# facebookresearch/SlowFast

Measured on AMD Instinct MI355X. Metric: clips/sec (fwd+bwd), SlowFast-8x8-R50 32x224^2 synthetic clips, per-GPU batch 32, higher is better.
Workload: dtype fp16; 1 GPU; SLOWFAST_8x8_R50: forward + cross_entropy loss + backward + sgd step, inputs resident in HBM, per-GPU batch 32; global_batch=32, parallelism=dp1, launch=hip-graph(fwd+bwd) + eager all-reduce/optimizer, optimizer=FlatOptimizer (fused unscale+norm+clip+update, dynamic loss scale on device)

## Files before the change

include/sfamd.h:

```cpp
#ifndef SFAMD_H
#define SFAMD_H
#include <stddef.h>
#include <stdint.h>
#ifdef __cplusplus
extern "C" {
#endif

#define SF_ABI_VERSION 26
typedef void* sf_stream_t;

typedef struct sf_conv_desc {
    int32_t N, Ci, Ti, Hi, Wi;
    int32_t Co, To, Ho, Wo;
    int32_t kT, kH, kW;
    int32_t sT, sH, sW;
    int32_t pT, pH, pW;
    int32_t dT, dH, dW;
    int32_t Cw;
    int32_t ldx, ldy;
    int32_t Cow;
} sf_conv_desc;

int sf_abi_version(void);
const char* sf_backend(void);
#define SF_ACT_FP16 0
#define SF_ACT_BF16_ID 1
int sf_act_dtype(void);
const char* sf_last_error(void);
const char* sf_build_id(void);

int sf_conv_weight_ld(const sf_conv_desc* d, int32_t* ldf, int32_t* ldd);
int sf_prep_weights(const sf_conv_desc* d, const float* w, void* wf, void* wd, sf_stream_t stream);
typedef struct sf_prep_item {
    const float* w;
    void* wf;
    void* wd;
    int32_t Co, Cow, Cw, Cp, taps, ldf, ldd;
    int32_t pad;
} sf_prep_item;
int sf_prep_item_fill(const sf_conv_desc* d, const float* w, void* wf, void* wd, sf_prep_item* item);
int64_t sf_prep_item_blocks(const sf_prep_item* item);
int sf_prep_weights_batch(const sf_prep_item* items, const int32_t* blk_item, const int32_t* blk_off, int32_t nblocks,
                          sf_stream_t stream);
int sf_conv_fwd_mtiles(const sf_conv_desc* d);
int sf_conv_fwd(const sf_conv_desc* d, const void* x, const void* wf, const float* in_scale, const float* in_shift,
                int in_relu, const float* bias, void* y, float* stat_part, sf_stream_t stream);
int sf_conv_fwd_fused(const sf_conv_desc* d, const void* x, const void* wf, const float* bias, const void* resid,
                      int32_t ldr, int out_relu, void* y, sf_stream_t stream);
int sf_conv_dgrad(const sf_conv_desc* d, const void* dy, const void* wd, const void* resid, int32_t ldr,
                  const void* resid_bits, void* dx, sf_stream_t stream);
int sf_conv_dgrad_bn(const sf_conv_desc* d, const void* dy, const void* wd, const void* resid, int32_t ldr,
                     const void* resid_bits, void* dx, const float* mask_scale, const float* mask_shift,
                     const void* mask_bits, const void* bn_y, int32_t bn_ldy, float* bn_part, int32_t bn_part_rows,
                     int32_t* bn_rows, sf_stream_t stream);
int64_t sf_conv_wgrad_workspace(const sf_conv_desc* d);
int64_t sf_conv_wgrad_rowtab_bytes(const sf_conv_desc* d);
int sf_conv_wgrad_rowtab(const sf_conv_desc* d, void* tab, sf_stream_t stream);
int sf_conv_wgrad(const sf_conv_desc* d, const void* x, const float* in_scale, const float* in_shift, int in_relu,
                  const void* dy, float* dw, float out_scale, int zero_first, void* workspace, int64_t workspace_bytes,
                  const void* rowtab, sf_stream_t stream);

int sf_bn_finalize(float* part, int32_t nblk, int32_t C, int32_t Creal, float count, const float* gamma, const float* beta,
                   float* running_mean, float* running_var, float momentum, float eps, float* scale, float* shift,
                   float* save_mean, float* save_rstd, sf_stream_t stream);
int sf_bn_act(int64_t M, int32_t C, const void* y, int32_t ldy, const float* scale, const float* shift, const void* r,
              int32_t ldr, const float* rscale, const float* rshift, int relu, void* out, int32_t ldo, void* mask_out,
              sf_stream_t stream);
int sf_bn_bwd_blocks(int64_t M, int32_t C);
int sf_bn_bwd_reduce(int64_t M, int32_t C, const void* dz, int32_t lddz, const void* zmask, int32_t ldm, const void* y,
                     int32_t ldy, const float* scale, const float* shift, int relu_self, float* part,
                     sf_stream_t stream);
int sf_bn_bwd_finalize(float* part, int32_t nblk, int32_t C, int32_t Creal, float count, const float* gamma, const float* mean,
                       const float* rstd, float inv_loss_scale, float* dgamma, float* dbeta, int accumulate,
                       float* coef, sf_stream_t stream);
int sf_bn_bwd_apply(int64_t M, int32_t C, const void* dz, int32_t lddz, const void* zmask, int32_t ldm, const void* y,
                    int32_t ldy, const float* scale, const float* shift, int relu_self, const float* coef, void* dy,
                    int32_t lddy, void* gout, int32_t ldg, sf_stream_t stream);

int sf_pool_fwd(int32_t N, int32_t T, int32_t H, int32_t W, int32_t C, int32_t kH, int32_t kW, int32_t sH, int32_t sW,
                int32_t pH, int32_t pW, const void* y, int32_t ldy, const float* scale, const float* shift, int relu,
                void* out, int32_t ldo, void* argmax, int32_t cls, sf_stream_t stream);
int sf_pool_bwd(int32_t N, int32_t T, int32_t H, int32_t W, int32_t C, int32_t kH, int32_t kW, int32_t sH, int32_t sW,
                int32_t pH, int32_t pW, const void* pooled, int32_t ldp, const void* argmax, int relu,
                const void* dout, int32_t lddo, void* g, int32_t ldg, int32_t cls, sf_stream_t stream);

int sf_pool3d_fwd(int32_t N, int32_t T, int32_t H, int32_t W, int32_t C, int32_t kT, int32_t kH, int32_t kW, const void* x,
                  int32_t ldx, void* out, int32_t ldo, void* argmax, sf_stream_t stream);
int sf_pool3d_bwd(int32_t N, int32_t T, int32_t H, int32_t W, int32_t C, int32_t kT, int32_t kH, int32_t kW,
                  const void* argmax, const void* dout, int32_t lddo, void* dx, int32_t lddx, sf_stream_t stream);

int sf_ncthw_to_cl(const float* x, int32_t N, int32_t C, int64_t S, int32_t Cp, void* out, sf_stream_t stream);
int sf_cl_to_ncthw(const void* x, int32_t ld, int32_t N, int32_t C, int64_t S, float* out, sf_stream_t stream);


int sf_bgemm(int64_t M, int32_t N, int32_t K, const void* A, int32_t lda, const void* W, int32_t ldw, const float* bias,
             const void* resid, int32_t ldr, void* Y, int32_t ldy, int32_t nbatch, int32_t bh, int64_t sa_b, int64_t sa_h,
             int64_t sw_b, int64_t sw_h, int64_t sy_b, int64_t sy_h, int64_t sr_b, int64_t sr_h, int32_t resid_row0,
             float alpha, sf_stream_t stream);
typedef struct sf_rows32 {
    const float* in;
    float* out;
    int32_t ld, period;
} sf_rows32;
int sf_gemm_rows32(int64_t M, int32_t N, int32_t K, const void* A, int32_t lda, const void* W, int32_t ldw, const float* bias,
                   const void* resid, int32_t ldr, void* Y, int32_t ldy, const sf_rows32* side, sf_stream_t stream);
int sf_bgemm_tn(int64_t M, int32_t R, int32_t Kc, const void* P, int32_t ldp, const void* X, int32_t ldx, void* Out,
                int32_t ldo, float scale, int32_t nbatch, int32_t bh, int64_t sp_b, int64_t sp_h, int64_t sx_b,
                int64_t sx_h, int64_t so_b, int64_t so_h, sf_stream_t stream);

int sf_layernorm_fwd(int64_t M, int32_t C, const void* x, int32_t ldx, const float* gamma, const float* beta, float eps,
                     void* y, int32_t ldy, float* mean, float* rstd, sf_stream_t stream);
int sf_layernorm_fwd_rows32(int64_t M, int32_t C, const void* x, int32_t ldx, const float* gamma, const float* beta, float eps,
                            void* y, int32_t ldy, float* mean, float* rstd, const sf_rows32* side, sf_stream_t stream);
int sf_layernorm_bwd_blocks(int64_t M, int32_t C);
int sf_layernorm_bwd(int64_t M, int32_t C, const void* dy, int32_t lddy, const void* x, int32_t ldx, const float* gamma,
                     const float* mean, const float* rstd, const void* resid, int32_t ldr, void* dx, int32_t lddx,
                     float* part, sf_stream_t stream);
int sf_layernorm_bwd_sums(int64_t M, int32_t C, const void* dy, int32_t lddy, const void* x, int32_t ldx, const float* gamma,
                          const float* mean, const float* rstd, const void* resid, int32_t ldr, void* dx, int32_t lddx,
                          float* part, sf_stream_t stream);
int sf_colsum_blocks(int64_t M, int32_t C);
int sf_colsum(int64_t M, int32_t C, const void* x, int32_t ldx, float* part, sf_stream_t stream);
int sf_colsum_finalize(float* part, int32_t nblk, int32_t C, int32_t fold, float* out0, float* out1, float scale,
                       int accumulate, sf_stream_t stream);
typedef struct sf_colfin_item {
    float* part;
    int32_t nblk, C, fold;
    float* out0;
    float* out1;
    float scale;
    int32_t accumulate;
    int32_t row_stride;
} sf_colfin_item;
int sf_colsum_finalize_batch(const sf_colfin_item* items, int32_t n, sf_stream_t stream);
int sf_rows_sum(const float* part, int32_t nblk, int64_t row_len, int64_t offset, int32_t n, float* out, float scale,
                int accumulate, sf_stream_t stream);
int sf_gelu_fwd(int64_t n, const void* h, void* a, sf_stream_t stream);
int sf_gelu_bwd(int64_t n, const void* h, const void* da, void* dh, sf_stream_t stream);

typedef struct sf_dw_desc {
    int32_t N, C, Cw, cls;
    int32_t Ti, Hi, Wi, To, Ho, Wo;
    int32_t kT, kH, kW, sT, sH, sW, pT, pH, pW;
    int32_t ldx, ldy;
    int32_t Cwreal;
} sf_dw_desc;
int sf_dwconv_fwd_blocks(const sf_dw_desc* d);
int sf_dwconv_fwd_sample_rows(const sf_dw_desc* d);
int sf_dwconv_fwd(const sf_dw_desc* d, const void* x, const float* w, void* y, float* stat_part, sf_stream_t stream);
int sf_dwconv_dgrad(const sf_dw_desc* d, const void* dy, const float* w, void* dx, sf_stream_t stream);
int sf_dwconv_dgrad_sum_rows(const sf_dw_desc* d);
int sf_dwconv_dgrad_sums(const sf_dw_desc* d, const void* dy, const float* w, void* dx, float* sum_part, sf_stream_t stream);
int64_t sf_dwconv_wgrad_workspace(const sf_dw_desc* d);
int sf_dwconv_wgrad(const sf_dw_desc* d, const void* x, const void* dy, float* dw, float out_scale, int zero_first,
                    void* workspace, int64_t workspace_bytes, sf_stream_t stream);
int sf_dwconv_pair_ok(const sf_dw_desc* d);
int sf_dwconv_fwd_pair(const sf_dw_desc* d, const void* x, const void* x2, const float* w, const float* w2, void* y, void* y2,
                       sf_stream_t stream);
int sf_dwconv_dgrad_pair(const sf_dw_desc* d, const void* dy, const void* dy2, const float* w, const float* w2, void* dx, void* dx2,
                         sf_stream_t stream);
int sf_dwconv_wgrad_pair(const sf_dw_desc* d, const void* x, const void* x2, const void* dy, const void* dy2, float* dw, float* dw2,
                         float out_scale, int zero_first, int zero_first2, void* workspace, int64_t workspace_bytes,
                         sf_stream_t stream);

typedef struct sf_attn_desc {
    int32_t B, heads, D, cls;
    int32_t Nq, qT, qH, qW;
    int32_t Nk, kT, kH, kW;
    int32_t rows_h, rows_w, rows_t;
} sf_attn_desc;
int sf_relpos_gather(const sf_attn_desc* d, const void* G, int32_t ldg, const int32_t* idx_h, const int32_t* idx_w,
                     const int32_t* idx_t, float* rq, sf_stream_t stream);
int sf_relpos_scatter(const sf_attn_desc* d, const float* drq, const int32_t* idx_h, const int32_t* idx_w,
                      const int32_t* idx_t, void* E, int32_t lde, sf_stream_t stream);
int sf_relpos_pack(const float* rel_h, const float* rel_w, const float* rel_t, int32_t rows_h, int32_t rows_w, int32_t rows_t,
                   int32_t D, int32_t TRp, void* t16, void* t16t, sf_stream_t stream);
int sf_relpos_unpack(const float* dtab, int32_t rows_h, int32_t rows_w, int32_t rows_t, int32_t D, float* grad_h, float* grad_w,
                     float* grad_t, int32_t acc_h, int32_t acc_w, int32_t acc_t, sf_stream_t stream);
int sf_softmax_fwd(const sf_attn_desc* d, void* s, int32_t lds, float scale, const float* rq, sf_stream_t stream);
int sf_softmax_bwd(const sf_attn_desc* d, void* dp, const void* prob, int32_t lds, float scale, float* drq,
                   sf_stream_t stream);
int sf_attn_fwd(const sf_attn_desc* d, const void* q, int32_t ldq, const void* k, const void* v, int32_t ldk, float scale,
                const float* rq, const void* onehot, int32_t residual, void* o, int32_t ldo, float* lse,
                sf_stream_t stream);
int64_t sf_attn_bwd_workspace(const sf_attn_desc* d);
int sf_attn_bwd(const sf_attn_desc* d, const void* q, int32_t ldq, const void* k, const void* v, int32_t ldk, float scale,
                const float* rq, const void* onehot, int32_t residual, const void* o, const void* dout, int32_t ldo,
                const float* lse, float* delta, void* dq, int32_t lddq, void* dk, void* dv, int32_t lddk, float* drq,
                void* workspace, int64_t workspace_bytes, sf_stream_t stream);
int sf_tmean_fwd(int32_t B, int32_t T, int64_t HW, int32_t C, const void* x, int32_t ldx, float* m, sf_stream_t stream);
int sf_tmean_bwd(int32_t B, int32_t T, int64_t HW, int32_t C, const float* dm, void* dx, int32_t lddx, sf_stream_t stream);
int sf_roi_align_max_fwd(int32_t R, int32_t B, int32_t H, int32_t W, int32_t C, int32_t res, float scale, int32_t aligned,
                         const float* m, const float* rois, float* out, int32_t ldo, int32_t col0, void* argmax,
                         sf_stream_t stream);
int sf_roi_align_max_bwd(int32_t R, int32_t B, int32_t H, int32_t W, int32_t C, int32_t res, float scale, int32_t aligned,
                         const float* rois, const float* dout, int32_t lddo, int32_t col0, const void* argmax, float* dm,
                         sf_stream_t stream);
int sf_gemm_act(int64_t M, int32_t N, int32_t K, const void* A, int32_t lda, const void* W, int32_t ldw, const float* bias,
                void* Y, int32_t ldy, int32_t mode, void* aux, int32_t ldaux, sf_stream_t stream);
int sf_gemm_act_colsum(int64_t M, int32_t N, int32_t K, const void* A, int32_t lda, const void* W, int32_t ldw,
                       const float* bias, void* Y, int32_t ldy, int32_t mode, void* aux, int32_t ldaux,
                       float* colsum_part, int32_t colsum_part_rows, int32_t* colsum_rows, sf_stream_t stream);
int sf_pack_clip_u8(const void* frames, int32_t N, int32_t Tin, int32_t H, int32_t W, const int32_t* t_index, int32_t Tout,
                    float mean0, float mean1, float mean2, float std0, float std1, float std2, int32_t reverse, void* out,
                    sf_stream_t stream);
int sf_mix_clip_f32(const float* src, float* dst, int32_t B, int32_t C, int32_t T, int32_t H, int32_t W, int32_t mode,
                    float lam, float one_minus_lam, int32_t yl, int32_t yh, int32_t xl, int32_t xh, sf_stream_t stream);
// ... 72 lines not shown
```

slowfast_amd/csrc/sf_api.hip:

```cpp
#include "../../include/sfamd.h"
#include "sf_bn.h"
#include "sf_common.h"
#include "sf_igemm.h"
#include "sf_igemm2.h"
#include "sf_wgrad2.h"
#include "sf_pool.h"
#include "sf_dwconv.h"
#include "sf_dwsweep.h"
#include "sf_dwtemporal.h"
#include "sf_tokens.h"
#include "sf_x3d.h"
#include "sf_stem.h"
#include "sf_attn.h"
#include "sf_roi.h"
#include "sf_optim.h"
#include "sf_mixup.h"
#include "sf_erase.h"

#include <stdarg.h>
#include <stdio.h>
#include <stdlib.h>
#include <string.h>

static thread_local char g_err[512] = "";

static int fail(const char* fmt, ...) {
    va_list ap;
    va_start(ap, fmt);
    vsnprintf(g_err, sizeof(g_err), fmt, ap);
    va_end(ap);
    return -1;
}
static int check_launch(const char* what) {
    hipError_t e = hipGetLastError();
    if (e != hipSuccess) return fail("%s: launch failed: %s", what, hipGetErrorString(e));
    return 0;
}
#define REQUIRE(cond, ...) \
    do { if (!(cond)) return fail(__VA_ARGS__); } while (0)

static inline int cdiv(int64_t a, int64_t b) { return (int)((a + b - 1) / b); }
static inline int roundup(int a, int b) { return (a + b - 1) / b * b; }

static inline int test_hook(const char* name, int def) { const char* e = getenv(name); return e ? atoi(e) : def; }
#ifdef SF_DIAG
static inline int tune_knob(const char* name, int def) { const char* e = getenv(name); return e ? atoi(e) : def; }
#else
#define tune_knob(name, def) (def)
#endif

extern "C" int sf_abi_version(void) { return SF_ABI_VERSION; }
extern "C" const char* sf_backend(void) {
#ifdef SF_HOSTSIM
    return "hostsim";
#else
    return "gfx950";
#endif
}
extern "C" int sf_act_dtype(void) { return SF_ACT_DTYPE_ID; }
extern "C" const char* sf_last_error(void) { return g_err; }
#ifndef SF_BUILD_ID
#define SF_BUILD_ID "unversioned"
#endif
extern "C" const char* sf_build_id(void) {
    static const char tagged[] = "sfamd-build-id:" SF_BUILD_ID;
    return tagged + 15;
}

static int check_desc(const sf_conv_desc* d) {
    REQUIRE(d != nullptr, "conv: null descriptor");
    REQUIRE(d->N > 0 && d->Ci > 0 && d->Co > 0, "conv: empty tensor");
    REQUIRE(d->Ci % 8 == 0 && d->Co % 8 == 0, "conv: channel counts must be multiples of 8 (Ci=%d Co=%d)", d->Ci, d->Co);
    REQUIRE(d->ldx >= d->Ci && d->ldx % 8 == 0 && d->ldy >= d->Co && d->ldy % 8 == 0, "conv: bad row pitch");
    REQUIRE(d->Cw > 0 && d->Cw <= d->Ci, "conv: Cw must be in (0, Ci]");
    REQUIRE(d->Cow >= 0 && d->Cow <= d->Co, "conv: Cow must be in [0, Co]");
    REQUIRE(d->sT > 0 && d->sH > 0 && d->sW > 0 && d->dT > 0 && d->dH > 0 && d->dW > 0, "conv: stride/dilation");
    int To = (d->Ti + 2 * d->pT - d->dT * (d->kT - 1) - 1) / d->sT + 1;
    int Ho = (d->Hi + 2 * d->pH - d->dH * (d->kH - 1) - 1) / d->sH + 1;
    int Wo = (d->Wi + 2 * d->pW - d->dW * (d->kW - 1) - 1) / d->sW + 1;
    REQUIRE(d->To >= 1 && d->Ho >= 1 && d->Wo >= 1 && d->To <= To && d->Ho <= Ho && d->Wo <= Wo,
            "conv: output dims (%d,%d,%d) exceed the geometry's (%d,%d,%d)", d->To, d->Ho, d->Wo, To, Ho, Wo);
    int64_t Mo = (int64_t)d->N * d->To * d->Ho * d->Wo, Mi = (int64_t)d->N * d->Ti * d->Hi * d->Wi;
    REQUIRE(Mo < (1ll << 31) && Mi < (1ll << 31), "conv: more than 2^31 positions");
    return 0;
}

static void fill_gather_common(GatherSide& g, const sf_conv_desc* d) {
    g.kT = d->kT; g.kH = d->kH; g.kW = d->kW;
    g.strT = d->sT; g.strH = d->sH; g.strW = d->sW;
    g.padT = d->pT; g.padH = d->pH; g.padW = d->pW;
    g.dilT = d->dT; g.dilH = d->dH; g.dilW = d->dW;
    g.fdkW = make_fastdiv(d->kW);
    g.fdkH = make_fastdiv(d->kH);
    g.fdsT = make_fastdiv(d->sT);
    g.fdsH = make_fastdiv(d->sH);
    g.fdsW = make_fastdiv(d->sW);
    g.scale = nullptr; g.shift = nullptr; g.relu = 0;
    g.fdHW = make_fastdiv((uint32_t)d->Hi * (uint32_t)d->Wi);
}
static bool is_pointwise(const sf_conv_desc* d) {
    return d->kH == 1 && d->kW == 1 && d->sT == 1 && d->sH == 1 && d->sW == 1 && d->pH == 0 && d->pW == 0 &&
           d->Ho == d->Hi && d->Wo == d->Wi;
}

static GatherSide gather_fwd(const sf_conv_desc* d, const void* x, const float* sc, const float* sh, int relu) {
    GatherSide g;
    memset(&g, 0, sizeof(g));
    fill_gather_common(g, d);
    g.src = (const f16*)x; g.ld = d->ldx; g.C = d->Ci;
    g.sT = d->Ti; g.sH = d->Hi; g.sW = d->Wi;
    g.mode = 0;
    g.Ktot = d->kT * d->kH * d->kW * d->Ci;
    g.fdC = make_fastdiv(d->Ci);
    g.fdrW = make_fastdiv(d->Wo); g.fdrH = make_fastdiv(d->Ho); g.fdrT = make_fastdiv(d->To);
    g.rowT = d->To;
    g.scale = sc; g.shift = sh; g.relu = relu;
    return g;
}
static GatherSide gather_dgrad(const sf_conv_desc* d, const void* dy) {
    GatherSide g;
    memset(&g, 0, sizeof(g));
    fill_gather_common(g, d);
    g.src = (const f16*)dy; g.ld = d->ldy; g.C = d->Co;
    g.sT = d->To; g.sH = d->Ho; g.sW = d->Wo;
    g.mode = 1;
    g.Ktot = d->kT * d->kH * d->kW * d->Co;
    g.fdC = make_fastdiv(d->Co);
    g.fdrW = make_fastdiv(d->Wi); g.fdrH = make_fastdiv(d->Hi); g.fdrT = make_fastdiv(d->Ti);
    g.rowT = d->Ti;
    return g;
}

static bool igemm_glds_ok(const IgemmParams& p, bool pw) {
    static const bool off = tune_knob("SF_IGEMM_GLDS", 1) == 0;
    if (off || !pw || p.g.scale) return false;
    if (p.g.Ktot != p.g.C || p.g.Ktot % 32 != 0 || p.g.ld % 8 != 0 || p.ldw % 8 != 0) return false;
    if (p.g.padT != 0) return false;
    if (((uintptr_t)p.g.src | (uintptr_t)p.wmat) & 15) return false;
    if (p.bh > 0 && ((p.sa_b | p.sa_h | p.sw_b | p.sw_h) & 7)) return false;
    return true;
}

template <int BN, int WM, int WN>
static void launch_igemm(const IgemmParams& p, bool pw, hipStream_t s, int nbatch = 1) {
    int mt = cdiv(p.M, 128);
    dim3 grid((unsigned)(mt * p.ntiles_n), (unsigned)nbatch);
    static const bool occ4 = tune_knob("SF_IGEMM_OCC4", 1) != 0;
    if (p.f32.out) {
        if (igemm_glds_ok(p, pw)) hipLaunchKernelGGL((sf_igemm_kernel<BN, WM, WN, true, true, BN == 128, true>), grid, dim3(SF_THREADS), 0, s, p);
        else hipLaunchKernelGGL((sf_igemm_kernel<BN, WM, WN, true, false, BN == 128, true>), grid, dim3(SF_THREADS), 0, s, p);
        return;
    }
    if (igemm_glds_ok(p, pw)) {
        hipLaunchKernelGGL((sf_igemm_kernel<BN, WM, WN, true, true, BN == 128>), grid, dim3(SF_THREADS), 0, s, p);
        return;
    }
    constexpr bool kCap = BN == 128;
    const bool cap = kCap && occ4;
    if (pw) {
        if (cap) hipLaunchKernelGGL((sf_igemm_kernel<BN, WM, WN, true, false, kCap>), grid, dim3(SF_THREADS), 0, s, p);
        else hipLaunchKernelGGL((sf_igemm_kernel<BN, WM, WN, true, false, false>), grid, dim3(SF_THREADS), 0, s, p);
    } else {
        if (cap) hipLaunchKernelGGL((sf_igemm_kernel<BN, WM, WN, false, false, kCap>), grid, dim3(SF_THREADS), 0, s, p);
        else hipLaunchKernelGGL((sf_igemm_kernel<BN, WM, WN, false, false, false>), grid, dim3(SF_THREADS), 0, s, p);
    }
}

template <int BN, int BK>
static void launch_igemm2(Igemm2Params& q, hipStream_t s) {
    q.ntiles_n = cdiv(q.Nout, BN);
    const dim3 grid((unsigned)(cdiv(q.M, 256) * q.ntiles_n));
    if constexpr (BN >= 64) {
        if (q.f32.out) { hipLaunchKernelGGL((sf_igemm2_kernel<256, BN, 4, 2, BK, 3, true>), grid, dim3(512), 0, s, q); return; }
    }
    hipLaunchKernelGGL((sf_igemm2_kernel<256, BN, 4, 2, BK, 3>), grid, dim3(512), 0, s, q);
}
static void launch_igemm2_auto(Igemm2Params& q, hipStream_t s) {
    const char* e;
    const int tiles = cdiv(q.M, 256) * cdiv(q.Nout, q.Nout > 64 ? 128 : 64);
    const int force_bk = tune_knob("SF_IGEMM2_BK", 0);
    const bool bk64 = q.C % 64 == 0 && force_bk != 32 && (force_bk == 64 || tiles <= 320);
    static const bool trace = test_hook("SF_TRACE", 0) != 0;
    q.ablate = tune_knob("SF_IGEMM2_ABLATE", 0);
    if (trace) fprintf(stderr, "[sfamd] igemm2: M=%d N=%d C=%d taps=%d BK=%d omap=%d\n", q.M, q.Nout, q.C, q.ntaps, bk64 ? 64 : 32, q.omap);
    const int t128 = test_hook("SF_IGEMM2_T128", 1);
    if (t128 && q.linear && q.Nout > 64 && !q.stat_part && !q.bnb_part && (!bk64 || t128 == 2)) {
        q.ntiles_n = cdiv(q.Nout, 128);
        const dim3 grid((unsigned)(cdiv(q.M, 128) * q.ntiles_n));
        if (q.f32.out) hipLaunchKernelGGL((sf_igemm2_kernel<128, 128, 2, 2, 32, 3, true>), grid, dim3(256), 0, s, q);
        else hipLaunchKernelGGL((sf_igemm2_kernel<128, 128, 2, 2, 32, 3>), grid, dim3(256), 0, s, q);
        return;
    }
    if (q.Nout > 64) { if (bk64) launch_igemm2<128, 64>(q, s); else launch_igemm2<128, 32>(q, s); }
    else if (q.Nout > 32) { if (bk64) launch_igemm2<64, 64>(q, s); else launch_igemm2<64, 32>(q, s); }
    else launch_igemm2<32, 32>(q, s);
}
static bool igemm2_operands_ok(const IgemmParams& p, int nbatch) {
    const GatherSide& g = p.g;
    if (nbatch != 1 || g.scale) return false;
    if (p.bh > 1 || (p.bh == 1 && (p.sa_b | p.sa_h | p.sw_b | p.sw_h | p.sy_b | p.sy_h | p.sr_b | p.sr_h))) return false;
    const int taps = g.kT * g.kH * g.kW;
    if (taps > SF_I2_MAXTAPS || g.C % 32 != 0 || g.Ktot != taps * g.C) return false;
    if (g.ld % 8 != 0 || p.ldw % 8 != 0 || p.ldw < g.Ktot) return false;
    if (((uintptr_t)g.src | (uintptr_t)p.wmat) & 15) return false;
    if ((g.kT - 1) * g.dilT > 127 || (g.kH - 1) * g.dilH > 127 || (g.kW - 1) * g.dilW > 127) return false;
    return true;
}
static void igemm2_common(Igemm2Params& q, const IgemmParams& p) {
    const GatherSide& g = p.g;
    memset(&q, 0, sizeof(q));
    q.src = g.src; q.ld = g.ld; q.C = g.C;
    q.sT = g.sT; q.sH = g.sH; q.sW = g.sW;
    q.wmat = p.wmat; q.ldw = p.ldw; q.Nout = p.Nout;
    q.y = p.y; q.ldy = p.ldy; q.bias = p.bias; q.resid = p.resid; q.ldr = p.ldr; q.stat_part = p.stat_part;
    q.act_mode = p.act_mode; q.act_aux = p.act_aux; q.ld_aux = p.ld_aux; q.resid_row0 = p.resid_row0; q.alpha = p.alpha;
    q.resid_bits = p.resid_bits;
    q.bnb_y = p.bnb_y; q.bnb_ld = p.bnb_ld; q.bnb_scale = p.bnb_scale; q.bnb_shift = p.bnb_shift; q.bnb_part = p.bnb_part;
    q.bnb_bits = p.bnb_bits;
    q.f32 = p.f32;
    q.linear = p.linear;
}
static bool try_igemm2(const IgemmParams& p, hipStream_t s, int nbatch = 1) {
    const char* e;
    const bool off = test_hook("SF_IGEMM2", 1) == 0;
    const int mink = test_hook("SF_IGEMM2_MINK", 512);
    const int minrows = test_hook("SF_IGEMM2_MINROWS", 4096);
    const GatherSide& g = p.g;
    if (off || !igemm2_operands_ok(p, nbatch)) return false;
    if (g.Ktot < mink || p.Nout <= 32 || p.M < minrows) return false;
    if (g.mode == 1 && !(g.strT == 1 && g.strH == 1 && g.strW == 1)) return false;
    const int taps = g.kT * g.kH * g.kW;
    Igemm2Params q;
    igemm2_common(q, p);
    q.fdrW = g.fdrW; q.fdrH = g.fdrH; q.fdrT = g.fdrT;
    const int sgn = g.mode == 0 ? 1 : -1;
    if (g.mode == 0) {
        q.mulT = g.strT; q.mulH = g.strH; q.mulW = g.strW;
        q.offT = -g.padT; q.offH = -g.padH; q.offW = -g.padW;
    } else {
        q.mulT = q.mulH = q.mulW = 1;
        q.offT = g.padT; q.offH = g.padH; q.offW = g.padW;
    }
    q.ntaps = taps;
    int t = 0;
    for (int kt = 0; kt < g.kT; ++kt)
        for (int kh = 0; kh < g.kH; ++kh)
            for (int kw = 0; kw < g.kW; ++kw, ++t) {
                const int dt = sgn * kt * g.dilT, dh = sgn * kh * g.dilH, dw = sgn * kw * g.dilW;
                q.dt[t] = (int8_t)dt; q.dh[t] = (int8_t)dh; q.dw[t] = (int8_t)dw;
                q.taps[t].dlin = (dt * g.sH + dh) * g.sW + dw;
                q.taps[t].wcol = t * g.C;
            }
    q.M = p.M;
    launch_igemm2_auto(q, s);
    return true;
}

static bool try_igemm2_strided_dgrad(const IgemmParams& p, hipStream_t s) {
    const char* e;
    const bool off = test_hook("SF_IGEMM2", 1) == 0 || tune_knob("SF_IGEMM2_STRIDED", 1) == 0;
    const int minrows = test_hook("SF_IGEMM2_MINROWS", 4096);
    const GatherSide& g = p.g;
    if (off || g.mode != 1 || (g.strT == 1 && g.strH == 1 && g.strW == 1)) return false;
    if (!igemm2_operands_ok(p, 1) || p.Nout <= 16 || p.M < minrows || p.stat_part || p.act_mode) return false;
    const int Ti = (int)g.fdrT.d, Hi = (int)g.fdrH.d, Wi = (int)g.fdrW.d;
    const int N = p.M / (Ti * Hi * Wi);
    const int str[3] = {g.strT, g.strH, g.strW}, pad[3] = {g.padT, g.padH, g.padW}, dil[3] = {g.dilT, g.dilH, g.dilW};
    const int ker[3] = {g.kT, g.kH, g.kW}, ext[3] = {Ti, Hi, Wi};
    for (int rt = 0; rt < str[0]; ++rt)
        for (int rh = 0; rh < str[1]; ++rh)
            for (int rw = 0; rw < str[2]; ++rw) {
                const int r[3] = {rt, rh, rw};
                int q0[3], cnt[3];
                bool empty = false;
                for (int a = 0; a < 3; ++a) {
                    const int num = pad[a] - r[a];
                    q0[a] = num > 0 ? (num + str[a] - 1) / str[a] : 0;
                    const int top = ext[a] - 1 + pad[a] - r[a];
                    const int q1 = top >= 0 ? top / str[a] : -1;
                    cnt[a] = q1 - q0[a] + 1;
                    if (cnt[a] <= 0) empty = true;
                }
                if (empty) continue;
                Igemm2Params q;
                igemm2_common(q, p);
                q.fdrT = make_fastdiv(cnt[0]); q.fdrH = make_fastdiv(cnt[1]); q.fdrW = make_fastdiv(cnt[2]);
                q.mulT = q.mulH = q.mulW = 1;
                q.offT = q0[0]; q.offH = q0[1]; q.offW = q0[2];
                int nt = 0, tap = 0;
                for (int kt = 0; kt < ker[0]; ++kt)
                    for (int kh = 0; kh < ker[1]; ++kh)
                        for (int kw = 0; kw < ker[2]; ++kw, ++tap) {
                            const int k[3] = {kt, kh, kw};
                            int d[3];
                            bool ok = true;
                            for (int a = 0; a < 3; ++a) {
                                const int v = r[a] - k[a] * dil[a];
                                if (v % str[a] != 0) { ok = false; break; }
                                d[a] = v / str[a];
                            }
                            if (!ok) continue;
                            q.dt[nt] = (int8_t)d[0]; q.dh[nt] = (int8_t)d[1]; q.dw[nt] = (int8_t)d[2];
                            q.taps[nt].dlin = (d[0] * g.sH + d[1]) * g.sW + d[2];
                            q.taps[nt].wcol = tap * g.C;
                            ++nt;
                        }
                q.ntaps = nt;
                q.M = N * cnt[0] * cnt[1] * cnt[2];
                q.omap = 1;
                q.oT = Ti; q.oH = Hi; q.oW = Wi;
                q.omT = str[0]; q.omH = str[1]; q.omW = str[2];
                q.ooT = str[0] * q0[0] + r[0] - pad[0]; q.ooH = str[1] * q0[1] + r[1] - pad[1]; q.ooW = str[2] * q0[2] + r[2] - pad[2];
                launch_igemm2_auto(q, s);
            }
    return true;
}

static int run_igemm(IgemmParams& p, bool pw, hipStream_t s, int* bm_used = nullptr) {
    if (bm_used) *bm_used = 256;
    if (try_igemm2(p, s)) return check_launch("igemm2");
    if (bm_used) *bm_used = 0;
    if (try_igemm2_strided_dgrad(p, s)) return check_launch("igemm2 strided dgrad");
    if (bm_used) *bm_used = 128;
    if (p.Nout > 64) { p.ntiles_n = cdiv(p.Nout, 128); launch_igemm<128, 64, 64>(p, pw, s); }
    else if (p.Nout > 32) { p.ntiles_n = 1; launch_igemm<64, 32, 64>(p, pw, s); }
    else if (p.Nout > 16) { p.ntiles_n = 1; launch_igemm<32, 32, 32>(p, pw, s); }
    else { p.ntiles_n = 1; launch_igemm<16, 32, 16>(p, pw, s); }
    return check_launch("igemm");
}

struct StemPlan {
    bool ok, thin3, small;
    int tiles_w, tiles_h, tiles_t, ntiles, F, PR;
    int wg_blocks, tiles_per_block, Kpad, wgroups;
    size_t ws_bytes;
};
static StemPlan plan_stem(const sf_conv_desc* d) {
    StemPlan s;
    memset(&s, 0, sizeof(s));
    static const bool off = tune_knob("SF_STEM_GENERIC", 0) != 0;
    if (off) return s;
    static const bool thin3_on = tune_knob("SF_STEM_THIN3", 1) != 0;
    const bool stemlike = d->kW == 4 && d->pW == 2;
    const bool thin3 = thin3_on && d->kW == 3 && d->pW == 1 && d->sH == 1 && d->sT == 1;
    if (d->Ci != 8 || d->Cw != 8 || !(stemlike || thin3) || d->sW != 1 || d->dT != 1 || d->dH != 1 || d->dW != 1)
        return s;
    s.thin3 = thin3;
    if (d->Co > 16 || d->Co % 8 != 0 || (d->Cow && d->Cow != d->Co)) return s;
    if (d->kT * d->kH > SF_STEM_MAX_SLICES) return s;
    s.F = (SF_STEM_TT - 1) * d->sT + d->kT;
    s.PR = (SF_STEM_TH - 1) * d->sH + d->kH;
    if ((int64_t)s.F * s.PR * SF_STEM_PC > SF_STEM_CHUNKS) return s;
    s.small = (int64_t)s.F * s.PR * SF_STEM_PC <= SF_STEM_CHUNKS_SMALL;
    s.tiles_w = cdiv(d->Wo, SF_STEM_TW);
    s.tiles_h = cdiv(d->Ho, SF_STEM_TH);
    s.tiles_t = cdiv(d->To, SF_STEM_TT);
    const int64_t nt = (int64_t)d->N * s.tiles_t * s.tiles_h * s.tiles_w;
    if (nt >= (1ll << 30)) return s;
    s.ntiles = (int)nt;
    const int gmax = s.small ? 1024 : 512;
    int g = s.ntiles < gmax ? s.ntiles : gmax;
    s.tiles_per_block = cdiv(s.ntiles, g);
    s.wg_blocks = cdiv(s.ntiles, s.tiles_per_block);
    s.Kpad = roundup(d->kT * d->kH * 32, 128);
    { const int nsl = d->kT * d->kH; s.wgroups = nsl <= 4 ? 8 / nsl : 1; }
    s.ws_bytes = (size_t)s.wg_blocks * s.wgroups * 16 * s.Kpad * 4;
    s.ok = true;
    return s;
}
#define SF_STEM_SLIDE_GROUPS 4
#define SF_STEM_FWD_LAUNCH(sp, q, stream)                                                                                          \
    do {                                                                                                                          \
        static const bool rm_ = tune_knob("SF_STEM_ROWMAJOR", 1) != 0;                           \
        const dim3 g_((sp).ntiles), b_(SF_THREADS);                                                                               \
        const int sg_ = test_hook("SF_STEM_SLIDE", SF_STEM_SLIDE_GROUPS);                                                         \
        if (rm_ && sg_ > 0 && (q).sH == 2 && (q).kH == 7 && !(sp).small && (q).sT == 1 && (q).kT > 1 && (q).kT <= 5 &&            \
            (q).Co <= 8 && !(q).bnb_y) {                                                                                                         \
            StemParams qs_ = (q);                    \
            qs_.seg_groups = sg_ < (sp).tiles_t ? sg_ : (sp).tiles_t;                                                             \
            qs_.tiles_t = cdiv((sp).tiles_t, qs_.seg_groups);                                                                     \
            qs_.fd_tt = make_fastdiv(qs_.tiles_t);                                                                                \
            const dim3 gs_((unsigned)((int64_t)(q).N * qs_.tiles_t * (sp).tiles_h * (sp).tiles_w));                                \
            if (test_hook("SF_TRACE", 0)) fprintf(stderr, "[sfamd] stem_fwd_slide: %u runs of %d groups\n", gs_.x, qs_.seg_groups); \
            hipLaunchKernelGGL((sf_stem_fwd_slide_kernel<2, 7>), gs_, b_, 0, (hipStream_t)(stream), qs_);                         \
        } else if (rm_ && (q).sH == 2 && (q).kH == 7 && !(sp).small)                                                              \
            hipLaunchKernelGGL((sf_stem_fwd_kernel<SF_STEM_CHUNKS, 2, 7>), g_, b_, 0, (hipStream_t)(stream), q);                  \
        else if (rm_ && (q).sH == 1 && (q).kH == 3 && (sp).small)                                                                 \
            hipLaunchKernelGGL((sf_stem_fwd_kernel<SF_STEM_CHUNKS_SMALL, 1, 3>), g_, b_, 0, (hipStream_t)(stream), q);            \
        else if ((sp).small) hipLaunchKernelGGL((sf_stem_fwd_kernel<SF_STEM_CHUNKS_SMALL>), g_, b_, 0, (hipStream_t)(stream), q); \
        else hipLaunchKernelGGL((sf_stem_fwd_kernel<SF_STEM_CHUNKS>), g_, b_, 0, (hipStream_t)(stream), q);                       \
    } while (0)
static StemParams stem_params(const sf_conv_desc* d, const StemPlan& s, const void* x) {
    StemParams p;
    memset(&p, 0, sizeof(p));
    p.x = (const f16*)x; p.ldx = d->ldx;
    p.N = d->N; p.Ti = d->Ti; p.Hi = d->Hi; p.Wi = d->Wi;
    p.To = d->To; p.Ho = d->Ho; p.Wo = d->Wo; p.Co = d->Co;
    p.kT = d->kT; p.kH = d->kH; p.sT = d->sT; p.sH = d->sH; p.pT = d->pT; p.pH = d->pH;
    p.pW = d->pW;
    if (s.thin3) { p.wo0 = 0; p.wos = 24; p.wog = 8; p.kwc = 3; }
    else { p.wo0 = 0; p.wos = 32; p.wog = 8; p.kwc = 4; }
    p.ldy = d->ldy;
    p.tiles_w = s.tiles_w; p.tiles_h = s.tiles_h; p.tiles_t = s.tiles_t; p.ntiles = s.ntiles;
    p.fd_tw = make_fastdiv(s.tiles_w); p.fd_th = make_fastdiv(s.tiles_h); p.fd_tt = make_fastdiv(s.tiles_t);
    p.F = s.F; p.PR = s.PR;
    p.fd_pc = make_fastdiv(SF_STEM_PC); p.fd_prpc = make_fastdiv(s.PR * SF_STEM_PC);
    p.Kpad = s.Kpad; p.tiles_per_block = s.tiles_per_block; p.wgroups = s.wgroups;
    return p;
}

extern "C" int sf_conv_weight_ld(const sf_conv_desc* d, int32_t* ldf, int32_t* ldd) {
    REQUIRE(d && ldf && ldd, "sf_conv_weight_ld: null argument");
    int taps = d->kT * d->kH * d->kW;
    *ldf = roundup(taps * d->Ci, 32);
    *ldd = roundup(taps * d->Co, 32);
    return 0;
}

static PrepParams prep_params(const sf_conv_desc* d, const float* w, void* wf, void* wd) {
    PrepParams p;
    memset(&p, 0, sizeof(p));
    p.w = w; p.Co = d->Co; p.Cow = d->Cow ? d->Cow : d->Co; p.Cw = d->Cw; p.Cp = d->Ci; p.taps = d->kT * d->kH * d->kW;
    int32_t ldf, ldd;
    sf_conv_weight_ld(d, &ldf, &ldd);
    p.wf = (f16*)wf; p.ldf = ldf; p.wd = (f16*)wd; p.ldd = ldd;
    return p;
}

extern "C" int sf_prep_weights(const sf_conv_desc* d, const float* w, void* wf, void* wd, sf_stream_t stream) {
    if (check_desc(d)) return -1;
    REQUIRE(w && wf, "sf_prep_weights: null pointer");
    const PrepParams p = prep_params(d, w, wf, wd);
    int64_t total = (int64_t)p.Co * p.ldf + (wd ? (int64_t)p.Cp * p.ldd : 0);
    int blocks = (int)((total + SF_THREADS - 1) / SF_THREADS);
    if (blocks > 4096) blocks = 4096;
    hipLaunchKernelGGL(sf_prep_weights_kernel, dim3(blocks), dim3(SF_THREADS), 0, (hipStream_t)stream, p);
    return check_launch("prep_weights");
}

static_assert(sizeof(sf_prep_item) == sizeof(PrepParams), "sf_prep_item must mirror PrepParams");
extern "C" int sf_prep_item_fill(const sf_conv_desc* d, const float* w, void* wf, void* wd, sf_prep_item* item) {
    if (check_desc(d)) return -1;
    REQUIRE(w && wf && item, "sf_prep_item_fill: null pointer");
    PrepParams p = prep_params(d, w, wf, wd);
    p.pad = sf_prep_tile_co(p.taps);
    memcpy(item, &p, sizeof(p));
    return 0;
}

extern "C" int64_t sf_prep_item_blocks(const sf_prep_item* item) {
    REQUIRE(item && item->Co > 0 && item->ldf > 0 && item->taps > 0, "sf_prep_item_blocks: bad item");
    REQUIRE(item->pad == sf_prep_tile_co(item->taps), "sf_prep_item_blocks: item was not written by sf_prep_item_fill");
    if (item->pad > 0) return (int64_t)cdiv(item->Co, item->pad) * cdiv(item->Cp, SF_PREP_TILE_CI);
    const int64_t n = (int64_t)item->Co * item->ldf + (item->wd ? (int64_t)item->Cp * item->ldd : 0);
    return cdiv(n, SF_PREP_BLOCK_ELEMS);
}

extern "C" int sf_prep_weights_batch(const sf_prep_item* items, const int32_t* blk_item, const int32_t* blk_off,
                                     int32_t nblocks, sf_stream_t stream) {
    REQUIRE(items && blk_item && blk_off && nblocks > 0, "sf_prep_weights_batch: bad arguments");
    hipLaunchKernelGGL(sf_prep_weights_batch_kernel, dim3(nblocks), dim3(SF_THREADS), 0, (hipStream_t)stream,
                       (const PrepParams*)items, blk_item, blk_off);
    return check_launch("prep_weights_batch");
}

extern "C" int sf_conv_fwd_mtiles(const sf_conv_desc* d) {
    if (!d) return fail("sf_conv_fwd_mtiles: null descriptor");
    return cdiv((int64_t)d->N * d->To * d->Ho * d->Wo, 128);
}

extern "C" int sf_conv_fwd(const sf_conv_desc* d, const void* x, const void* wf, const float* in_scale,
                           const float* in_shift, int in_relu, const float* bias, void* y, float* stat_part,
                           sf_stream_t stream) {
    if (check_desc(d)) return -1;
    REQUIRE(x && wf && y, "sf_conv_fwd: null pointer");
    REQUIRE((in_scale == nullptr) == (in_shift == nullptr), "sf_conv_fwd: in_scale/in_shift must come together");
    REQUIRE(!in_scale || d->Ci <= 512, "sf_conv_fwd: fused input BatchNorm supports Ci <= 512 (got %d)", d->Ci);
    if (!in_scale && !bias) {
        const StemPlan sp = plan_stem(d);
        if (sp.ok && (!stat_part || sp.ntiles <= sf_conv_fwd_mtiles(d))) {
            StemParams q = stem_params(d, sp, x);
            int32_t ldf0, ldd0;
            sf_conv_weight_ld(d, &ldf0, &ldd0);
            q.wmat = (const f16*)wf; q.ldw = ldf0; q.y = (f16*)y;
            q.stat_part = stat_part; q.stat_rows = sf_conv_fwd_mtiles(d);
            const bool trace = test_hook("SF_TRACE", 0) != 0;
            if (trace) fprintf(stderr, "[sfamd] stem_fwd: %d tiles, patch %dx%dx%d chunks\n", sp.ntiles, sp.F, sp.PR, SF_STEM_PC);
            SF_STEM_FWD_LAUNCH(sp, q, stream);
            return check_launch("stem_fwd");
        }
    }
    IgemmParams p;
    memset(&p, 0, sizeof(p));
    p.g = gather_fwd(d, x, in_scale, in_shift, in_relu);
    p.M = d->N * d->To * d->Ho * d->Wo;
    int32_t ldf, ldd;
    sf_conv_weight_ld(d, &ldf, &ldd);
    p.wmat = (const f16*)wf; p.ldw = ldf; p.Nout = d->Co;
    p.ksteps = cdiv(p.g.Ktot, 32);
    p.y = (f16*)y; p.ldy = d->ldy;
    p.bias = bias; p.resid = nullptr; p.ldr = 0;
    p.stat_part = stat_part;
    return run_igemm(p, is_pointwise(d), (hipStream_t)stream);
}

extern "C" int sf_conv_fwd_fused(const sf_conv_desc* d, const void* x, const void* wf, const float* bias,
                                 const void* resid, int32_t ldr, int out_relu, void* y, sf_stream_t stream) {
    if (check_desc(d)) return -1;
    REQUIRE(x && wf && y, "sf_conv_fwd_fused: null pointer");
    REQUIRE(!resid || (ldr >= d->Co && ldr % 8 == 0), "sf_conv_fwd_fused: bad residual pitch");
    if (!resid) {
        const StemPlan sp = plan_stem(d);
        if (sp.ok) {
            StemParams q = stem_params(d, sp, x);
            int32_t ldf0, ldd0;
            sf_conv_weight_ld(d, &ldf0, &ldd0);
            q.wmat = (const f16*)wf; q.ldw = ldf0; q.y = (f16*)y;
            q.bias = bias; q.out_relu = out_relu;
            SF_STEM_FWD_LAUNCH(sp, q, stream);
            return check_launch("stem_fwd_fused");
        }
    }
    IgemmParams p;
    memset(&p, 0, sizeof(p));
    p.g = gather_fwd(d, x, nullptr, nullptr, 0);
    p.M = d->N * d->To * d->Ho * d->Wo;
    int32_t ldf, ldd;
    sf_conv_weight_ld(d, &ldf, &ldd);
    p.wmat = (const f16*)wf; p.ldw = ldf; p.Nout = d->Co;
    p.ksteps = cdiv(p.g.Ktot, 32);
    p.y = (f16*)y; p.ldy = d->ldy;
    p.bias = bias; p.resid = (const f16*)resid; p.ldr = ldr;
    p.act_mode = out_relu ? 3 : 0;
    return run_igemm(p, is_pointwise(d), (hipStream_t)stream);
}

struct BnFuse {
    const float* scale; const float* shift; const void* bits;
    const void* y0; int32_t ld0; float* part0;
};
static int conv_dgrad_impl(const sf_conv_desc* d, const void* dy, const void* wd, const void* resid, int32_t ldr,
                           const void* resid_bits, void* dx, const BnFuse* bn, int32_t* bn_rows, sf_stream_t stream) {
    if (check_desc(d)) return -1;
    REQUIRE(dy && wd && dx, "sf_conv_dgrad: null pointer");
    REQUIRE(!resid || (ldr >= d->Ci && ldr % 8 == 0), "sf_conv_dgrad: bad residual pitch");
    IgemmParams p;
    memset(&p, 0, sizeof(p));
    p.g = gather_dgrad(d, dy);
    p.M = d->N * d->Ti * d->Hi * d->Wi;
    int32_t ldf, ldd;
    sf_conv_weight_ld(d, &ldf, &ldd);
    p.wmat = (const f16*)wd; p.ldw = ldd; p.Nout = d->Ci;
    p.ksteps = cdiv(p.g.Ktot, 32);
    p.y = (f16*)dx; p.ldy = d->ldx;
    p.resid = (const f16*)resid; p.ldr = ldr;
    REQUIRE(!resid_bits || resid, "sf_conv_dgrad: resid_bits without a residual");
    p.resid_bits = (const uint8_t*)resid_bits;
    const bool fuse = bn && d->sT == 1 && d->sH == 1 && d->sW == 1;
    if (!resid && d->Co == 8 && d->To == d->Ti && d->Ho == d->Hi && d->Wo == d->Wi) {
        sf_conv_desc dd = *d;
        dd.Ci = d->Co; dd.Cw = d->Co; dd.Co = d->Ci; dd.Cow = 0;
        dd.pT = d->kT - 1 - d->pT; dd.pH = d->kH - 1 - d->pH; dd.pW = d->kW - 1 - d->pW;
        dd.ldx = d->ldy; dd.ldy = d->ldx;
        const StemPlan sp = plan_stem(&dd);
        if (sp.ok && sp.thin3 && (!fuse || sp.ntiles <= cdiv(p.M, 128))) {
            StemParams q = stem_params(&dd, sp, dy);
            const int S = d->kT * d->kH;
            q.wmat = (const f16*)wd; q.ldw = ldd; q.y = (f16*)dx;
            q.wo0 = ((S - 1) * 3 + 2) * 8; q.wos = -24; q.wog = -8; q.kwc = 3;
            if (fuse) {
                q.bnb_y = (const f16*)bn->y0; q.bnb_ld = bn->ld0; q.bnb_scale = bn->scale; q.bnb_shift = bn->shift;
                q.bnb_bits = (const uint8_t*)bn->bits;
                q.stat_part = bn->part0; q.stat_rows = 0;
            }
            SF_STEM_FWD_LAUNCH(sp, q, stream);
            if (bn_rows) *bn_rows = fuse ? sp.ntiles : 0;
            return check_launch("stem_dgrad");
        }
    }
    if (fuse) {
        p.bnb_y = (const f16*)bn->y0; p.bnb_ld = bn->ld0; p.bnb_part = bn->part0;
        p.bnb_scale = bn->scale; p.bnb_shift = bn->shift; p.bnb_bits = (const uint8_t*)bn->bits;
    }
    int bm = 0;
    const int rc = run_igemm(p, is_pointwise(d), (hipStream_t)stream, &bm);
    if (bn_rows) *bn_rows = (fuse && bm > 0) ? cdiv(p.M, bm) : 0;
    return rc;
}

extern "C" int sf_conv_dgrad(const sf_conv_desc* d, const void* dy, const void* wd, const void* resid, int32_t ldr,
                             const void* resid_bits, void* dx, sf_stream_t stream) {
    return conv_dgrad_impl(d, dy, wd, resid, ldr, resid_bits, dx, nullptr, nullptr, stream);
}

extern "C" int sf_conv_dgrad_bn(const sf_conv_desc* d, const void* dy, const void* wd, const void* resid, int32_t ldr,
                                const void* resid_bits, void* dx, const float* mask_scale, const float* mask_shift,
                                const void* mask_bits, const void* bn_y, int32_t bn_ldy, float* bn_part, int32_t bn_part_rows,
                                int32_t* bn_rows, sf_stream_t stream) {
    REQUIRE(d && bn_y && bn_part && bn_rows, "sf_conv_dgrad_bn: null pointer");
    REQUIRE(mask_bits || (mask_scale && mask_shift), "sf_conv_dgrad_bn: a mask source is needed (mask_bits, or mask_scale + mask_shift)");
    REQUIRE(bn_ldy >= d->Ci && bn_ldy % 8 == 0 && ((uintptr_t)bn_y & 15) == 0, "sf_conv_dgrad_bn: bad bn_y pitch / alignment");
    REQUIRE((int64_t)bn_part_rows * 128 >= (int64_t)d->N * d->Ti * d->Hi * d->Wi,
            "sf_conv_dgrad_bn: the partial table needs ceil(positions / 128) rows of [2][Ci] floats");
    const BnFuse bn = {mask_scale, mask_shift, mask_bits, bn_y, bn_ldy, bn_part};
    return conv_dgrad_impl(d, dy, wd, resid, ldr, resid_bits, dx, &bn, bn_rows, stream);
}

template <int BMW, int WM, int WN, int KS>
static void launch_wgrad(WgradParams& p, dim3 grid3, hipStream_t s) {
    p.tiles_k = grid3.x; p.tiles_c = grid3.y;
    const dim3 grid(grid3.x * grid3.y * grid3.z);
    hipLaunchKernelGGL((sf_wgrad_kernel<BMW, WM, WN, KS>), grid, dim3(SF_THREADS), 0, s, p);
}

struct WgradPlan {
    int BMW, KS, tiles_k, tiles_c, Co_pad, Kpad, nchunks, chunks_per_split, splits;
    size_t ws_bytes;
};
static WgradPlan plan_wgrad(const sf_conv_desc* d) {
    WgradPlan w;
    const int taps = d->kT * d->kH * d->kW;
    const int Ktot = taps * d->Ci;
    const int64_t M = (int64_t)d->N * d->To * d->Ho * d->Wo;
    w.BMW = d->Co >= 128 ? 128 : d->Co >= 64 ? 64 : d->Co >= 32 ? 32 : 16;
    w.KS = w.BMW <= 32 ? 4 : 1;
    w.tiles_k = cdiv(Ktot, 128);
    w.tiles_c = cdiv(d->Co, w.BMW);
    w.Kpad = w.tiles_k * 128;
    w.Co_pad = w.tiles_c * w.BMW;
    w.nchunks = cdiv(M, 32);
    const int64_t slab = (int64_t)w.Co_pad * w.Kpad * 4;
    static const int target = tune_knob("SF_WGRAD_BLOCKS", 1024);
    int splits = cdiv(target, (int64_t)w.tiles_k * w.tiles_c);
    const int64_t cap = (256ll << 20) / slab;
    if (splits > cap) splits = (int)(cap < 1 ? 1 : cap);
    const int nstages = cdiv(w.nchunks, w.KS);
    if (splits > nstages) splits = nstages;
    if (splits < 1) splits = 1;
    w.chunks_per_split = cdiv(nstages, splits) * w.KS;
    w.splits = cdiv(w.nchunks, w.chunks_per_split);
    w.ws_bytes = (size_t)slab * w.splits;
    return w;
}

struct Wgrad2Plan {
    bool ok, thin, dual;
    int BMW, BKW, tiles_k, tiles_c, Co_pad, Kpad, rows_per_split, splits;
    int slabs;
    size_t tab_bytes, ws_bytes;
};
static Wgrad2Plan plan_wgrad2(const sf_conv_desc* d) {
    Wgrad2Plan w;
    memset(&w, 0, sizeof(w));
    const char* e;
    if (test_hook("SF_WGRAD2", 1) == 0) return w;
    const int mink = test_hook("SF_WGRAD2_MINK", 192);
    const int minrows = test_hook("SF_WGRAD2_MINROWS", 4096);
    const int taps = d->kT * d->kH * d->kW;
    const int target = test_hook("SF_WGRAD2_BLOCKS", 512);
    (void)taps;
    const int Ktot = taps * d->Ci;
    const int64_t M = (int64_t)d->N * d->To * d->Ho * d->Wo;
    if (taps > SF_I2_MAXTAPS || M < minrows) return w;
    if ((d->kT - 1) * d->dT > 127 || (d->kH - 1) * d->dH > 127 || (d->kW - 1) * d->dW > 127) return w;
    if (plan_stem(d).ok) return w;
    if (d->Co <= 32) {
        if (test_hook("SF_WGRAD2T", 1) == 0) return w;
        const int minrows_t = test_hook("SF_WGRAD2T_MINROWS", 16384);
        if (M < minrows_t) return w;
        w.thin = true;
        w.BMW = d->Co <= 16 ? 16 : 32;
        w.BKW = Ktot <= 32 ? 32 : 128;
        w.tiles_k = cdiv(Ktot, w.BKW);
        w.tiles_c = 1;
        w.Kpad = w.tiles_k * w.BKW;
        w.Co_pad = w.BMW;
        const int target_t = test_hook("SF_WGRAD2T_BLOCKS", w.BKW == 128 ? 512 : w.BMW == 32 ? 768 : 1024);
        int splits = target_t / w.tiles_k;
        if (splits < 1) splits = 1;
        w.rows_per_split = roundup(cdiv(M, splits), 128);
        w.splits = cdiv(M, w.rows_per_split);
        w.tab_bytes = ((size_t)M * 8 + 255) / 256 * 256 + 1280;
        w.ws_bytes = w.tab_bytes + (size_t)w.Co_pad * w.Kpad * 4 * w.splits;
        w.slabs = w.splits;
        w.ok = true;
        return w;
    }
    if (Ktot < mink) return w;
    w.BMW = d->Co > 64 ? 128 : 64;
    w.tiles_k = cdiv(Ktot, 256);
    w.tiles_c = cdiv(d->Co, w.BMW);
    w.Kpad = w.tiles_k * 256;
    w.Co_pad = w.tiles_c * w.BMW;
    int splits = target / (w.tiles_k * w.tiles_c);
    const int64_t slab = (int64_t)w.Co_pad * w.Kpad * 4;
    const int64_t cap = (256ll << 20) / slab;
    if (splits > cap) splits = (int)(cap < 1 ? 1 : cap);
    if (splits < 1) splits = 1;
    w.dual = false;
    if (splits >= 2 && test_hook("SF_WGRAD2_DUAL", 1) != 0) {
        const int tiles = w.tiles_k * w.tiles_c;
        const int pairs = (target / 2) / tiles;
        const int64_t steps = cdiv(cdiv(M, splits), 32);
        if (pairs >= 1 && 2 * pairs * 10 >= (2 * pairs < splits ? splits : 2 * pairs) * 9 && steps <= test_hook("SF_WGRAD2_DUAL_STEPS", 80)) {
            w.dual = true;
            if (2 * pairs < splits) splits = 2 * pairs;
        }
    }
    w.rows_per_split = roundup(cdiv(M, splits), 32);
    w.splits = cdiv(M, w.rows_per_split);
    if (w.splits < 2) w.dual = false;
    w.slabs = w.dual ? cdiv(w.splits, 2) : w.splits;
    w.tab_bytes = ((size_t)M * 8 + 255) / 256 * 256 + 1280;
    w.ws_bytes = w.tab_bytes + (size_t)slab * w.splits;
    w.ok = true;
    return w;
}

static void launch_rowtab(const sf_conv_desc* d, void* tab, hipStream_t s) {
    RowtabParams t;
    memset(&t, 0, sizeof(t));
    t.tab = (i32x2*)tab;
    t.M = d->N * d->To * d->Ho * d->Wo;
    t.fdW = make_fastdiv(d->Wo); t.fdH = make_fastdiv(d->Ho); t.fdT = make_fastdiv(d->To);
    t.sT = d->Ti; t.sH = d->Hi; t.sW = d->Wi;
    t.strT = d->sT; t.strH = d->sH; t.strW = d->sW; t.padT = d->pT; t.padH = d->pH; t.padW = d->pW;
    t.ntaps = d->kT * d->kH * d->kW;
    int ti = 0;
    for (int kt = 0; kt < d->kT; ++kt)
        for (int kh = 0; kh < d->kH; ++kh)
            for (int kw = 0; kw < d->kW; ++kw, ++ti) {
                t.dt[ti] = (int8_t)(kt * d->dT); t.dh[ti] = (int8_t)(kh * d->dH); t.dw[ti] = (int8_t)(kw * d->dW);
            }
    hipLaunchKernelGGL(sf_wgrad2_rowtab_kernel, dim3(cdiv(t.M, SF_THREADS)), dim3(SF_THREADS), 0, s, t);
}

extern "C" int64_t sf_conv_wgrad_rowtab_bytes(const sf_conv_desc* d) {
    if (check_desc(d)) return -1;
    const Wgrad2Plan w2 = plan_wgrad2(d);
    return w2.ok ? (int64_t)w2.tab_bytes : 0;
}

extern "C" int sf_conv_wgrad_rowtab(const sf_conv_desc* d, void* tab, sf_stream_t stream) {
    if (check_desc(d)) return -1;
    REQUIRE(tab && (uintptr_t)tab % 16 == 0, "sf_conv_wgrad_rowtab: tab must be a 16-byte aligned device pointer");
    REQUIRE(plan_wgrad2(d).ok, "sf_conv_wgrad_rowtab: this geometry does not take the row-table kernel (sf_conv_wgrad_rowtab_bytes == 0)");
    launch_rowtab(d, tab, (hipStream_t)stream);
    return check_launch("wgrad_rowtab");
}

extern "C" int64_t sf_conv_wgrad_workspace(const sf_conv_desc* d) {
    if (check_desc(d)) return -1;
    int64_t generic = (int64_t)plan_wgrad(d).ws_bytes;
    const Wgrad2Plan w2 = plan_wgrad2(d);
    if (w2.ok && (int64_t)w2.ws_bytes > generic) generic = (int64_t)w2.ws_bytes;
    const StemPlan sp = plan_stem(d);
    return sp.ok && (int64_t)sp.ws_bytes > generic ? (int64_t)sp.ws_bytes : generic;
}
// ... 2009 lines not shown
```

slowfast_amd/csrc/sf_igemm.h:

```cpp
#pragma once
#include "sf_common.h"

struct IgemmParams {
    GatherSide g;
    int M;
    const f16* wmat;
    int ldw;
    int Nout;
    int ksteps;
    f16* y;
    int ldy;
    const float* bias;
    const f16* resid;
    int ldr;
    float* stat_part;
    int ntiles_n;
    int bh;
    int64_t sa_b, sa_h, sw_b, sw_h, sy_b, sy_h, sr_b, sr_h;
    int act_mode;
    f16* act_aux;
    int ld_aux;
    int resid_row0;
    const uint8_t* resid_bits;
    float alpha;
    const f16* bnb_y; int bnb_ld;
    const float* bnb_scale; const float* bnb_shift;
    float* bnb_part;
    const uint8_t* bnb_bits;
    F32Rows f32;
    int linear;
};

__device__ __forceinline__ void bnb_accumulate(const f16x8& dz, const f16x8& yv, const float (&sc)[8], const float (&sh)[8],
                                               float (&sg)[8], float (&sgy)[8], bool use_bits, uint32_t bits) {
#pragma unroll
    for (int e = 0; e < 8; ++e) {
        const bool open = use_bits ? ((bits >> e) & 1u) != 0u : ((float)yv[e] * sc[e] + sh[e] > 0.f);
        const float g = open ? (float)dz[e] : 0.f;
        sg[e] += g;
        sgy[e] += g * (float)yv[e];
    }
}

struct EpiLoads {
    f16x8 r, y;
    uint32_t rbits, bbits;
};

template <int NW, int CG>
__device__ __forceinline__ void bnb_reduce_store(float (&sg)[8], float (&sgy)[8], float* red, float* prow, int n0, int Nout,
                                                 float* sgy2 = nullptr, float* prow2 = nullptr) {
    const int tid = threadIdx.x, lane = tid & 63, wave = tid >> 6;
#pragma unroll
    for (int e = 0; e < 8; ++e)
        for (int mask = CG; mask < 64; mask <<= 1) {
            sg[e] += __shfl_xor(sg[e], mask);
            sgy[e] += __shfl_xor(sgy[e], mask);
            if (prow2) sgy2[e] += __shfl_xor(sgy2[e], mask);
        }
    __syncthreads();
    if (lane < CG) {
#pragma unroll
        for (int e = 0; e < 8; ++e) {
            red[(wave * CG + lane) * 24 + e] = sg[e];
            red[(wave * CG + lane) * 24 + 8 + e] = sgy[e];
            if (prow2) red[(wave * CG + lane) * 24 + 16 + e] = sgy2[e];
        }
    }
    __syncthreads();
    if (tid < CG * 8) {
        const int cgi = tid >> 3, e = tid & 7;
        const int col = n0 + cgi * 8 + e;
        if (col < Nout) {
            float s = 0.f, q = 0.f, q2 = 0.f;
#pragma unroll
            for (int w = 0; w < NW; ++w) {
                s += red[(w * CG + cgi) * 24 + e];
                q += red[(w * CG + cgi) * 24 + 8 + e];
                if (prow2) q2 += red[(w * CG + cgi) * 24 + 16 + e];
            }
            prow[col] = s;
            prow[Nout + col] = q;
            if (prow2) { prow2[col] = s; prow2[Nout + col] = q2; }
        }
    }
}

template <int BN, int WM, int WN, bool PW, bool GL = false, bool OCC4 = false, bool F32R = false>
__global__ __launch_bounds__(SF_THREADS, OCC4 ? 4 : 1) void sf_igemm_kernel(IgemmParams p) {
    constexpr int BM = 128, BK = 32;
    constexpr int NST = 2;
    constexpr int WAVES_N = BN / WN, WAVES_M = BM / WM;
    static_assert(WAVES_M * WAVES_N == 4, "4 waves per workgroup");
    constexpr int TM = WM / 16, TN = WN / 16;
    constexpr int A_ELEMS = BM * BK, B_ELEMS = BN * BK;
    constexpr int STG_LD = BN + 8;
    constexpr int SMEM_MAIN = NST * (A_ELEMS + B_ELEMS), SMEM_STG = BM * STG_LD;
    constexpr int SMEM = SMEM_MAIN > SMEM_STG ? SMEM_MAIN : SMEM_STG;
    constexpr int NB = (BN * 4 + SF_THREADS - 1) / SF_THREADS;

    constexpr int TF_BYTES = GL ? 0 : 2 * 512 * 4;
    __shared__ __attribute__((aligned(16))) unsigned char lds_raw[SMEM * 2 + TF_BYTES + WAVES_M * 2 * BN * 4];
    f16* const smem = reinterpret_cast<f16*>(lds_raw);
    float* const s_scale = reinterpret_cast<float*>(lds_raw + SMEM * 2);
    float* const s_shift = s_scale + 512;
    float (*const s_red)[2][BN] = reinterpret_cast<float (*)[2][BN]>(lds_raw + SMEM * 2 + TF_BYTES);

    const int tid = threadIdx.x;
    const int lane = tid & 63, wave = __builtin_amdgcn_readfirstlane(tid >> 6);
    const int wm = wave / WAVES_N, wn = wave % WAVES_N;
    const int tile = (int)xcd_remap(blockIdx.x, gridDim.x);
    const int nt = tile % p.ntiles_n, mt = tile / p.ntiles_n;
    const int m0 = mt * BM, n0 = nt * BN;
    const GatherSide& g = p.g;
    const bool has_tf = g.scale != nullptr;
    const f16* a_src = g.src;
    const f16* wmat = p.wmat;
    f16* yout = p.y;
    const f16* resid = p.resid;
    if (p.bh > 0) {
        const int zb = blockIdx.y / p.bh, zj = blockIdx.y % p.bh;
        a_src += zb * p.sa_b + zj * p.sa_h;
        wmat += zb * p.sw_b + zj * p.sw_h;
        yout += zb * p.sy_b + zj * p.sy_h;
        if (resid) resid += zb * p.sr_b + zj * p.sr_h;
    }

    if constexpr (!GL) {
        if (has_tf) {
            for (int c = tid; c < g.C; c += SF_THREADS) {
                s_scale[c] = g.scale[c];
                s_shift[c] = g.shift[c];
            }
        }
    }

    const int kq = tid & 3;
    RowPos rp[2];
    if constexpr (!GL) {
#pragma unroll
        for (int j = 0; j < 2; ++j) {
            int row = m0 + (tid >> 2) + 64 * j;
            rp[j] = PW ? decode_row_pw(g, (uint32_t)row, row < p.M) : decode_row(g, (uint32_t)row, row < p.M);
        }
    }
    const float act_lo = g.relu ? 0.f : -INFINITY;
    constexpr int NBC = (BN / 16 + 3) / 4;
    const f16* ga[2];
    const f16* gb[NBC];
    if constexpr (GL) {
#pragma unroll
        for (int j = 0; j < 2; ++j) {
            const int row = (wave + 4 * j) * 16 + (lane >> 2);
            const int slot = ((lane & 3) - 2 * ((row >> 2) & 3)) & 3;
            int m = m0 + row;
            if (m >= p.M) m = p.M - 1;
            ga[j] = a_src + (int64_t)m * g.ld + slot * 8;
        }
#pragma unroll
        for (int j = 0; j < NBC; ++j) {
            const int row = (wave + 4 * j) * 16 + (lane >> 2);
            const int slot = ((lane & 3) - 2 * ((row >> 2) & 3)) & 3;
            int co = n0 + row;
            if (co >= p.Nout) co = p.Nout - 1;
            gb[j] = wmat + (int64_t)co * p.ldw + slot * 8;
        }
    }
    auto issue_tile = [&](int ks, int buf) {
        f16* As = smem + buf * (A_ELEMS + B_ELEMS);
        f16* Bs = As + A_ELEMS;
#pragma unroll
        for (int j = 0; j < 2; ++j) SF_GLOBAL_LOAD_LDS16(ga[j] + ks * BK, As + (wave + 4 * j) * 16 * BK);
#pragma unroll
        for (int j = 0; j < NBC; ++j)
            if ((wave + 4 * j) * 16 < BN) SF_GLOBAL_LOAD_LDS16(gb[j] + ks * BK, Bs + (wave + 4 * j) * 16 * BK);
    };

    struct Stage {
        f16x8 ra[2], rb[NB];
        bool ok[2];
        uint32_t c0;
    };
    Stage st0;

    auto load_tile = [&](int ks, Stage& st) {
        const uint32_t k0 = (uint32_t)(ks * BK + kq * 8);
#pragma unroll
        for (int j = 0; j < 2; ++j) {
            int64_t off;
            uint32_t c0 = 0;
            bool ok = PW ? gather_offset_pw(g, rp[j], k0, off, c0) : gather_offset(g, rp[j], k0, off, c0);
            st.ra[j] = ok ? ld16(a_src + off) : zero8();
            st.ok[j] = ok;
            if (ok) st.c0 = c0;
        }
#pragma unroll
        for (int j = 0; j < NB; ++j) {
            int idx = tid + SF_THREADS * j;
            int brow = idx >> 2;
            int co = n0 + brow;
            bool ok = (idx < BN * 4) && (co < p.Nout) && (k0 < (uint32_t)g.Ktot);
            st.rb[j] = ok ? ld16(wmat + (int64_t)co * p.ldw + k0) : zero8();
        }
    };
    auto store_tile = [&](int buf, const Stage& st) {
        f16* As = smem + buf * (A_ELEMS + B_ELEMS);
        f16* Bs = As + A_ELEMS;
#pragma unroll
        for (int j = 0; j < 2; ++j) {
            f16x8 v = st.ra[j];
            if (has_tf && st.ok[j]) v = bn_act8(v, s_scale + st.c0, s_shift + st.c0, act_lo);
            st16(As + lds_tile_off((tid >> 2) + 64 * j, kq), v);
        }
#pragma unroll
        for (int j = 0; j < NB; ++j) {
            int idx = tid + SF_THREADS * j;
            if (idx < BN * 4) st16(Bs + lds_tile_off(idx >> 2, kq), st.rb[j]);
        }
    };

    f32x4 acc[TM][TN];
#pragma unroll
    for (int i = 0; i < TM; ++i)
#pragma unroll
        for (int j = 0; j < TN; ++j) acc[i][j] = (f32x4){0.f, 0.f, 0.f, 0.f};

    auto compute = [&](int buf) {
        const f16* As = smem + buf * (A_ELEMS + B_ELEMS);
        const f16* Bs = As + A_ELEMS;
        f16x8 af[TM], bf[TN];
#pragma unroll
        for (int i = 0; i < TM; ++i) af[i] = ld16(As + lds_tile_off(wm * WM + i * 16 + (lane & 15), lane >> 4));
#pragma unroll
        for (int j = 0; j < TN; ++j) bf[j] = ld16(Bs + lds_tile_off(wn * WN + j * 16 + (lane & 15), lane >> 4));
#pragma unroll
        for (int i = 0; i < TM; ++i)
#pragma unroll
            for (int j = 0; j < TN; ++j)
                acc[i][j] = SF_MFMA16(af[i], bf[j], acc[i][j]);
    };

    if constexpr (GL) {
        issue_tile(0, 0);
        SF_WAIT_VMEM();
        __syncthreads();
        for (int ks = 0; ks < p.ksteps; ++ks) {
            if (ks + 1 < p.ksteps) issue_tile(ks + 1, (ks + 1) & 1);
            compute(ks & 1);
            SF_WAIT_VMEM();
            __syncthreads();
        }
    } else {
        if (has_tf) __syncthreads();
        load_tile(0, st0);
        store_tile(0, st0);
        __syncthreads();
        for (int ks = 0; ks < p.ksteps; ++ks) {
            const bool more = ks + 1 < p.ksteps;
            if (more) load_tile(ks + 1, st0);
            compute(ks & 1);
            if (more) store_tile((ks + 1) & 1, st0);
            __syncthreads();
        }
    }

    {
        const float alpha = p.alpha != 0.f ? p.alpha : 1.f;
#pragma unroll
        for (int j = 0; j < TN; ++j) {
            const int colj = n0 + wn * WN + j * 16 + (lane & 15);
            const float b = (p.bias && colj < p.Nout) ? p.bias[colj] : 0.f;
#pragma unroll
            for (int i = 0; i < TM; ++i)
#pragma unroll
                for (int r = 0; r < 4; ++r) acc[i][j][r] = acc[i][j][r] * alpha + b;
        }
    }
    if constexpr (F32R) f32_rows_epilogue<TM, TN>(acc, p.f32, m0 + wm * WM, n0 + wn * WN, p.M, p.Nout, resid, p.ldr, p.resid_row0);
    if (p.stat_part) {
#pragma unroll
        for (int j = 0; j < TN; ++j) {
            float s = 0.f, q = 0.f;
#pragma unroll
            for (int i = 0; i < TM; ++i)
#pragma unroll
                for (int r = 0; r < 4; ++r) {
                    const bool rowok = m0 + wm * WM + i * 16 + 4 * (lane >> 4) + r < p.M;
                    const float v = rowok ? acc[i][j][r] : 0.f;
                    s += v;
                    q += v * v;
                }
            s = wave_sum_over_row_groups(s);
            q = wave_sum_over_row_groups(q);
            if (lane < 16) {
                s_red[wm][0][wn * WN + j * 16 + lane] = s;
                s_red[wm][1][wn * WN + j * 16 + lane] = q;
            }
        }
    }
    f16* stg = smem;
#pragma unroll
    for (int i = 0; i < TM; ++i)
#pragma unroll
        for (int j = 0; j < TN; ++j) {
            const int col = wn * WN + j * 16 + (lane & 15);
#pragma unroll
            for (int r = 0; r < 4; ++r) {
                const int row = wm * WM + i * 16 + 4 * (lane >> 4) + r;
                stg[row * STG_LD + col] = (f16)acc[i][j][r];
            }
        }
    __syncthreads();
    if (p.stat_part && tid < BN) {
        const int col = n0 + tid;
        if (col < p.Nout) {
            float s = 0.f, q = 0.f;
#pragma unroll
            for (int w = 0; w < WAVES_M; ++w) {
                s += s_red[w][0][tid];
                q += s_red[w][1][tid];
            }
            p.stat_part[((int64_t)mt * 2 + 0) * p.Nout + col] = s;
            p.stat_part[((int64_t)mt * 2 + 1) * p.Nout + col] = q;
        }
    }
    constexpr int CG = BN / 8;
    static_assert(SF_THREADS % CG == 0 && 64 % CG == 0, "a thread keeps one column group over the whole store loop");
    const bool bnb = p.bnb_part != nullptr;
    float bsg[8], bsgy[8], bsc[8], bsh[8];
#pragma unroll
    for (int e = 0; e < 8; ++e) { bsg[e] = 0.f; bsgy[e] = 0.f; bsc[e] = 1.f; bsh[e] = 0.f; }
    if (bnb && p.bnb_y && !p.bnb_bits && n0 + (tid % CG) * 8 < p.Nout) { load8f(p.bnb_scale + n0 + (tid % CG) * 8, bsc); load8f(p.bnb_shift + n0 + (tid % CG) * 8, bsh); }
    constexpr int ITER = BM * CG / SF_THREADS > 0 ? BM * CG / SF_THREADS : 1;
    static_assert(BM * CG % SF_THREADS == 0 || BM * CG < SF_THREADS, "whole store iterations");
    constexpr int CH = (BN >= 128 && OCC4) ? 2 : 1;
    static_assert(ITER % CH == 0, "whole chunks");
    const int ecg = tid % CG, ecol = n0 + ecg * 8;
    for (int it0 = 0; it0 < ITER; it0 += CH) {
        EpiLoads L[CH];
        bool ok[CH], rok[CH];
#pragma unroll
        for (int u = 0; u < CH; ++u) {
            const int idx = tid + (it0 + u) * SF_THREADS;
            const int row = idx / CG, m = m0 + row;
            ok[u] = idx < BM * CG && m < p.M && ecol < p.Nout;
            rok[u] = ok[u] && resid && m >= p.resid_row0;
            if constexpr (F32R) {
                uint32_t srow;
                if (f32_row(p.f32, m, srow)) rok[u] = false;
            }
            L[u].rbits = 0xffu; L[u].bbits = 0u;
            if (rok[u]) {
                L[u].r = ld16(resid + (int64_t)m * p.ldr + ecol);
                if (p.resid_bits) L[u].rbits = p.resid_bits[(int64_t)m * (p.Nout >> 3) + (ecol >> 3)];
            }
            if (ok[u] && bnb && p.bnb_y) {
                L[u].y = ld16(p.bnb_y + (int64_t)m * p.bnb_ld + ecol);
                if (p.bnb_bits) L[u].bbits = p.bnb_bits[(int64_t)m * (p.Nout >> 3) + (ecol >> 3)];
            }
        }
#pragma unroll
        for (int u = 0; u < CH; ++u) {
            if (!ok[u]) continue;
            const int idx = tid + (it0 + u) * SF_THREADS;
            const int row = idx / CG, m = m0 + row;
            f16x8 v = ld16(stg + row * STG_LD + ecg * 8);
            if (rok[u]) {
#pragma unroll
                for (int e = 0; e < 8; ++e) {
                    const f16 r = ((L[u].rbits >> e) & 1u) ? L[u].r[e] : (f16)0.f;
                    v[e] = (f16)((float)v[e] + (float)r);
                }
            }
            if (p.act_mode == 2) {
                const f16x8 h = ld16(p.act_aux + (int64_t)m * p.ld_aux + ecol);
#pragma unroll
                for (int e = 0; e < 8; ++e) v[e] = (f16)((float)v[e] * gelu_df((float)h[e]));
            }
            if (p.act_mode == 3) {
#pragma unroll
                for (int e = 0; e < 8; ++e) v[e] = v[e] > (f16)0.f ? v[e] : (f16)0.f;
            }
            st16(yout + (int64_t)m * p.ldy + ecol, v);
            if (p.act_mode == 1) {
                f16x8 a;
#pragma unroll
                for (int e = 0; e < 8; ++e) a[e] = (f16)gelu_f((float)v[e]);
                st16(p.act_aux + (int64_t)m * p.ld_aux + ecol, a);
            }
            if (bnb && p.bnb_y) bnb_accumulate(v, L[u].y, bsc, bsh, bsg, bsgy, p.bnb_bits != nullptr, L[u].bbits);
            else if (bnb) {
#pragma unroll
                for (int e = 0; e < 8; ++e) bsg[e] += (float)v[e];
            }
        }
    }
    if (bnb) bnb_reduce_store<4, CG>(bsg, bsgy, reinterpret_cast<float*>(smem), p.bnb_part + (int64_t)mt * 2 * p.Nout, n0, p.Nout);
}

struct WgradParams {
    GatherSide g;
    const f16* dy;
    int ldy;
    int Co;
    int M;
    float* ws;
    int Co_pad, Kpad;
    int nchunks;
    int chunks_per_split;
    int tiles_k, tiles_c;
    int bh;
    int64_t sp_b, sp_h, sx_b, sx_h, so_b, so_h;
    f16* out16; int ldo; float out_scale;
};

struct WgradReduceParams {
    const float* ws;
    int splits, Co, Co_pad, Kpad, Ktot;
    FastDiv fdC;
    float* dw;
    int Cw, taps;
    float out_scale;
    int accumulate;
    int lanes;
    int slice4;
};

__global__ __launch_bounds__(SF_THREADS) void sf_wgrad_reduce_kernel(WgradReduceParams p) {
    __shared__ f32x4 s_acc[SF_THREADS];
    const int L = p.lanes, E = SF_THREADS / L;
    const int e = threadIdx.x % E, z0 = threadIdx.x / E;
    const int64_t total = (int64_t)p.Co * p.Kpad;
    const int64_t slab = (int64_t)p.Co_pad * p.Kpad;
    const int64_t idx = ((int64_t)blockIdx.x * E + e) * 4;
    f32x4 a0 = {0.f, 0.f, 0.f, 0.f}, a1 = a0, a2 = a0, a3 = a0;
    if (idx < total) {
        const float* src = p.ws + idx;
        int z = z0;
        for (; z + 3 * L < p.splits; z += 4 * L) {
            const f32x4 v0 = *reinterpret_cast<const f32x4*>(src + (int64_t)z * slab);
            const f32x4 v1 = *reinterpret_cast<const f32x4*>(src + (int64_t)(z + L) * slab);
            const f32x4 v2 = *reinterpret_cast<const f32x4*>(src + (int64_t)(z + 2 * L) * slab);
            const f32x4 v3 = *reinterpret_cast<const f32x4*>(src + (int64_t)(z + 3 * L) * slab);
            a0 += v0; a1 += v1; a2 += v2; a3 += v3;
        }
        for (; z < p.splits; z += L) a0 += *reinterpret_cast<const f32x4*>(src + (int64_t)z * slab);
    }
    s_acc[threadIdx.x] = (a0 + a1) + (a2 + a3);
    __syncthreads();
    for (int half = L >> 1; half >= 1; half >>= 1) {
        if (z0 < half) s_acc[threadIdx.x] += s_acc[threadIdx.x + half * E];
        __syncthreads();
    }
    if (z0 == 0 && idx < total) {
        const int co = (int)(idx / p.Kpad), kcol0 = (int)(idx % p.Kpad);
        const f32x4 r = s_acc[threadIdx.x];
#pragma unroll
        for (int j = 0; j < 4; ++j) {
            const int kcol = kcol0 + j;
            if (kcol < p.Ktot) {
                uint32_t tap, ci;
                fd_divmod((uint32_t)kcol, p.fdC, tap, ci);
                if (p.slice4) {
                    if ((tap & 3u) == 3u) continue;
                    tap = (tap >> 2) * 3u + (tap & 3u);
                }
                if (ci < (uint32_t)p.Cw) {
                    float* dst = p.dw + ((int64_t)co * p.Cw + ci) * p.taps + tap;
                    const float v = r[j] * p.out_scale;
                    *dst = p.accumulate ? *dst + v : v;
                }
            }
        }
    }
}

template <class V>
// ... 206 lines not shown
```

slowfast_amd/csrc/sf_igemm2.h:

```cpp
#pragma once
#include "sf_common.h"

#define SF_I2_MAXTAPS 32



struct Igemm2Tap {
    int32_t dlin;
    int32_t wcol;
};

struct Igemm2Params {
    const f16* src;
    int ld, C;
    int sT, sH, sW;
    FastDiv fdrW, fdrH, fdrT;
    int mulT, mulH, mulW, offT, offH, offW;
    int ntaps;
    int8_t dt[SF_I2_MAXTAPS], dh[SF_I2_MAXTAPS], dw[SF_I2_MAXTAPS];
    Igemm2Tap taps[SF_I2_MAXTAPS];
    int M;
    const f16* wmat;
    int ldw, Nout;
    f16* y;
    int ldy;
    const float* bias;
    const f16* resid;
    int ldr;
    float* stat_part;
    int ntiles_n;
    int act_mode;
    f16* act_aux;
    int ld_aux;
    int resid_row0;
    float alpha;
    const uint8_t* resid_bits;
    int omap;
    int oT, oH, oW, omT, omH, omW, ooT, ooH, ooW;
    const f16* bnb_y; int bnb_ld;
    const float* bnb_scale; const float* bnb_shift;
    float* bnb_part;
    const uint8_t* bnb_bits;
    int ablate;
    F32Rows f32;
    int linear;
};

template <int BK>
__device__ __forceinline__ int i2_lds_off(int row, int kslot) {
    if constexpr (BK == 64) return row * 64 + ((kslot ^ (row & 7)) << 3);
    else return lds_tile_off(row, kslot);
}

template <int BM, int BN, int WAVES_M, int WAVES_N, bool F32R>
__device__ __forceinline__ void i2_epilogue(const Igemm2Params& p, f32x4 (&acc)[BM / WAVES_M / 16][BN / WAVES_N / 16], f16* smem,
                                            float (*s_red)[2][BN], int* s_orow, int mt, int nt) {
    constexpr int NW = WAVES_M * WAVES_N, NT = 64 * NW;
    constexpr int WM = BM / WAVES_M, WN = BN / WAVES_N;
    constexpr int TM = WM / 16, TN = WN / 16;
    constexpr int STG_LD = BN + 8;
    constexpr int HALVES = BM / 128, WPH = WAVES_M / HALVES;
    static_assert(WAVES_M % HALVES == 0, "a wave row belongs to one 128-row group");
    const int tid = threadIdx.x;
    const int lane = tid & 63, wave = __builtin_amdgcn_readfirstlane(tid >> 6);
    const int wm = wave / WAVES_N, wn = wave % WAVES_N;
    const int m0 = mt * BM, n0 = nt * BN;
    {
        const float alpha = p.alpha != 0.f ? p.alpha : 1.f;
#pragma unroll
        for (int j = 0; j < TN; ++j) {
            const int colj = n0 + wn * WN + j * 16 + (lane & 15);
            const float b = (p.bias && colj < p.Nout) ? p.bias[colj] : 0.f;
#pragma unroll
            for (int i = 0; i < TM; ++i)
#pragma unroll
                for (int r = 0; r < 4; ++r) acc[i][j][r] = acc[i][j][r] * alpha + b;
        }
    }
    if constexpr (F32R) f32_rows_epilogue<TM, TN>(acc, p.f32, m0 + wm * WM, n0 + wn * WN, p.M, p.Nout, p.resid, p.ldr, p.resid_row0);
    if (p.stat_part) {
#pragma unroll
        for (int j = 0; j < TN; ++j) {
            float s = 0.f, q = 0.f;
#pragma unroll
            for (int i = 0; i < TM; ++i)
#pragma unroll
                for (int r = 0; r < 4; ++r) {
                    const bool rowok = m0 + wm * WM + i * 16 + 4 * (lane >> 4) + r < p.M;
                    const float v = rowok ? acc[i][j][r] : 0.f;
                    s += v;
                    q += v * v;
                }
            s = wave_sum_over_row_groups(s);
            q = wave_sum_over_row_groups(q);
            if (lane < 16) {
                s_red[wm][0][wn * WN + j * 16 + lane] = s;
                s_red[wm][1][wn * WN + j * 16 + lane] = q;
            }
        }
    }
    f16* stg = smem;
#pragma unroll
    for (int i = 0; i < TM; ++i)
#pragma unroll
        for (int j = 0; j < TN; ++j) {
            const int col = wn * WN + j * 16 + (lane & 15);
#pragma unroll
            for (int r = 0; r < 4; ++r) {
                const int row = wm * WM + i * 16 + 4 * (lane >> 4) + r;
                stg[row * STG_LD + col] = (f16)acc[i][j][r];
            }
        }
    __syncthreads();
    if (p.stat_part && tid < HALVES * BN) {
        const int half = tid / BN, c = tid % BN;
        const int col = n0 + c;
        const int prow = mt * HALVES + half;
        if (col < p.Nout && (int64_t)prow * 128 < p.M) {
            float s = 0.f, q = 0.f;
#pragma unroll
            for (int w = 0; w < WPH; ++w) {
                s += s_red[half * WPH + w][0][c];
                q += s_red[half * WPH + w][1][c];
            }
            p.stat_part[((int64_t)prow * 2 + 0) * p.Nout + col] = s;
            p.stat_part[((int64_t)prow * 2 + 1) * p.Nout + col] = q;
        }
    }
    constexpr int CG = BN / 8;
    static_assert(NT % CG == 0 && 64 % CG == 0, "a thread keeps one column group over the whole store loop");
    const bool bnb = p.bnb_part != nullptr;
    float bsg[8], bsgy[8], bsc[8], bsh[8];
#pragma unroll
    for (int e = 0; e < 8; ++e) { bsg[e] = 0.f; bsgy[e] = 0.f; bsc[e] = 1.f; bsh[e] = 0.f; }
    if (bnb && p.bnb_y && !p.bnb_bits && n0 + (tid % CG) * 8 < p.Nout) { load8f(p.bnb_scale + n0 + (tid % CG) * 8, bsc); load8f(p.bnb_shift + n0 + (tid % CG) * 8, bsh); }
    constexpr int ITER = BM * CG / NT;
    static_assert(BM * CG % NT == 0 && ITER >= 1, "whole store iterations");
    constexpr int CH = ITER < 2 ? ITER : 2;
    static_assert(ITER % CH == 0, "whole chunks");
    const int ecg = tid % CG, ecol = n0 + ecg * 8;
    for (int it0 = 0; it0 < ITER; it0 += CH) {
        EpiLoads L[CH];
        bool ok[CH], rok[CH];
        int mo[CH];
#pragma unroll
        for (int u = 0; u < CH; ++u) {
            const int idx = tid + (it0 + u) * NT;
            const int row = idx / CG, mr = m0 + row;
            ok[u] = mr < p.M && ecol < p.Nout;
            const int m = ok[u] ? (p.omap ? s_orow[row] : mr) : 0;
            mo[u] = m;
            rok[u] = ok[u] && p.resid && m >= p.resid_row0;
            if constexpr (F32R) {
                uint32_t srow;
                if (f32_row(p.f32, m, srow)) rok[u] = false;
            }
            L[u].rbits = 0xffu; L[u].bbits = 0u;
            if (rok[u]) {
                L[u].r = ld16(p.resid + (int64_t)m * p.ldr + ecol);
                if (p.resid_bits) L[u].rbits = p.resid_bits[(int64_t)m * (p.Nout >> 3) + (ecol >> 3)];
            }
            if (ok[u] && bnb && p.bnb_y) {
                L[u].y = ld16(p.bnb_y + (int64_t)m * p.bnb_ld + ecol);
                if (p.bnb_bits) L[u].bbits = p.bnb_bits[(int64_t)m * (p.Nout >> 3) + (ecol >> 3)];
            }
        }
#pragma unroll
        for (int u = 0; u < CH; ++u) {
            if (!ok[u]) continue;
            const int idx = tid + (it0 + u) * NT;
            const int row = idx / CG, m = mo[u];
            f16x8 v = ld16(stg + row * STG_LD + ecg * 8);
            if (rok[u]) {
#pragma unroll
                for (int e = 0; e < 8; ++e) {
                    const f16 r = ((L[u].rbits >> e) & 1u) ? L[u].r[e] : (f16)0.f;
                    v[e] = (f16)((float)v[e] + (float)r);
                }
            }
            if (p.act_mode == 2) {
                const f16x8 h = ld16(p.act_aux + (int64_t)m * p.ld_aux + ecol);
#pragma unroll
                for (int e = 0; e < 8; ++e) v[e] = (f16)((float)v[e] * gelu_df((float)h[e]));
            }
            if (p.act_mode == 3) {
#pragma unroll
                for (int e = 0; e < 8; ++e) v[e] = v[e] > (f16)0.f ? v[e] : (f16)0.f;
            }
            st16(p.y + (int64_t)m * p.ldy + ecol, v);
            if (p.act_mode == 1) {
                f16x8 a;
#pragma unroll
                for (int e = 0; e < 8; ++e) a[e] = (f16)gelu_f((float)v[e]);
                st16(p.act_aux + (int64_t)m * p.ld_aux + ecol, a);
            }
            if (bnb && p.bnb_y) bnb_accumulate(v, L[u].y, bsc, bsh, bsg, bsgy, p.bnb_bits != nullptr, L[u].bbits);
            else if (bnb) {
#pragma unroll
                for (int e = 0; e < 8; ++e) bsg[e] += (float)v[e];
            }
        }
    }
    if (bnb) bnb_reduce_store<NW, CG>(bsg, bsgy, reinterpret_cast<float*>(smem), p.bnb_part + (int64_t)mt * 2 * p.Nout, n0, p.Nout);
}

template <int BM, int BN, int WAVES_M, int WAVES_N, int BK, int NST, bool F32R = false>
__global__ __launch_bounds__(64 * WAVES_M * WAVES_N, (BK == 32 ? 2 : 1) * (WAVES_M * WAVES_N) / 4) void sf_igemm2_kernel(Igemm2Params p) {
    constexpr int NW = WAVES_M * WAVES_N, NT = 64 * NW;
    constexpr int WM = BM / WAVES_M, WN = BN / WAVES_N;
    constexpr int TM = WM / 16, TN = WN / 16;
    constexpr int KSL = BK / 8;
    constexpr int RPI = 64 / KSL;
    constexpr int NA = BM / RPI / NW;
    constexpr int NBI = BN / RPI;
    constexpr int NB = (NBI + NW - 1) / NW;
    static_assert(BM % (RPI * NW) == 0, "A tile: whole copy instructions per wave");
    static_assert(NBI % NW == 0 || NBI < NW, "B tile: uniform copy count per wave or one partial round");
    static_assert(BM % 128 == 0, "statistics are kept per 128 rows");
    constexpr int A_ELEMS = BM * BK, B_ELEMS = BN * BK, STAGE = A_ELEMS + B_ELEMS;
    constexpr int STG_LD = BN + 8;
    constexpr int SMEM_MAIN = NST * STAGE, SMEM_STG = BM * STG_LD;
    constexpr int SMEM = SMEM_MAIN > SMEM_STG ? SMEM_MAIN : SMEM_STG;
    constexpr int HALVES = BM / 128, WPH = WAVES_M / HALVES;
    static_assert(WAVES_M % HALVES == 0, "a wave row belongs to one 128-row group");

    __shared__ __attribute__((aligned(16))) unsigned char lds_raw[SMEM * 2 + WAVES_M * 2 * BN * 4 + BM * 4];
    f16* const smem = reinterpret_cast<f16*>(lds_raw);
    float (*const s_red)[2][BN] = reinterpret_cast<float (*)[2][BN]>(lds_raw + SMEM * 2);
    int* const s_orow = reinterpret_cast<int*>(lds_raw + SMEM * 2 + WAVES_M * 2 * BN * 4);

    const int tid = threadIdx.x;
    const int lane = tid & 63, wave = __builtin_amdgcn_readfirstlane(tid >> 6);
    const int wm = wave / WAVES_N, wn = wave % WAVES_N;
    const int tile = (int)xcd_remap(blockIdx.x, gridDim.x);
    const int nt = tile % p.ntiles_n, mt = tile / p.ntiles_n;
    const int m0 = mt * BM, n0 = nt * BN;

    const int lrow = lane / KSL;
    int kslot;
    if constexpr (BK == 64) kslot = (lane & 7) ^ (lrow & 7);
    else kslot = ((lane & 3) - 2 * ((lrow >> 2) & 3)) & 3;
    int64_t aoff[NA];
    uint32_t amask[NA];
#pragma unroll
    for (int j = 0; j < NA; ++j) {
        int m = m0 + (wave + NW * j) * RPI + lrow;
        if (m >= p.M) m = p.M - 1;
        uint32_t q, a, b, c, n;
        fd_divmod((uint32_t)m, p.fdrW, q, c);
        fd_divmod(q, p.fdrH, q, b);
        fd_divmod(q, p.fdrT, n, a);
        const int bt = (int)a * p.mulT + p.offT, bh = (int)b * p.mulH + p.offH, bw = (int)c * p.mulW + p.offW;
        aoff[j] = ((((int64_t)n * p.sT + bt) * p.sH + bh) * p.sW + bw) * (int64_t)p.ld + kslot * 8;
        uint32_t mk = 0;
        for (int t = 0; t < p.ntaps; ++t) {
            const int st = bt + p.dt[t], sh = bh + p.dh[t], sw = bw + p.dw[t];
            const bool ok = (unsigned)st < (unsigned)p.sT && (unsigned)sh < (unsigned)p.sH && (unsigned)sw < (unsigned)p.sW;
            mk |= (ok ? 1u : 0u) << t;
        }
        amask[j] = mk;
    }
    if (p.omap) {
        for (int r = tid; r < BM; r += NT) {
            int m = m0 + r;
            if (m >= p.M) m = p.M - 1;
            uint32_t q, a, b, c, n;
            fd_divmod((uint32_t)m, p.fdrW, q, c);
            fd_divmod(q, p.fdrH, q, b);
            fd_divmod(q, p.fdrT, n, a);
            s_orow[r] = (((int)n * p.oT + (int)a * p.omT + p.ooT) * p.oH + (int)b * p.omH + p.ooH) * p.oW + (int)c * p.omW + p.ooW;
        }
    }
    const f16* bptr[NB];
#pragma unroll
    for (int j = 0; j < NB; ++j) {
        int co = n0 + (wave + NW * j) * RPI + lrow;
        if (co >= p.Nout) co = p.Nout - 1;
        bptr[j] = p.wmat + (int64_t)co * p.ldw + kslot * 8;
    }
    const f16* const zline = reinterpret_cast<const f16*>(sf_zero_line);
    const int csteps = p.C / BK;
    const int ksteps = p.ntaps * csteps;

    auto issue = [&](int tap, int c0, int buf) {
        f16* As = smem + buf * STAGE;
        f16* Bs = As + A_ELEMS;
        const int64_t dsrc = (int64_t)p.taps[tap].dlin * p.ld + c0;
        const int wk = p.taps[tap].wcol + c0;
#pragma unroll
        for (int j = 0; j < NA; ++j) {
            const f16* g = ((amask[j] >> tap) & 1u) ? p.src + (aoff[j] + dsrc) : zline;
            SF_GLOBAL_LOAD_LDS16(g, As + (wave + NW * j) * 512);
        }
#pragma unroll
        for (int j = 0; j < NB; ++j)
            if (NBI % NW == 0 || wave + NW * j < NBI) SF_GLOBAL_LOAD_LDS16(bptr[j] + wk, Bs + (wave + NW * j) * 512);
    };

    f32x4 acc[TM][TN];
#pragma unroll
    for (int i = 0; i < TM; ++i)
#pragma unroll
        for (int j = 0; j < TN; ++j) acc[i][j] = (f32x4){0.f, 0.f, 0.f, 0.f};

    auto compute = [&](int buf) {
        const f16* As = smem + buf * STAGE;
        const f16* Bs = As + A_ELEMS;
#pragma unroll
        for (int kk = 0; kk < BK / 32; ++kk) {
            f16x8 af[TM], bf[TN];
#pragma unroll
            for (int i = 0; i < TM; ++i) af[i] = ld16(As + i2_lds_off<BK>(wm * WM + i * 16 + (lane & 15), kk * 4 + (lane >> 4)));
#pragma unroll
            for (int j = 0; j < TN; ++j) bf[j] = ld16(Bs + i2_lds_off<BK>(wn * WN + j * 16 + (lane & 15), kk * 4 + (lane >> 4)));
            if (SF_ABLATE(p) & 4) {
#pragma unroll
                for (int i = 0; i < TM; ++i) SF_KEEP_ALIVE(af[i]);
#pragma unroll
                for (int j = 0; j < TN; ++j) SF_KEEP_ALIVE(bf[j]);
                continue;
            }
#pragma unroll
            for (int i = 0; i < TM; ++i)
#pragma unroll
                for (int j = 0; j < TN; ++j)
                    acc[i][j] = SF_MFMA16(af[i], bf[j], acc[i][j]);
        }
    };

    {
        constexpr int COPIES = NA + (NBI % NW == 0 ? NB : NB - 1);
        int tap_i = 0, c_i = 0;
        auto advance = [&]() { if (++tap_i == p.ntaps) { tap_i = 0; c_i += BK; } };
        int issued = 0;
        for (; issued < NST - 1 && issued < ksteps; ++issued) { issue(tap_i, c_i, issued); advance(); }
        int cur = 0, nxt = NST - 1;
        for (int ks = 0; ks < ksteps; ++ks) {
            if constexpr (NST == 3) {
                if (ks + 1 < ksteps) SF_WAIT_VMEM_N(COPIES);
                else SF_WAIT_VMEM();
            } else {
                SF_WAIT_VMEM();
            }
            if (!(SF_ABLATE(p) & 16)) SF_BARRIER_KEEP_VMEM();
            if (issued < ksteps) { if (!(SF_ABLATE(p) & 1)) issue(tap_i, c_i, nxt); advance(); ++issued; }
            if (!(SF_ABLATE(p) & 2)) compute(cur);
            cur = cur == NST - 1 ? 0 : cur + 1;
            nxt = nxt == NST - 1 ? 0 : nxt + 1;
        }
        __syncthreads();
        if (SF_ABLATE(p) & 8) return;
    }

    i2_epilogue<BM, BN, WAVES_M, WAVES_N, F32R>(p, acc, smem, s_red, s_orow, mt, nt);
}
```

slowfast_amd/engine.py:

```python
import functools
import os

import torch

from . import lib as _sflib

from . import ops

_f16 = _sflib.act_dtype()
_listeners = []
FORCE_WEIGHT_PREP = False
PARAM_EPOCH = 0
PACK_RECORD = None
PACK_PLAN = os.environ.get("SF_PACK_PLAN", "1") != "0"
MATERIALIZE = os.environ.get("SF_MATERIALIZE", "1") != "0"
BN_FUSE_REDUCE = os.environ.get("SF_BN_FUSE_REDUCE", "1") != "0"
SEGMENTS = None


class _Segments:
    def __init__(self):
        self.cuts = []

    def cut(self, tensors):
        leaves = [t.detach().requires_grad_(True) if t.requires_grad else t for t in tensors]
        for l, t in zip(leaves, tensors):
            tag = getattr(t, "_sf_block_bn", None)
            if l is not t and tag is not None:
                l._sf_block_bn = tag
        if any(l is not t for l, t in zip(leaves, tensors)):
            self.cuts.append((list(tensors), leaves))
        return leaves


class WeightPackPlan:

    def __init__(self, record):
        from ctypes import byref, sizeof
        import numpy as np
        from .lib import PrepItem, get_lib
        lib = get_lib()
        seen, self.entries = set(), []
        for unit, geom, need_dgrad in record:
            k = (id(unit), None if geom is None else geom.Ci)
            if k in seen:
                continue
            seen.add(k)
            self.entries.append((unit, geom, need_dgrad))
        self.device = None
        items = (PrepItem * max(1, len(self.entries)))()
        blk_item, blk_off = [], []
        self._bufs, self._src = [], []
        for i, (unit, geom, need_dgrad) in enumerate(self.entries):
            w, desc, wf, wd = unit.pack_item(geom, need_dgrad)
            assert w.dtype == torch.float32 and w.is_contiguous()
            self.device = w.device
            lib.call("sf_prep_item_fill", byref(desc), w.data_ptr(), wf.data_ptr(), None if wd is None else wd.data_ptr(),
                     byref(items[i]))
            nb = lib.call("sf_prep_item_blocks", byref(items[i]))
            blk_item += [i] * nb
            blk_off += list(range(nb))
            self._bufs.append((wf, wd))
            self._src.append((w, w.data_ptr()))
        self.nblocks = len(blk_item)
        if self.entries:
            raw = np.frombuffer(bytes(items), dtype=np.uint8).copy()
            self.items = torch.from_numpy(raw).to(self.device)
            self.blk_item = torch.tensor(blk_item, dtype=torch.int32, device=self.device)
            self.blk_off = torch.tensor(blk_off, dtype=torch.int32, device=self.device)

    def __len__(self):
        return len(self.entries)

    def valid(self):
        return all(w.data_ptr() == ptr for w, ptr in self._src)

    def run(self):
        if not self.entries:
            return
        from .lib import get_lib
        stream = torch.cuda.current_stream(self.device).cuda_stream if self.device.type == "cuda" else None
        get_lib().call("sf_prep_weights_batch", self.items.data_ptr(), self.blk_item.data_ptr(), self.blk_off.data_ptr(),
                       self.nblocks, stream)
        for (unit, geom, _), (wf, wd) in zip(self.entries, self._bufs):
            unit.pack_assign(geom, wf, wd)

    def release(self):
        for unit, _, _ in self.entries:
            unit._planned = False


def cut(x):
    if SEGMENTS is None:
        return x
    if isinstance(x, (list, tuple)):
        return type(x)(SEGMENTS.cut(list(x)))
    return SEGMENTS.cut([x])[0]


WGRAD_STREAM = os.environ.get("SF_WGRAD_STREAM", "0") != "0"
_side_streams = {}
_side_keep = []
_side_pending = set()
_join_queued = False


def _fork_wgrad(device):
    global _join_queued
    side = _side_streams.get(device)
    if side is None:
        side = _side_streams[device] = torch.cuda.Stream(device=device)
    side.wait_stream(torch.cuda.current_stream(device))
    _side_pending.add(device)
    if not _join_queued:
        try:
            torch.autograd.Variable._execution_engine.queue_callback(join_side_streams)
            _join_queued = True
        except RuntimeError:
            pass
    return side


def join_side_streams():
    global _join_queued
    _join_queued = False
    for device in list(_side_pending):
        torch.cuda.current_stream(device).wait_stream(_side_streams[device])
    _side_pending.clear()
    _side_keep.clear()
    for device in {d for d, _ in _pathway_streams}:
        _join_pathways(device)


PATHWAY_STREAMS = os.environ.get("SF_PATHWAY_STREAMS", "1") != "0"
CAT_IN_PLACE = os.environ.get("SF_CAT_IN_PLACE", "1") != "0"
_pathway_streams = {}
_pathway_main = {}


def _pathway_stream(device, p):
    s = _pathway_streams.get((device, p))
    if s is None:
        s = _pathway_streams[(device, p)] = torch.cuda.Stream(device=device)
    return s


def run_pathways(n, fn, like):
    if not (PATHWAY_STREAMS and n > 1 and like.is_cuda):
        return [fn(p) for p in range(n)]
    dev = like.device
    main = torch.cuda.current_stream(dev)
    _pathway_main[dev] = main
    outs = [None] * n
    sides = []
    for p in range(1, n):
        side = _pathway_stream(dev, p)
        side.wait_stream(main)
        with torch.cuda.stream(side):
            outs[p] = fn(p)
        sides.append(side)
    outs[0] = fn(0)
    for side in sides:
        main.wait_stream(side)
    return outs


BRANCH_STREAMS = os.environ.get("SF_BRANCH_STREAMS", "1") != "0"


# ... 288 lines not shown
    def _fold_source(self, w):
        return w

    def fold(self):
        w = self.conv.weight.detach().float()
        b = self.conv.bias.detach().float() if self.conv.bias is not None else None
        bn = self.bn
        if bn is not None:
            assert bn.running_mean is not None, "BatchNorm without running statistics cannot be folded"
            scale = torch.rsqrt(bn.running_var.detach().float() + bn.eps)
            if bn.weight is not None:
                scale = scale * bn.weight.detach().float()
            shift = -bn.running_mean.detach().float() * scale
            if bn.bias is not None:
                shift = shift + bn.bias.detach().float()
            w = w * scale.view(-1, 1, 1, 1, 1)
            b = shift if b is None else b * scale + shift
        self._fold_w, self._fold_b, self._fold_packed = self._fold_source(w).contiguous(), b, {}

    def infer(self, x, relu=False, resid=None, out=None):
        geom = self.geom(x.shape)
        packed = self._fold_packed.get(geom.in_shape)
        if packed is None:
            wf, _ = ops.prep_weights(self._fold_w, geom, need_dgrad=False)
            b = self._fold_b
            if b is not None and b.numel() < geom.Co:
                b = torch.nn.functional.pad(b, (0, geom.Co - b.numel()))
            packed = self._fold_packed[geom.in_shape] = (wf, None if b is None else b.contiguous())
        return ops.conv_fwd_fused(x, packed[0], geom, bias=packed[1], resid=resid, relu=relu, out=out)


class StemConvUnit(ConvUnit):

    def __init__(self, conv, bn=None):
        super().__init__(conv, bn)
        kT, kH, kW = conv.kernel_size
        sT, sH, sW = conv.stride
        pT, pH, pW = conv.padding
        assert conv.in_channels <= 4 and sW % 2 == 0 and conv.dilation == (1, 1, 1)
        self.lead = pW % 2
        self.kext = kW + self.lead + ((kW + self.lead) % 2)
        self.k2 = (kT, kH, self.kext // 2)
        self.s2 = (sT, sH, sW // 2)
        self.p2 = (pT, pH, (pW + self.lead) // 2)

    def prepare_input(self, x):
        if getattr(x, "_sf_wpairs", False):
            return x
        return ops.ncthw_to_cl_wpairs(x.float())

    @staticmethod
    def prepare_shape(shape):
        N, C, T, H, W = shape
        return (N, 8, T, H, W // 2)

    def geom(self, in_shape):
        key = tuple(in_shape)
        g = self._geoms.get(key)
        if g is None:
            c = self.conv
            N, C2, T, H, W2 = key
            assert C2 == 8
            Wo = (2 * W2 + 2 * c.padding[2] - c.kernel_size[2]) // c.stride[2] + 1
            g = ops.ConvGeom(key, c.out_channels, self.k2, self.s2, self.p2, (1, 1, 1), Cw=8)
            g = ops.ConvGeom(key, c.out_channels, self.k2, self.s2, self.p2, (1, 1, 1), Cw=8,
                             out_dims=(g.To, g.Ho, Wo))
            self._geoms[key] = g
        return g

    def _virtual_weight(self, w):
        Co, Cin, kT, kH, kW = w.shape
        wv = torch.nn.functional.pad(w, (self.lead, self.kext - kW - self.lead, 0, 0, 0, 0, 0, 4 - Cin))
        wv = wv.view(Co, 4, kT, kH, self.kext // 2, 2).permute(0, 5, 1, 2, 3, 4)
        return wv.reshape(Co, 8, kT, kH, self.kext // 2).contiguous()

    def _fold_source(self, w):
        return self._virtual_weight(w)

    def weights(self, geom, fresh=False):
        w = self.conv.weight
        key = (w.data_ptr(), w._version, geom.Ci, w.device, PARAM_EPOCH)
        if (fresh and FORCE_WEIGHT_PREP) or self._wkey != key:
            self._w = ops.prep_weights(self._virtual_weight(w.detach()), geom, need_dgrad=False)
            self._wkey = key
        return self._w

    def backward(self, x, in_affine, dy, need_dx, resid=None):
        assert not need_dx, "the stems take the input clip: no data gradient"
        geom = self.geom(x.shape)
        w = self.conv.weight
        if w.requires_grad:
            Co, Cin, kT, kH, kW = w.shape
            dwv = torch.empty((Co, 8, kT, kH, self.kext // 2), dtype=torch.float32, device=w.device)
            ops.conv_wgrad(x, dy, geom, dwv, in_affine=in_affine, out_scale=1.0, zero_first=True)
            dw = dwv.view(Co, 2, 4, kT, kH, self.kext // 2).permute(0, 2, 3, 4, 5, 1).reshape(Co, 4, kT, kH, self.kext)
            dw = dw[:, :Cin, :, :, self.lead:self.lead + kW]
            dst, zero_first = _grad_dest(w)
            if zero_first:
                dst.copy_(dw)
            else:
                dst.add_(dw)
        return None


class StemFn(torch.autograd.Function):

    @staticmethod
    def forward(ctx, x, mod, *params):
        record_params(ctx, params)
        unit = mod._unit
        xcl = unit.prepare_input(x) if isinstance(unit, StemConvUnit) else ops.to_cl(x)
        y, st = unit.forward(xcl, None, mod.training)
        k, s, p = mod.pool_layer.kernel_size, mod.pool_layer.stride, mod.pool_layer.padding
        assert k[0] == 1 and s[0] == 1 and p[0] == 0, "stem pooling is spatial-only in every reference config"
        out, arg = ops.pool_fwd(y, k[1:], s[1:], p[1:], affine=(st.scale, st.shift, True))
        if CAPTURE is not None:
            CAPTURE.append({"kind": "stem", "mod": mod, "raw": [y], "bn": [(st.scale, st.shift)], "out": out,
                            "argmax": torch.where(arg == 255, torch.zeros_like(arg), arg)})
        ctx.mod, ctx.xcl, ctx.y, ctx.st = mod, xcl, y, st
        ctx.pool = (tuple(k[1:]), tuple(s[1:]), tuple(p[1:]))
        ctx.pooled, ctx.arg = out, arg
        return out

    @staticmethod
    @delivers_grads
    def backward(ctx, dout):
        unit = ctx.mod._unit
        st = ctx.st
        g = ops.pool_bwd(ctx.y.shape, ctx.pooled, ctx.arg, as_cl(dout), *ctx.pool, relu=True)
        dy = unit.bn_backward(g, ctx.y, st)
        unit.backward(ctx.xcl, None, dy, need_dx=False)
        _notify(unit.params())
        ctx.xcl = ctx.y = ctx.pooled = ctx.arg = None
        return (None, None) + param_grads(ctx, 2)


class FuseFn(torch.autograd.Function):

    @staticmethod
    def forward(ctx, x_s, x_f, mod, *params):
        record_params(ctx, params)
        unit = mod._unit
        x_s, x_f = as_cl(x_s), as_cl(x_f)
        yf, st = unit.forward(x_f, None, mod.training)
        N, Cs, T, H, W = x_s.shape
        Cf = yf.shape[1]
        assert tuple(yf.shape) == (N, Cf, T, H, W), "lateral connection does not match the Slow pathway shape"
        cat = getattr(x_s, "_sf_cat", None)
        if cat is not None and tuple(cat.shape) == (N, Cs + Cf, T, H, W) and cat.data_ptr() == x_s.data_ptr():
            pass
        else:
            cat = ops.cl_empty((N, Cs + Cf, T, H, W), x_s.device)
            ops.bn_act(x_s, out=cat[:, :Cs])
        ops.bn_act(yf, st.scale, st.shift, relu=True, out=cat[:, Cs:])
        if CAPTURE is not None:
            CAPTURE.append({"kind": "fuse", "mod": mod, "raw": [yf], "bn": [(st.scale, st.shift)]})
        ctx.mod, ctx.yf, ctx.st, ctx.Cs = mod, yf, st, Cs
        ctx.save_for_backward(x_f)
        return cat, x_f.view_as(x_f)

    @staticmethod
    @delivers_grads
    def backward(ctx, dcat, dxf):
        unit = ctx.mod._unit
        (x_f,) = ctx.saved_tensors
        dcat = as_cl(dcat)
        dyf = unit.bn_backward(dcat[:, ctx.Cs:], ctx.yf, ctx.st, relu_self=True)
        need_dx = ctx.needs_input_grad[1]
        dx_f = unit.backward(x_f, None, dyf, need_dx=need_dx, resid=as_cl(dxf) if dxf is not None else None)
        _notify(unit.params())
        ctx.yf = None
        dx_s = dcat[:, :ctx.Cs] if ctx.needs_input_grad[0] else None
        return (dx_s, dx_f, None) + param_grads(ctx, 3)


class ResBlockFn(torch.autograd.Function):

    @staticmethod
    def forward(ctx, x, mod, *params):
        record_params(ctx, params)
        ctx.prev_bn = getattr(x, "_sf_block_bn", None) if BN_FUSE_REDUCE else None
        x = as_cl(x)
        units, P = mod.branch2._chain, mod._proj
        tr = mod.training
        raw, bn, act = [], [], []
        h, prologue = x, None
        for i, u in enumerate(units):
            h, st = u.forward(h, prologue, tr)
            raw.append(h)
            bn.append(st)
            if MATERIALIZE and i + 1 < len(units):
                h = ops.bn_act(h, st.scale, st.shift, relu=True)
                act.append(h)
                prologue = None
            else:
                act.append(None)
                prologue = (st.scale, st.shift, True)
        yc, sc = raw[-1], bn[-1]
        out_view, cat = None, None
        extra = getattr(mod, "_cat_extra", 0)
        if extra and CAT_IN_PLACE:
            N_, C_, T_, H_, W_ = yc.shape
            cat = ops.cl_empty((N_, C_ + extra, T_, H_, W_), x.device)
            out_view = cat[:, :C_]
        if P is not None:
            y1, s1 = P.forward(x, None, tr)
            out, bits = ops.bn_act(yc, sc.scale, sc.shift, relu=True, resid=y1, rscale=s1.scale, rshift=s1.shift,
                                   want_mask=True, out=out_view)
        else:
            y1, s1 = None, None
            out, bits = ops.bn_act(yc, sc.scale, sc.shift, relu=True, resid=x, want_mask=True, out=out_view)
        if cat is not None:
            out._sf_cat = cat
        if CAPTURE is not None:
            CAPTURE.append({"kind": "resblock", "mod": mod, "raw": list(raw), "bn": [(b.scale, b.shift) for b in bn], "out": out})
        ctx.mod = mod
        ctx.raw = (raw, y1, act, bits)
        ctx.bn = (bn, s1)
        ctx.save_for_backward(x)
        if BN_FUSE_REDUCE and tr:
            out._sf_block_bn = {"bits": bits, "y0": yc, "sync": _sync_of(units[-1].bn) is not None}
        return out

    @staticmethod
    @delivers_grads
    def backward(ctx, dout):
        mod = ctx.mod
        units, P = mod.branch2._chain, mod._proj
        (x,) = ctx.saved_tensors
        raw, y1, act, bits = ctx.raw
        bn, s1 = ctx.bn
        last = len(units) - 1
        part_c = tagged_bn_part(dout, raw[last])
        dout = as_cl(dout)
        need_dx = ctx.needs_input_grad[0]
        dy = units[last].bn_backward(dout, raw[last], bn[last], zmask=bits, part=part_c)
        if P is not None:
            dy1 = P.bn_backward(dout, y1, s1, zmask=bits)
        for i in range(last, 0, -1):
            part = None
            if act[i - 1] is not None and BN_FUSE_REDUCE and _sync_of(units[i - 1].bn) is None:
                d_in, part = units[i].backward(act[i - 1], None, dy, need_dx=True, bn_fuse=(raw[i - 1], bn[i - 1]))
            elif act[i - 1] is not None:
                d_in = units[i].backward(act[i - 1], None, dy, need_dx=True)
            else:
                d_in = units[i].backward(raw[i - 1], (bn[i - 1].scale, bn[i - 1].shift, True), dy, need_dx=True)
            dy = units[i - 1].bn_backward(d_in, raw[i - 1], bn[i - 1], relu_self=True, part=part)
        prev = ctx.prev_bn if need_dx else None
        if prev is not None and prev["sync"]:
            prev = None
        if P is not None:
            dx1 = P.backward(x, None, dy1, need_dx=need_dx)
            dx = units[0].backward(x, None, dy, need_dx=need_dx, resid=dx1, bn_fuse=prev)
        else:
            dx = units[0].backward(x, None, dy, need_dx=need_dx, resid=dout, resid_bits=bits, bn_fuse=prev)
        if prev is not None:
            dx, pc = dx
            if pc is not None:
                tag_bn_part(dx, prev["y0"], pc)
        _notify(mod._param_list)
        ctx.raw = ctx.bn = ctx.prev_bn = None
        return (dx, None) + param_grads(ctx, 2)


CUT_BACKWARD = False
_cut_bn_tags = {}


def retag_cut_grad(g):
    tag = _cut_bn_tags.pop(g.data_ptr(), None)
    if tag is not None and getattr(g, "_sf_bn_part", None) is None and tag[2] == g.data_ptr() and tag[3] == g._version:
        g._sf_bn_part = tag


def tag_bn_part(dx, y0, part):
    dx._sf_bn_part = (y0.data_ptr(), part, dx.data_ptr(), dx._version)
    if CUT_BACKWARD:
        _cut_bn_tags[dx.data_ptr()] = dx._sf_bn_part


def tagged_bn_part(dout, y0):
    tag = getattr(dout, "_sf_bn_part", None)
    if tag is None or tag[0] != y0.data_ptr() or tag[2] != dout.data_ptr() or tag[3] != dout._version:
        return None
    return tag[1]


class ConvBNActFn(torch.autograd.Function):

    @staticmethod
    def forward(ctx, x, unit, relu, training, *params):
        record_params(ctx, params)
        x = as_cl(x)
        y, st = unit.forward(x, None, training)
        out = ops.bn_act(y, st.scale, st.shift, relu=relu)
        if CAPTURE is not None:
            CAPTURE.append({"kind": "convbnact", "mod": None, "raw": [y], "bn": [(st.scale, st.shift)], "out": out})
        ctx.unit, ctx.relu, ctx.y, ctx.st = unit, relu, y, st
        ctx.save_for_backward(x)
        return out

    @staticmethod
    @delivers_grads
    def backward(ctx, dout):
        unit = ctx.unit
        (x,) = ctx.saved_tensors
        dy = unit.bn_backward(as_cl(dout), ctx.y, ctx.st, relu_self=ctx.relu)
        dx = unit.backward(x, None, dy, need_dx=ctx.needs_input_grad[0])
        _notify(unit.params())
        ctx.y = None
        return (dx, None, None, None) + param_grads(ctx, 4)
```

slowfast_amd/lib.py:

```python
import ctypes
import os
from ctypes import POINTER, Structure, c_char_p, c_float, c_int, c_int32, c_int64, c_void_p

_HERE = os.path.dirname(os.path.abspath(__file__))
ABI_VERSION = 26
ACT_MODE = os.environ.get("SF_ACT_DTYPE", "fp16").lower()
if ACT_MODE not in ("fp16", "bf16"):
    raise ValueError(f"SF_ACT_DTYPE={ACT_MODE!r}: expected fp16 or bf16")
DEFAULT_LIBRARY = os.path.join(_HERE, "libsfamd.so" if ACT_MODE == "fp16" else "libsfamd_bf16.so")


def act_dtype():
    import torch
    return torch.float16 if ACT_MODE == "fp16" else torch.bfloat16


def act_eps():
    return 2.0 ** -11 if ACT_MODE == "fp16" else 2.0 ** -8


class ConvDesc(Structure):

    _fields_ = [(n, c_int32) for n in (
        "N", "Ci", "Ti", "Hi", "Wi", "Co", "To", "Ho", "Wo", "kT", "kH", "kW", "sT", "sH", "sW",
        "pT", "pH", "pW", "dT", "dH", "dW", "Cw", "ldx", "ldy", "Cow")]


class PrepItem(Structure):

    _fields_ = [("w", c_void_p), ("wf", c_void_p), ("wd", c_void_p)] + [(n, c_int32) for n in (
        "Co", "Cow", "Cw", "Cp", "taps", "ldf", "ldd", "pad")]


class DwDesc(Structure):

    _fields_ = [(n, c_int32) for n in (
        "N", "C", "Cw", "cls", "Ti", "Hi", "Wi", "To", "Ho", "Wo", "kT", "kH", "kW", "sT", "sH", "sW",
        "pT", "pH", "pW", "ldx", "ldy", "Cwreal")]


class Rows32(Structure):

    _fields_ = [("in_", c_void_p), ("out", c_void_p), ("ld", c_int32), ("period", c_int32)]


class ColFinItem(Structure):

    _fields_ = [("part", c_void_p), ("nblk", c_int32), ("C", c_int32), ("fold", c_int32), ("out0", c_void_p),
                ("out1", c_void_p), ("scale", c_float), ("accumulate", c_int32), ("row_stride", c_int32)]


class AttnDesc(Structure):

    _fields_ = [(n, c_int32) for n in (
        "B", "heads", "D", "cls", "Nq", "qT", "qH", "qW", "Nk", "kT", "kH", "kW", "rows_h", "rows_w", "rows_t")]


_P = c_void_p
_F = c_void_p
_SIGNATURES = {
    "sf_abi_version": (c_int, []),
    "sf_backend": (c_char_p, []),
    "sf_act_dtype": (c_int, []),
    "sf_last_error": (c_char_p, []),
    "sf_build_id": (c_char_p, []),
    "sf_conv_weight_ld": (c_int, [POINTER(ConvDesc), POINTER(c_int32), POINTER(c_int32)]),
    "sf_prep_weights": (c_int, [POINTER(ConvDesc), _F, _P, _P, _P]),
    "sf_prep_item_fill": (c_int, [POINTER(ConvDesc), _F, _P, _P, POINTER(PrepItem)]),
    "sf_prep_item_blocks": (c_int64, [POINTER(PrepItem)]),
    "sf_prep_weights_batch": (c_int, [_P, _P, _P, c_int32, _P]),
    "sf_conv_fwd_mtiles": (c_int, [POINTER(ConvDesc)]),
    "sf_conv_fwd": (c_int, [POINTER(ConvDesc), _P, _P, _F, _F, c_int, _F, _P, _F, _P]),
    "sf_conv_fwd_fused": (c_int, [POINTER(ConvDesc), _P, _P, _F, _P, c_int32, c_int, _P, _P]),
    "sf_conv_dgrad": (c_int, [POINTER(ConvDesc), _P, _P, _P, c_int32, _P, _P, _P]),
    "sf_conv_dgrad_bn": (c_int, [POINTER(ConvDesc), _P, _P, _P, c_int32, _P, _P, _P, _P, _P, _P, c_int32, _P, c_int32,
                                 POINTER(c_int32), _P]),
    "sf_conv_wgrad_workspace": (c_int64, [POINTER(ConvDesc)]),
    "sf_conv_wgrad_rowtab_bytes": (c_int64, [POINTER(ConvDesc)]),
    "sf_conv_wgrad_rowtab": (c_int, [POINTER(ConvDesc), _P, _P]),
    "sf_conv_wgrad": (c_int, [POINTER(ConvDesc), _P, _F, _F, c_int, _P, _F, c_float, c_int, _P, c_int64, _P, _P]),
    "sf_bn_finalize": (c_int, [_F, c_int32, c_int32, c_int32, c_float, _F, _F, _F, _F, c_float, c_float, _F, _F, _F, _F, _P]),
    "sf_bn_act": (c_int, [c_int64, c_int32, _P, c_int32, _F, _F, _P, c_int32, _F, _F, c_int, _P, c_int32, _P, _P]),
    "sf_bn_bwd_blocks": (c_int, [c_int64, c_int32]),
    "sf_flat_blocks": (c_int, [c_int64]),
    "sf_flat_sumsq": (c_int, [_F, c_int64, _F, _P]),
    "sf_step_control": (c_int, [_F, c_int32, _F, c_float, c_float, c_int, c_float, c_float, c_int32, _P]),
    "sf_flat_sgd": (c_int, [_F, _F, _F, _P, _P, _P, c_int32, _F, _P, _P, c_int32, c_float, c_float, c_float, c_int, _P]),
    "sf_flat_adamw": (c_int, [_F, _F, _F, _F, _P, _P, _P, c_int32, _F, _P, _P, c_int32, c_float, c_float, c_float, c_float, _P]),
    "sf_flat_sgd_tab": (c_int, [_F, _F, _F, _P, _P, _P, c_int32, _F, _F, _F, c_float, c_float, c_float, c_int, _P]),
    "sf_flat_adamw_tab": (c_int, [_F, _F, _F, _F, _P, _P, _P, c_int32, _F, _F, _F, c_float, c_float, c_float, c_float, _P]),
    "sf_flat_lars_trust": (c_int, [_F, _F, _P, _P, _P, c_int32, _P, c_int32, _F, _F, _P, _F, c_float, c_float, c_float, _P]),
    "sf_bn_bwd_reduce": (c_int, [c_int64, c_int32, _P, c_int32, _P, c_int32, _P, c_int32, _F, _F, c_int, _F, _P]),
    "sf_bn_bwd_finalize": (c_int, [_F, c_int32, c_int32, c_int32, c_float, _F, _F, _F, c_float, _F, _F, c_int, _F, _P]),
    "sf_bn_bwd_apply": (c_int, [c_int64, c_int32, _P, c_int32, _P, c_int32, _P, c_int32, _F, _F, c_int, _F, _P,
                                c_int32, _P, c_int32, _P]),
    "sf_pool_fwd": (c_int, [c_int32] * 11 + [_P, c_int32, _F, _F, c_int, _P, c_int32, _P, c_int32, _P]),
    "sf_pool_bwd": (c_int, [c_int32] * 11 + [_P, c_int32, _P, c_int, _P, c_int32, _P, c_int32, c_int32, _P]),
    "sf_pool3d_fwd": (c_int, [c_int32] * 8 + [_P, c_int32, _P, c_int32, _P, _P]),
    "sf_pool3d_bwd": (c_int, [c_int32] * 8 + [_P, _P, c_int32, _P, c_int32, _P]),
    "sf_ncthw_to_cl": (c_int, [_F, c_int32, c_int32, c_int64, c_int32, _P, _P]),
    "sf_cl_to_ncthw": (c_int, [_P, c_int32, c_int32, c_int32, c_int64, _F, _P]),
    "sf_bgemm": (c_int, [c_int64, c_int32, c_int32, _P, c_int32, _P, c_int32, _F, _P, c_int32, _P, c_int32, c_int32,
                         c_int32] + [c_int64] * 8 + [c_int32, c_float, _P]),
    "sf_bgemm_tn": (c_int, [c_int64, c_int32, c_int32, _P, c_int32, _P, c_int32, _P, c_int32, c_float, c_int32, c_int32]
                    + [c_int64] * 6 + [_P]),
    "sf_layernorm_fwd": (c_int, [c_int64, c_int32, _P, c_int32, _F, _F, c_float, _P, c_int32, _F, _F, _P]),
    "sf_gemm_rows32": (c_int, [c_int64, c_int32, c_int32, _P, c_int32, _P, c_int32, _F, _P, c_int32, _P, c_int32,
                               POINTER(Rows32), _P]),
    "sf_layernorm_fwd_rows32": (c_int, [c_int64, c_int32, _P, c_int32, _F, _F, c_float, _P, c_int32, _F, _F,
                                        POINTER(Rows32), _P]),
    "sf_layernorm_bwd_blocks": (c_int, [c_int64, c_int32]),
    "sf_layernorm_bwd": (c_int, [c_int64, c_int32, _P, c_int32, _P, c_int32, _F, _F, _F, _P, c_int32, _P, c_int32, _F, _P]),
    "sf_layernorm_bwd_sums": (c_int, [c_int64, c_int32, _P, c_int32, _P, c_int32, _F, _F, _F, _P, c_int32, _P, c_int32, _F, _P]),
    "sf_colsum_blocks": (c_int, [c_int64, c_int32]),
    "sf_colsum": (c_int, [c_int64, c_int32, _P, c_int32, _F, _P]),
    "sf_colsum_finalize": (c_int, [_F, c_int32, c_int32, c_int32, _F, _F, c_float, c_int, _P]),
    "sf_colsum_finalize_batch": (c_int, [POINTER(ColFinItem), c_int32, _P]),
    "sf_rows_sum": (c_int, [_F, c_int32, c_int64, c_int64, c_int32, _F, c_float, c_int, _P]),
    "sf_gelu_fwd": (c_int, [c_int64, _P, _P, _P]),
    "sf_gelu_bwd": (c_int, [c_int64, _P, _P, _P, _P]),
    "sf_dwconv_fwd_blocks": (c_int, [POINTER(DwDesc)]),
    "sf_dwconv_fwd_sample_rows": (c_int, [POINTER(DwDesc)]),
    "sf_dwconv_pair_ok": (c_int, [POINTER(DwDesc)]),
    "sf_dwconv_fwd_pair": (c_int, [POINTER(DwDesc), _P, _P, _F, _F, _P, _P, _P]),
    "sf_dwconv_dgrad_pair": (c_int, [POINTER(DwDesc), _P, _P, _F, _F, _P, _P, _P]),
    "sf_dwconv_wgrad_pair": (c_int, [POINTER(DwDesc), _P, _P, _P, _P, _F, _F, c_float, c_int, c_int, _P, c_int64, _P]),
    "sf_dwconv_fwd": (c_int, [POINTER(DwDesc), _P, _F, _P, _F, _P]),
    "sf_dwconv_dgrad": (c_int, [POINTER(DwDesc), _P, _F, _P, _P]),
    "sf_dwconv_dgrad_sum_rows": (c_int, [POINTER(DwDesc)]),
    "sf_dwconv_dgrad_sums": (c_int, [POINTER(DwDesc), _P, _F, _P, _F, _P]),
    "sf_dwconv_wgrad_workspace": (c_int64, [POINTER(DwDesc)]),
    "sf_dwconv_wgrad": (c_int, [POINTER(DwDesc), _P, _P, _F, c_float, c_int, _P, c_int64, _P]),
    "sf_relpos_gather": (c_int, [POINTER(AttnDesc), _P, c_int32, _P, _P, _P, _F, _P]),
    "sf_relpos_scatter": (c_int, [POINTER(AttnDesc), _F, _P, _P, _P, _P, c_int32, _P]),
    "sf_relpos_pack": (c_int, [_F, _F, _F, c_int32, c_int32, c_int32, c_int32, c_int32, _P, _P, _P]),
    "sf_relpos_unpack": (c_int, [_F, c_int32, c_int32, c_int32, c_int32, _F, _F, _F, c_int32, c_int32, c_int32, _P]),
    "sf_softmax_fwd": (c_int, [POINTER(AttnDesc), _P, c_int32, c_float, _F, _P]),
    "sf_softmax_bwd": (c_int, [POINTER(AttnDesc), _P, _P, c_int32, c_float, _F, _P]),
    "sf_attn_fwd": (c_int, [POINTER(AttnDesc), _P, c_int32, _P, _P, c_int32, c_float, _F, _P, c_int32, _P, c_int32, _F, _P]),
    "sf_attn_bwd_workspace": (c_int64, [POINTER(AttnDesc)]),
    "sf_attn_bwd": (c_int, [POINTER(AttnDesc), _P, c_int32, _P, _P, c_int32, c_float, _F, _P, c_int32, _P, _P, c_int32, _F,
                            _F, _P, c_int32, _P, _P, c_int32, _F, _P, c_int64, _P]),
    "sf_tmean_fwd": (c_int, [c_int32, c_int32, c_int64, c_int32, _P, c_int32, _F, _P]),
    "sf_tmean_bwd": (c_int, [c_int32, c_int32, c_int64, c_int32, _F, _P, c_int32, _P]),
    "sf_roi_align_max_fwd": (c_int, [c_int32, c_int32, c_int32, c_int32, c_int32, c_int32, c_float, c_int32, _F, _F, _F,
                                     c_int32, c_int32, _P, _P]),
    "sf_roi_align_max_bwd": (c_int, [c_int32, c_int32, c_int32, c_int32, c_int32, c_int32, c_float, c_int32, _F, _F,
                                     c_int32, c_int32, _P, _F, _P]),
    "sf_gemm_act": (c_int, [c_int64, c_int32, c_int32, _P, c_int32, _P, c_int32, _F, _P, c_int32, c_int32, _P, c_int32, _P]),
    "sf_gemm_act_colsum": (c_int, [c_int64, c_int32, c_int32, _P, c_int32, _P, c_int32, _F, _P, c_int32, c_int32, _P, c_int32, _P, c_int32, POINTER(c_int32), _P]),
    "sf_pack_clip_u8": (c_int, [_P, c_int32, c_int32, c_int32, c_int32, _P, c_int32, c_float, c_float, c_float, c_float,
                                c_float, c_float, c_int32, _P, _P]),
    "sf_mix_clip_f32": (c_int, [_F, _F, c_int32, c_int32, c_int32, c_int32, c_int32, c_int32, c_float, c_float, c_int32, c_int32,
                                c_int32, c_int32, _P]),
    "sf_pack_clip_u8_mix": (c_int, [_P, c_int32, c_int32, c_int32, c_int32, _P, c_int32, c_float, c_float, c_float, c_float,
                                    c_float, c_float, c_int32, _P, c_int32, c_float, c_float, c_int32, c_int32, c_int32, c_int32,
                                    _P]),
    "sf_mix_targets": (c_int, [_P, c_int32, c_int32, c_float, c_float, c_float, c_float, _F, _P]),
    "sf_erase_clip_f32": (c_int, [_F, _F, c_int32, c_int32, c_int32, c_int32, c_int32, c_int32, _P, _P, c_int32, c_int32, _P]),
    "sf_pack_clip_u8_aug": (c_int, [_P, c_int32, c_int32, c_int32, c_int32, _P, c_int32, c_float, c_float, c_float, c_float,
                                    c_float, c_float, c_int32, _P, c_int32, _P, _P, c_int32, c_int32, c_int32, c_float, c_float,
                                    c_int32, c_int32, c_int32, c_int32, _P]),
    "sf_row_scale_add": (c_int, [_P, c_int32, _P, c_int64, _P, c_int32, _P, c_int32, c_int64, c_int32, _P]),
    "sf_row_scale_add_rows32": (c_int, [_P, c_int32, _P, c_int64, _P, c_int32, _P, c_int32, c_int64, c_int32,
                                        POINTER(Rows32), _P]),
    "sf_transpose_heads": (c_int, [_P, c_int32, _P, c_int32, c_int32, c_int32, c_int32, c_int32, _P]),
    "sf_sample_chunks": (c_int, [c_int64, c_int32]),
    "sf_sample_mean": (c_int, [c_int32, c_int64, c_int32, _P, c_int32, _F, _F, c_int, _F, _F, _P]),
    "sf_se_gate_fwd": (c_int, [c_int32, c_int32, c_int32, c_int32, _F, _F, _F, _F, _F, _F, _F, _P]),
    "sf_gate_act_fwd": (c_int, [c_int32, c_int64, c_int32, _P, c_int32, _F, _F, _F, c_int, _P, c_int32, _P]),
    "sf_gate_grad": (c_int, [c_int32, c_int64, c_int32, _P, c_int32, _F, _F, _P, c_int32, _F, c_int, _F, _F, _P]),
    "sf_se_gate_bwd": (c_int, [c_int32, c_int32, c_int32, c_int32, _F, _F, _F, _F, _F, _F, _F, _F, _P]),
    "sf_outer_sum": (c_int, [_F, c_int32, _F, c_int32, c_int32, c_int32, c_int32, _F, c_float, c_int, _P]),
    "sf_gate_act_bwd": (c_int, [c_int32, c_int64, c_int32, _P, c_int32, _F, _F, _F, c_int, _P, c_int32, _F, _P, c_int32, _P]),
    "sf_gate_bwd_sums": (c_int, [c_int32, c_int64, c_int32, _P, c_int32, _F, _F, _P, c_int32, _F, c_int, _P, c_int32, _F, _F, _P]),
    "sf_bn_bwd_apply_sample": (c_int, [c_int64, c_int32, _P, c_int32, _P, c_int32, _F, _F, c_int64, _P, c_int32, _P]),
    "sf_gate_act_bwd_bn_rows": (c_int, [c_int32, c_int64, c_int32]),
    "sf_gate_act_bwd_bn": (c_int, [c_int32, c_int64, c_int32, _P, c_int32, _F, _F, _F, c_int, _P, c_int32, _F, _P, c_int32, _F, _P]),
}
EXPORTED_SYMBOLS = tuple(_SIGNATURES)


class SfError(RuntimeError):
    pass


class SfLibrary:
    def __init__(self, path):
        if not os.path.exists(path):
            raise SfError(
                f"native library not found: {path}. Build it with `python -m slowfast_amd.build_ext` "
                "(hipcc --offload-arch=gfx950); slowfast_amd has no CPU/PyTorch fallback.")
        self.path = path
        self.cdll = ctypes.CDLL(path)
        for name, (res, args) in _SIGNATURES.items():
            fn = getattr(self.cdll, name)
            fn.restype = res
            fn.argtypes = args
        ver = self.cdll.sf_abi_version()
        if ver != ABI_VERSION:
            raise SfError(f"{path}: ABI version {ver}, expected {ABI_VERSION}")
        self.backend = self.cdll.sf_backend().decode()
        self.build_id = self.cdll.sf_build_id().decode()
        from . import build_ext
        if build_ext.sources_present():
            want = build_ext.source_id(sim=self.backend == "hostsim")
            if self.build_id != want and os.environ.get("SF_ALLOW_STALE_LIBRARY", "0") == "0":
                raise SfError(f"{path} was built from other sources (build id {self.build_id}, sources {want}): rebuild with "
                              "`python -m slowfast_amd.build_ext` (SF_ALLOW_STALE_LIBRARY=1 overrides)")
        else:
            import warnings
            warnings.warn(f"{path}: kernel sources not found beside the package, build id {self.build_id} not verified")
        self.act_mode = ("fp16", "bf16")[self.cdll.sf_act_dtype()]
        if self.act_mode != ACT_MODE:
            raise SfError(f"{path} is the {self.act_mode} build of the library, this process runs with SF_ACT_DTYPE={ACT_MODE}")

    def call(self, name, *args, work=None):
        fn = getattr(self.cdll, name)
        if _observer is not None:
            rc = _observer(name, lambda: fn(*args), work)
        else:
            rc = fn(*args)
        if rc < 0:
            raise SfError(f"{name}: {self.cdll.sf_last_error().decode()}")
        return rc


_lib = None
_observer = None
# ... 18 lines not shown
```

slowfast_amd/ops.py:

```python
from ctypes import byref, c_int32

import torch

from . import lib as _sflib

from .lib import ConvDesc, SfError, get_lib

_f16 = _sflib.act_dtype()


def _triple(v):
    return tuple(v) if isinstance(v, (tuple, list)) else (v, v, v)


def _stream(t):
    if t.is_cuda:
        return torch.cuda.current_stream(t.device).cuda_stream
    if get_lib().backend != "hostsim":
        raise SfError("slowfast_amd kernels need CUDA/HIP tensors (got a CPU tensor and the gfx950 library)")
    return None


def _ptr(t):
    return None if t is None else t.data_ptr()


def cl_empty(shape, device, ld=None, zero=False):
    N, C, T, H, W = shape
    ld = C if ld is None else ld
    base = (torch.zeros if zero else torch.empty)((N, T, H, W, ld), dtype=_f16, device=device)
    return base[..., :C].permute(0, 4, 1, 2, 3)


def cl_ld(x):
    if x.dim() != 5 or x.dtype != _f16:
        raise SfError(f"expected a 5-D fp16 channels-last activation, got {tuple(x.shape)} {x.dtype}")
    N, C, T, H, W = x.shape
    if C > 1 and x.stride(1) != 1:
        raise SfError("activation is not channels-last (channel stride != 1); use ops.to_cl()")
    if W > 1:
        ld = x.stride(4)
    elif H > 1:
        ld = x.stride(3)
    elif T > 1:
        ld = x.stride(2)
    elif N > 1:
        ld = x.stride(0)
    else:
        ld = C
    exp = (T * H * W * ld, 1, H * W * ld, W * ld, ld)
    for dim, size in enumerate(x.shape):
        if size > 1 and x.stride(dim) != exp[dim]:
            raise SfError(f"activation strides {x.stride()} are not channels-last with pitch {ld}")
    if ld < C or ld % 8 or C % 8 or x.data_ptr() % 16:
        raise SfError(f"activation needs C % 8 == 0, pitch % 8 == 0, 16-byte base (C={C}, ld={ld})")
    return ld


def is_cl(x):
    try:
        cl_ld(x)
        return True
    except SfError:
        return False


def rows(x):
    N, C, T, H, W = x.shape
    return N * T * H * W


def ncthw_to_cl(x, Cp=None):
    assert x.dim() == 5 and x.dtype == torch.float32
    x = x.contiguous()
    N, C, T, H, W = x.shape
    Cp = Cp or (C + 7) // 8 * 8
    out = cl_empty((N, Cp, T, H, W), x.device)
    get_lib().call("sf_ncthw_to_cl", x.data_ptr(), N, C, T * H * W, Cp, out.data_ptr(), _stream(x),
                   work=dict(bytes=4.0 * x.numel() + 2.0 * out.numel()))
    return out


def ncthw_to_cl_wpairs(x):
    assert x.dim() == 5 and x.dtype == torch.float32 and x.shape[1] <= 4 and x.shape[4] % 2 == 0
    x = x.contiguous()
    N, C, T, H, W = x.shape
    base = torch.empty((N, T, H, W // 2, 8), dtype=_f16, device=x.device)
    get_lib().call("sf_ncthw_to_cl", x.data_ptr(), N, C, T * H * W, 4, base.data_ptr(), _stream(x),
                   work=dict(bytes=4.0 * x.numel() + 2.0 * base.numel()))
    return base.permute(0, 4, 1, 2, 3)


def cl_to_ncthw(x):
    ld = cl_ld(x)
    N, C, T, H, W = x.shape
    out = torch.empty((N, C, T, H, W), dtype=torch.float32, device=x.device)
    get_lib().call("sf_cl_to_ncthw", x.data_ptr(), ld, N, C, T * H * W, out.data_ptr(), _stream(x))
    return out


def to_cl(x):
    if x.dtype == _f16 and is_cl(x):
        return x
    return ncthw_to_cl(x.float())


class ConvGeom:

    def __init__(self, in_shape, Co, kernel, stride=1, padding=0, dilation=1, Cw=None, out_dims=None):
        self.N, self.Ci, self.Ti, self.Hi, self.Wi = in_shape
        self.Cow = Co
        self.Co = (Co + 7) // 8 * 8
        self.k, self.s, self.p, self.d = _triple(kernel), _triple(stride), _triple(padding), _triple(dilation)
        self.Cw = self.Ci if Cw is None else Cw
        self.To, self.Ho, self.Wo = [
            (i + 2 * p - d * (k - 1) - 1) // s + 1
            for i, k, s, p, d in zip((self.Ti, self.Hi, self.Wi), self.k, self.s, self.p, self.d)]
        if out_dims is not None:
            assert all(1 <= o <= f for o, f in zip(out_dims, (self.To, self.Ho, self.Wo)))
            self.To, self.Ho, self.Wo = out_dims
        self.taps = self.k[0] * self.k[1] * self.k[2]
        ldf, ldd = c_int32(), c_int32()
        get_lib().call("sf_conv_weight_ld", byref(self.desc(self.Ci, self.Co)), byref(ldf), byref(ldd))
        self.ldf, self.ldd = ldf.value, ldd.value
        self.ws_bytes = None

    @property
    def in_shape(self):
        return (self.N, self.Ci, self.Ti, self.Hi, self.Wi)

    @property
    def out_shape(self):
        return (self.N, self.Co, self.To, self.Ho, self.Wo)

    @property
    def out_rows(self):
        return self.N * self.To * self.Ho * self.Wo

    def work(self, reads_x=0, reads_y=0, writes_x=0, writes_y=0):
        xe = self.N * self.Cw * self.Ti * self.Hi * self.Wi
        ye = self.out_rows * self.Co
        return dict(flops=2.0 * self.out_rows * self.Co * self.Cw * self.taps,
                    bytes=2.0 * ((reads_x + writes_x) * xe + (reads_y + writes_y) * ye))

    def desc(self, ldx, ldy):
        return ConvDesc(self.N, self.Ci, self.Ti, self.Hi, self.Wi, self.Co, self.To, self.Ho, self.Wo,
                        *self.k, *self.s, *self.p, *self.d, self.Cw, ldx, ldy, self.Cow)


def prep_weights(w, geom, need_dgrad=True):
    assert w.dtype == torch.float32 and tuple(w.shape) == (geom.Cow, geom.Cw) + geom.k, (w.shape, geom.Cow, geom.Cw)
    w = w.contiguous()
    wf = torch.empty((geom.Co, geom.ldf), dtype=_f16, device=w.device)
    wd = torch.empty((geom.Ci, geom.ldd), dtype=_f16, device=w.device) if need_dgrad else None
    get_lib().call("sf_prep_weights", byref(geom.desc(geom.Ci, geom.Co)), w.data_ptr(), wf.data_ptr(), _ptr(wd),
                   _stream(w))
    return wf, wd


def _affine(in_affine):
    if in_affine is None:
        return None, None, 0
    scale, shift, relu = in_affine
    assert scale.dtype == torch.float32 and shift.dtype == torch.float32
    return scale, shift, int(bool(relu))


def conv_fwd(x, wf, geom, in_affine=None, bias=None, stats=True, out=None):
    assert tuple(x.shape) == geom.in_shape, (x.shape, geom.in_shape)
    ldx = cl_ld(x)
    y = cl_empty(geom.out_shape, x.device) if out is None else out
    ldy = cl_ld(y)
    lib = get_lib()
    d = geom.desc(ldx, ldy)
    part = None
    if stats:
        mt = lib.call("sf_conv_fwd_mtiles", byref(d))
        part = torch.empty((mt, 2, geom.Co), dtype=torch.float32, device=x.device)
    sc, sh, relu = _affine(in_affine)
    lib.call("sf_conv_fwd", byref(d), x.data_ptr(), wf.data_ptr(), _ptr(sc), _ptr(sh), relu, _ptr(bias),
             y.data_ptr(), _ptr(part), _stream(x), work=geom.work(reads_x=1, reads_y=0, writes_y=1))
    return y, part


def conv_fwd_fused(x, wf, geom, bias=None, resid=None, relu=False, out=None):
    assert tuple(x.shape) == geom.in_shape, (x.shape, geom.in_shape)
    y = cl_empty(geom.out_shape, x.device) if out is None else out
    assert tuple(y.shape) == geom.out_shape
    if bias is not None:
        assert bias.dtype == torch.float32 and bias.numel() == geom.Co, "bias must cover the padded channel count"
    ldr = 0
    if resid is not None:
        assert tuple(resid.shape) == geom.out_shape
        ldr = cl_ld(resid)
    get_lib().call("sf_conv_fwd_fused", byref(geom.desc(cl_ld(x), cl_ld(y))), x.data_ptr(), wf.data_ptr(), _ptr(bias),
                   _ptr(resid), ldr, int(bool(relu)), y.data_ptr(), _stream(x),
                   work=geom.work(reads_x=1, reads_y=int(resid is not None), writes_y=1))
    return y


def conv_dgrad(dy, wd, geom, resid=None, out=None, resid_bits=None, bn=None):
    assert tuple(dy.shape) == geom.out_shape
    if resid is not None:
        assert tuple(resid.shape) == geom.in_shape
    if out is not None:
        assert tuple(out.shape) == geom.in_shape
    if bn is not None:
        if not isinstance(bn, dict):
            y0, sc, sh = bn
            bits = None
        else:
            bits, y0 = bn["bits"], bn["y0"]
            sc = sh = None
            assert bits.dtype == torch.uint8 and bits.numel() == rows(y0) * (geom.Ci // 8) and bits.is_contiguous()
        assert tuple(y0.shape) == geom.in_shape
        dx = cl_empty(geom.in_shape, dy.device) if out is None else out
        M = rows(y0)
        cap = (M + 127) // 128
        part = torch.empty((cap, 2, geom.Ci), dtype=torch.float32, device=dy.device)
        nrows = c_int32(0)
        if resid_bits is not None:
            assert resid is not None and resid_bits.dtype == torch.uint8 and resid_bits.numel() == rows(resid) * (geom.Ci // 8)
        get_lib().call("sf_conv_dgrad_bn", byref(geom.desc(cl_ld(dx), cl_ld(dy))), dy.data_ptr(), wd.data_ptr(), _ptr(resid),
                       cl_ld(resid) if resid is not None else 0, _ptr(resid_bits), dx.data_ptr(), _ptr(sc), _ptr(sh), _ptr(bits),
                       y0.data_ptr(), cl_ld(y0), part.data_ptr(), cap, byref(nrows), _stream(dy),
                       work=geom.work(reads_x=1 + int(resid is not None), reads_y=1, writes_x=1))
        return dx, (part[:nrows.value] if nrows.value > 0 else None)
    ldy = cl_ld(dy)
    dx = cl_empty(geom.in_shape, dy.device) if out is None else out
    ldx = cl_ld(dx)
    ldr = cl_ld(resid) if resid is not None else 0
    if resid_bits is not None:
        assert resid is not None and resid_bits.dtype == torch.uint8 and resid_bits.numel() == rows(resid) * (geom.Ci // 8)
    get_lib().call("sf_conv_dgrad", byref(geom.desc(ldx, ldy)), dy.data_ptr(), wd.data_ptr(), _ptr(resid), ldr,
                   _ptr(resid_bits), dx.data_ptr(), _stream(dy),
                   work=geom.work(reads_x=int(resid is not None), reads_y=1, writes_x=1))
    return dx


_workspaces = {}
_retired_workspaces = []


def _workspace(device, nbytes, key=None):
    sid = torch.cuda.current_stream(device).cuda_stream if device.type == "cuda" else 0
    k = (device, key, sid)
    ws = _workspaces.get(k)
    if ws is None or ws.numel() < nbytes:
        if ws is not None:
            _retired_workspaces.append(ws)
        ws = torch.empty(max(int(nbytes * 1.25), 1 << 20), dtype=torch.uint8, device=device)
        _workspaces[k] = ws
    return ws


def conv_wgrad(x, dy, geom, dw, in_affine=None, out_scale=1.0, zero_first=True, side=False):
    assert tuple(x.shape) == geom.in_shape and tuple(dy.shape) == geom.out_shape
    assert dw.dtype == torch.float32 and dw.is_contiguous() and dw.numel() == geom.Cow * geom.Cw * geom.taps
    sc, sh, relu = _affine(in_affine)
    lib = get_lib()
    d = geom.desc(cl_ld(x), cl_ld(dy))
    if geom.ws_bytes is None:
        geom.ws_bytes = lib.call("sf_conv_wgrad_workspace", byref(d))
    ws = _workspace(x.device, geom.ws_bytes, "wgrad-side" if side else None)
    lib.call("sf_conv_wgrad", byref(d), x.data_ptr(), _ptr(sc), _ptr(sh), relu,
                   dy.data_ptr(), dw.data_ptr(), float(out_scale), int(zero_first), ws.data_ptr(), ws.numel(),
                   _ptr(_wgrad_rowtab(geom, d, x.device)) if sc is None else None, _stream(x),
                   work=geom.work(reads_x=1, reads_y=1))
    return dw


_rowtabs = {}


def _capturing(device):
    return device.type == "cuda" and torch.cuda.is_current_stream_capturing()


def _wgrad_rowtab(geom, d, device):
    nbytes = getattr(geom, "_rowtab_bytes", None)
    if nbytes is None:
        nbytes = geom._rowtab_bytes = get_lib().call("sf_conv_wgrad_rowtab_bytes", byref(d))
    if nbytes <= 0:
        return None
    key = (device, 0, geom.N, geom.Ti, geom.Hi, geom.Wi, geom.To, geom.Ho, geom.Wo, geom.k, geom.s, geom.p, geom.d)
    if key not in _rowtabs:
        tab = torch.empty(nbytes, dtype=torch.uint8, device=device)
        get_lib().call("sf_conv_wgrad_rowtab", byref(d), tab.data_ptr(), _stream(tab))
        if _capturing(device):
            return tab
        if device.type == "cuda":
            torch.cuda.current_stream(device).synchronize()
        _rowtabs[key] = tab
    return _rowtabs[key]


def bn_finalize(part, count, gamma, beta, running_mean, running_var, momentum, eps, training=True, C=None):
    Creal = gamma.numel()
    C = C or (part.shape[2] if part is not None else Creal)
    dev = gamma.device
    scale, shift, mean, rstd = (torch.empty(C, dtype=torch.float32, device=dev) for _ in range(4))
    nblk = part.shape[0] if training else 0
    get_lib().call("sf_bn_finalize", _ptr(part) if training else None, nblk, C, Creal, float(count), gamma.data_ptr(),
                   beta.data_ptr(), _ptr(running_mean), _ptr(running_var), float(momentum), float(eps),
                   scale.data_ptr(), shift.data_ptr(), mean.data_ptr(), rstd.data_ptr(), _stream(gamma))
    return scale, shift, mean, rstd


def bn_act(y, scale=None, shift=None, relu=False, resid=None, rscale=None, rshift=None, out=None, want_mask=False):
    ldy = cl_ld(y)
    N, C, T, H, W = y.shape
    out = cl_empty(y.shape, y.device) if out is None else out
    assert tuple(out.shape) == tuple(y.shape)
    mask = torch.empty((rows(y), C // 8), dtype=torch.uint8, device=y.device) if want_mask else None
    get_lib().call("sf_bn_act", rows(y), C, y.data_ptr(), ldy, _ptr(scale), _ptr(shift), _ptr(resid),
                   cl_ld(resid) if resid is not None else 0, _ptr(rscale), _ptr(rshift), int(bool(relu)),
                   out.data_ptr(), cl_ld(out), _ptr(mask), _stream(y),
                   work=dict(bytes=2.0 * y.numel() * (2 + int(resid is not None) + (1 / 16 if want_mask else 0))))
    return (out, mask) if want_mask else out


def bn_bwd(dz, y, gamma, mean, rstd, dgamma, dbeta, zmask=None, relu_affine=None, inv_loss_scale=1.0,
           accumulate=False, want_g=False, out=None, sync=None, part=None, sample_add=None):
    lib = get_lib()
    N, C, T, H, W = y.shape
    M = rows(y)
    s = _stream(y)
    fused_part = part
    if fused_part is None:
        nblk = lib.call("sf_bn_bwd_blocks", M, C)
        part = torch.empty((nblk, 2, C), dtype=torch.float32, device=y.device)
    else:
        assert part.dtype == torch.float32 and part.is_contiguous() and tuple(part.shape[1:]) == (2, C)
        nblk = part.shape[0]
    sc, sh = (relu_affine if relu_affine is not None else (None, None))
    relu_self = int(relu_affine is not None)
    bits = zmask is not None and zmask.dtype == torch.uint8
    if bits:
        assert zmask.numel() == M * (C // 8) and zmask.is_contiguous()
    mcost = 0.0 if zmask is None else (1 / 16 if bits else 1.0)
    lddz, ldy, ldm = cl_ld(dz), cl_ld(y), (0 if bits or zmask is None else cl_ld(zmask))
    if fused_part is None:
        lib.call("sf_bn_bwd_reduce", M, C, dz.data_ptr(), lddz, _ptr(zmask), ldm, y.data_ptr(), ldy, _ptr(sc), _ptr(sh),
                 relu_self, part.data_ptr(), s, work=dict(bytes=2.0 * y.numel() * (2 + mcost)))
    coef = torch.empty((3, C), dtype=torch.float32, device=y.device)
    if sync is None:
        lib.call("sf_bn_bwd_finalize", part.data_ptr(), nblk, C, gamma.numel(), float(M), gamma.data_ptr(), mean.data_ptr(),
                 rstd.data_ptr(), float(inv_loss_scale), dgamma.data_ptr(), dbeta.data_ptr(), int(accumulate),
                 coef.data_ptr(), s)
    else:
        import torch.distributed as dist
        group, gsize = sync
        tot = part.sum(0, keepdim=True)
        loc = tot.clone()
        lib.call("sf_bn_bwd_finalize", loc.data_ptr(), 1, C, gamma.numel(), float(M), gamma.data_ptr(), mean.data_ptr(),
                 rstd.data_ptr(), float(inv_loss_scale), dgamma.data_ptr(), dbeta.data_ptr(), int(accumulate),
                 coef.data_ptr(), s)
        dist.all_reduce(tot, group=group)
        scratch = torch.empty((2, gamma.numel()), dtype=torch.float32, device=y.device)
        lib.call("sf_bn_bwd_finalize", tot.data_ptr(), 1, C, gamma.numel(), float(M) * gsize, gamma.data_ptr(),
                 mean.data_ptr(), rstd.data_ptr(), float(inv_loss_scale), scratch[0].data_ptr(), scratch[1].data_ptr(), 0,
                 coef.data_ptr(), s)
    dy = cl_empty(y.shape, y.device) if out is None else out
    if sample_add is not None:
        assert fused_part is not None and zmask is None and relu_affine is None and not want_g
        assert sample_add.dtype == torch.float32 and sample_add.is_contiguous() and tuple(sample_add.shape) == (N, C)
        lib.call("sf_bn_bwd_apply_sample", M, C, dz.data_ptr(), lddz, y.data_ptr(), ldy, coef.data_ptr(), sample_add.data_ptr(),
                 M // N, dy.data_ptr(), cl_ld(dy), s, work=dict(bytes=2.0 * y.numel() * 3))
        return dy
    g = cl_empty(y.shape, y.device) if want_g else None
    lib.call("sf_bn_bwd_apply", M, C, dz.data_ptr(), lddz, _ptr(zmask), ldm, y.data_ptr(), ldy, _ptr(sc), _ptr(sh),
             relu_self, coef.data_ptr(), dy.data_ptr(), cl_ld(dy), _ptr(g), cl_ld(g) if g is not None else 0, s,
             work=dict(bytes=2.0 * y.numel() * (3 + mcost + int(want_g))))
    return (dy, g) if want_g else dy


def _pool_args(y, kernel, stride, padding):
    N, C, T, H, W = y.shape
    (kH, kW), (sH, sW), (pH, pW) = kernel, stride, padding
    return (N, T, H, W, C, kH, kW, sH, sW, pH, pW), ((H + 2 * pH - kH) // sH + 1, (W + 2 * pW - kW) // sW + 1)


def pool_fwd(y, kernel, stride, padding, affine=None, want_argmax=True):
    args, (Ho, Wo) = _pool_args(y, kernel, stride, padding)
    N, C, T, H, W = y.shape
    out = cl_empty((N, C, T, Ho, Wo), y.device)
    arg = torch.empty((N, T, Ho, Wo, C), dtype=torch.uint8, device=y.device) if want_argmax else None
    sc, sh, relu = _affine(affine)
    get_lib().call("sf_pool_fwd", *args, y.data_ptr(), cl_ld(y), _ptr(sc), _ptr(sh), relu, out.data_ptr(),
                   cl_ld(out), _ptr(arg), 0, _stream(y), work=dict(bytes=2.0 * (y.numel() + out.numel())))
# ... 13 lines not shown
```

Before: 865.7 clips/s.

## Fuse dual BN-backward reductions into dgrad epilogue for projection and fusion branches

Adds a dgrad variant whose epilogue accumulates BN-backward partial sums for up to two BN sets, either two BNs sharing one window and mask (main path plus projection shortcut) or two disjoint channel windows (slow/fast concat). It removes the separate reduction passes over dy and y that the projection BN and the fast-branch BN backward used to need. The Python side threads the second partial table through tagged slots, including across cut-backward boundaries. In exchange it adds register pressure and extra loads in the store epilogue, a new kernel template instantiation, and more complex tag bookkeeping.

Result: no change. 874.3 clips/s (median of 6 runs) (+1.0%).

```diff
diff --git a/include/sfamd.h b/include/sfamd.h
--- a/include/sfamd.h
+++ b/include/sfamd.h
@@ -6,7 +6,7 @@
 extern "C" {
 #endif
 
-#define SF_ABI_VERSION 26
+#define SF_ABI_VERSION 27
 typedef void* sf_stream_t;
 
 typedef struct sf_conv_desc {
@@ -53,6 +53,17 @@
                      const void* resid_bits, void* dx, const float* mask_scale, const float* mask_shift,
                      const void* mask_bits, const void* bn_y, int32_t bn_ldy, float* bn_part, int32_t bn_part_rows,
                      int32_t* bn_rows, sf_stream_t stream);
+typedef struct sf_bn_set {
+    const void* y; int32_t ldy;
+    const void* bits; int32_t ld_bits;
+    const float* scale; const float* shift;
+    int32_t c0, c1;
+    float* part;
+    int32_t rows;
+} sf_bn_set;
+int sf_conv_dgrad_bn2(const sf_conv_desc* d, const void* dy, const void* wd, const void* resid, int32_t ldr,
+                      const void* resid_bits, void* dx, sf_bn_set* sets, int32_t nsets, int32_t bn_part_rows,
+                      sf_stream_t stream);
 int64_t sf_conv_wgrad_workspace(const sf_conv_desc* d);
 int64_t sf_conv_wgrad_rowtab_bytes(const sf_conv_desc* d);
 int sf_conv_wgrad_rowtab(const sf_conv_desc* d, void* tab, sf_stream_t stream);
diff --git a/slowfast_amd/csrc/sf_api.hip b/slowfast_amd/csrc/sf_api.hip
--- a/slowfast_amd/csrc/sf_api.hip
+++ b/slowfast_amd/csrc/sf_api.hip
@@ -146,6 +146,14 @@
     int mt = cdiv(p.M, 128);
     dim3 grid((unsigned)(mt * p.ntiles_n), (unsigned)nbatch);
     static const bool occ4 = tune_knob("SF_IGEMM_OCC4", 1) != 0;
+    if constexpr (BN >= 32) {
+        if (p.bnb2_n) {
+            if (igemm_glds_ok(p, pw)) hipLaunchKernelGGL((sf_igemm_kernel<BN, WM, WN, true, true, BN == 128, false, true>), grid, dim3(SF_THREADS), 0, s, p);
+            else if (pw) hipLaunchKernelGGL((sf_igemm_kernel<BN, WM, WN, true, false, BN == 128, false, true>), grid, dim3(SF_THREADS), 0, s, p);
+            else hipLaunchKernelGGL((sf_igemm_kernel<BN, WM, WN, false, false, BN == 128, false, true>), grid, dim3(SF_THREADS), 0, s, p);
+            return;
+        }
+    }
     if (p.f32.out) {
         if (igemm_glds_ok(p, pw)) hipLaunchKernelGGL((sf_igemm_kernel<BN, WM, WN, true, true, BN == 128, true>), grid, dim3(SF_THREADS), 0, s, p);
         else hipLaunchKernelGGL((sf_igemm_kernel<BN, WM, WN, true, false, BN == 128, true>), grid, dim3(SF_THREADS), 0, s, p);
@@ -170,6 +178,9 @@
 static void launch_igemm2(Igemm2Params& q, hipStream_t s) {
     q.ntiles_n = cdiv(q.Nout, BN);
     const dim3 grid((unsigned)(cdiv(q.M, 256) * q.ntiles_n));
+    if constexpr (BN == 128) {
+        if (q.bnb2_n) { hipLaunchKernelGGL((sf_igemm2_kernel<256, BN, 4, 2, BK, 3, false, true>), grid, dim3(512), 0, s, q); return; }
+    }
     if constexpr (BN >= 64) {
         if (q.f32.out) { hipLaunchKernelGGL((sf_igemm2_kernel<256, BN, 4, 2, BK, 3, true>), grid, dim3(512), 0, s, q); return; }
     }
@@ -217,10 +228,11 @@
     q.resid_bits = p.resid_bits;
     q.bnb_y = p.bnb_y; q.bnb_ld = p.bnb_ld; q.bnb_scale = p.bnb_scale; q.bnb_shift = p.bnb_shift; q.bnb_part = p.bnb_part;
     q.bnb_bits = p.bnb_bits;
+    q.bnb2[0] = p.bnb2[0]; q.bnb2[1] = p.bnb2[1]; q.bnb2_n = p.bnb2_n; q.bnb2_dual = p.bnb2_dual;
     q.f32 = p.f32;
     q.linear = p.linear;
 }
-static bool try_igemm2(const IgemmParams& p, hipStream_t s, int nbatch = 1) {
+static bool igemm2_eligible(const IgemmParams& p, int nbatch) {
     const char* e;
     const bool off = test_hook("SF_IGEMM2", 1) == 0;
     const int mink = test_hook("SF_IGEMM2_MINK", 512);
@@ -229,6 +241,11 @@
     if (off || !igemm2_operands_ok(p, nbatch)) return false;
     if (g.Ktot < mink || p.Nout <= 32 || p.M < minrows) return false;
     if (g.mode == 1 && !(g.strT == 1 && g.strH == 1 && g.strW == 1)) return false;
+    return true;
+}
+static bool try_igemm2(const IgemmParams& p, hipStream_t s, int nbatch = 1) {
+    if (!igemm2_eligible(p, nbatch)) return false;
+    const GatherSide& g = p.g;
     const int taps = g.kT * g.kH * g.kW;
     Igemm2Params q;
     igemm2_common(q, p);
@@ -316,7 +333,21 @@
     return true;
 }
 
-static int run_igemm(IgemmParams& p, bool pw, hipStream_t s, int* bm_used = nullptr) {
+static int bnb2_to_one_set(IgemmParams& p) {
+    const BnbSet A = p.bnb2[0];
+    const int n = p.bnb2_n;
+    memset(p.bnb2, 0, sizeof(p.bnb2));
+    p.bnb2_n = p.bnb2_dual = 0;
+    if (n < 1 || A.c0 != 0 || A.c1 != p.Nout || (A.bits && A.ldb != p.Nout / 8)) return 0;
+    p.bnb_y = A.y; p.bnb_ld = A.ld; p.bnb_scale = A.scale; p.bnb_shift = A.shift; p.bnb_bits = A.bits; p.bnb_part = A.part;
+    return 1;
+}
+static int run_igemm(IgemmParams& p, bool pw, hipStream_t s, int* bm_used = nullptr, int* bn2_used = nullptr) {
+    if (p.bnb2_n) {
+        const bool ok2 = igemm2_eligible(p, 1) ? p.Nout > 64 : p.Nout > 16;
+        const int used = ok2 ? 2 : bnb2_to_one_set(p);
+        if (bn2_used) *bn2_used = used;
+    }
     if (bm_used) *bm_used = 256;
     if (try_igemm2(p, s)) return check_launch("igemm2");
     if (bm_used) *bm_used = 0;
@@ -538,7 +569,14 @@
 struct BnFuse {
     const float* scale; const float* shift; const void* bits;
     const void* y0; int32_t ld0; float* part0;
+    sf_bn_set* sets; int32_t nsets;
 };
+static BnbSet bnb_set_of(const sf_bn_set& t) {
+    BnbSet b;
+    b.y = (const f16*)t.y; b.bits = (const uint8_t*)t.bits; b.scale = t.scale; b.shift = t.shift; b.part = t.part;
+    b.ld = t.ldy; b.ldb = t.ld_bits; b.c0 = t.c0; b.c1 = t.c1;
+    return b;
+}
 static int conv_dgrad_impl(const sf_conv_desc* d, const void* dy, const void* wd, const void* resid, int32_t ldr,
                            const void* resid_bits, void* dx, const BnFuse* bn, int32_t* bn_rows, sf_stream_t stream) {
     if (check_desc(d)) return -1;
@@ -557,34 +595,46 @@
     REQUIRE(!resid_bits || resid, "sf_conv_dgrad: resid_bits without a residual");
     p.resid_bits = (const uint8_t*)resid_bits;
     const bool fuse = bn && d->sT == 1 && d->sH == 1 && d->sW == 1;
+    const bool fuse2 = fuse && bn->sets;
+    if (bn && bn->sets)
+        for (int i = 0; i < bn->nsets; ++i) bn->sets[i].rows = 0;
+    if (fuse2) {
+        p.bnb2_n = bn->nsets;
+        for (int i = 0; i < bn->nsets; ++i) p.bnb2[i] = bnb_set_of(bn->sets[i]);
+        p.bnb2_dual = bn->nsets == 2 && p.bnb2[0].c0 == p.bnb2[1].c0 && p.bnb2[0].c1 == p.bnb2[1].c1;
+    }
     if (!resid && d->Co == 8 && d->To == d->Ti && d->Ho == d->Hi && d->Wo == d->Wi) {
         sf_conv_desc dd = *d;
         dd.Ci = d->Co; dd.Cw = d->Co; dd.Co = d->Ci; dd.Cow = 0;
         dd.pT = d->kT - 1 - d->pT; dd.pH = d->kH - 1 - d->pH; dd.pW = d->kW - 1 - d->pW;
         dd.ldx = d->ldy; dd.ldy = d->ldx;
         const StemPlan sp = plan_stem(&dd);
-        if (sp.ok && sp.thin3 && (!fuse || sp.ntiles <= cdiv(p.M, 128))) {
+        const bool fuse_t = fuse && !fuse2;
+        if (sp.ok && sp.thin3 && (!fuse_t || sp.ntiles <= cdiv(p.M, 128))) {
             StemParams q = stem_params(&dd, sp, dy);
             const int S = d->kT * d->kH;
             q.wmat = (const f16*)wd; q.ldw = ldd; q.y = (f16*)dx;
             q.wo0 = ((S - 1) * 3 + 2) * 8; q.wos = -24; q.wog = -8; q.kwc = 3;
-            if (fuse) {
+            if (fuse_t) {
                 q.bnb_y = (const f16*)bn->y0; q.bnb_ld = bn->ld0; q.bnb_scale = bn->scale; q.bnb_shift = bn->shift;
                 q.bnb_bits = (const uint8_t*)bn->bits;
                 q.stat_part = bn->part0; q.stat_rows = 0;
             }
             SF_STEM_FWD_LAUNCH(sp, q, stream);
-            if (bn_rows) *bn_rows = fuse ? sp.ntiles : 0;
+            if (bn_rows) *bn_rows = fuse_t ? sp.ntiles : 0;
             return check_launch("stem_dgrad");
         }
     }
-    if (fuse) {
+    if (fuse && !fuse2) {
         p.bnb_y = (const f16*)bn->y0; p.bnb_ld = bn->ld0; p.bnb_part = bn->part0;
         p.bnb_scale = bn->scale; p.bnb_shift = bn->shift; p.bnb_bits = (const uint8_t*)bn->bits;
     }
-    int bm = 0;
-    const int rc = run_igemm(p, is_pointwise(d), (hipStream_t)stream, &bm);
-    if (bn_rows) *bn_rows = (fuse && bm > 0) ? cdiv(p.M, bm) : 0;
+    int bm = 0, used2 = 0;
+    const int rc = run_igemm(p, is_pointwise(d), (hipStream_t)stream, &bm, &used2);
+    const int rows = (fuse && bm > 0) ? cdiv(p.M, bm) : 0;
+    if (fuse2) {
+        for (int i = 0; i < bn->nsets && i < used2; ++i) bn->sets[i].rows = rows;
+    } else if (bn_rows) *bn_rows = rows;
     return rc;
 }
 
@@ -602,8 +652,36 @@
     REQUIRE(bn_ldy >= d->Ci && bn_ldy % 8 == 0 && ((uintptr_t)bn_y & 15) == 0, "sf_conv_dgrad_bn: bad bn_y pitch / alignment");
     REQUIRE((int64_t)bn_part_rows * 128 >= (int64_t)d->N * d->Ti * d->Hi * d->Wi,
             "sf_conv_dgrad_bn: the partial table needs ceil(positions / 128) rows of [2][Ci] floats");
-    const BnFuse bn = {mask_scale, mask_shift, mask_bits, bn_y, bn_ldy, bn_part};
+    const BnFuse bn = {mask_scale, mask_shift, mask_bits, bn_y, bn_ldy, bn_part, nullptr, 0};
     return conv_dgrad_impl(d, dy, wd, resid, ldr, resid_bits, dx, &bn, bn_rows, stream);
+}
+
+extern "C" int sf_conv_dgrad_bn2(const sf_conv_desc* d, const void* dy, const void* wd, const void* resid, int32_t ldr,
+                                 const void* resid_bits, void* dx, sf_bn_set* sets, int32_t nsets, int32_t bn_part_rows,
+                                 sf_stream_t stream) {
+    REQUIRE(d && sets && (nsets == 1 || nsets == 2), "sf_conv_dgrad_bn2: one or two sets");
+    REQUIRE((int64_t)bn_part_rows * 128 >= (int64_t)d->N * d->Ti * d->Hi * d->Wi,
+            "sf_conv_dgrad_bn2: the partial tables need ceil(positions / 128) rows of [2][c1 - c0] floats");
+    for (int i = 0; i < nsets; ++i) {
+        const sf_bn_set& t = sets[i];
+        REQUIRE(t.y && t.part, "sf_conv_dgrad_bn2: null pointer in set %d", i);
+        REQUIRE(t.c0 >= 0 && t.c0 < t.c1 && t.c1 <= d->Ci && t.c0 % 8 == 0 && t.c1 % 8 == 0,
+                "sf_conv_dgrad_bn2: set %d: window [%d, %d) must be multiples of 8 inside [0, %d)", i, t.c0, t.c1, d->Ci);
+        REQUIRE(t.ldy >= t.c1 - t.c0 && t.ldy % 8 == 0 && ((uintptr_t)t.y & 15) == 0, "sf_conv_dgrad_bn2: set %d: bad y pitch / alignment", i);
+        REQUIRE(t.bits ? t.ld_bits >= (t.c1 - t.c0) / 8 : (t.scale && t.shift),
+                "sf_conv_dgrad_bn2: set %d needs a mask source (bits with its pitch, or scale + shift)", i);
+    }
+    if (nsets == 2) {
+        const sf_bn_set &a = sets[0], &b = sets[1];
+        const bool same = a.c0 == b.c0 && a.c1 == b.c1, disjoint = a.c1 <= b.c0 || b.c1 <= a.c0;
+        REQUIRE(same || disjoint, "sf_conv_dgrad_bn2: the windows must be identical or disjoint");
+        REQUIRE(!same || (a.bits && a.bits == b.bits && a.ld_bits == b.ld_bits),
+                "sf_conv_dgrad_bn2: sets over the same window share one bit mask");
+    }
+    BnFuse bn;
+    memset(&bn, 0, sizeof(bn));
+    bn.sets = sets; bn.nsets = nsets;
+    return conv_dgrad_impl(d, dy, wd, resid, ldr, resid_bits, dx, &bn, nullptr, stream);
 }
 
 template <int BMW, int WM, int WN, int KS>
diff --git a/slowfast_amd/csrc/sf_igemm.h b/slowfast_amd/csrc/sf_igemm.h
--- a/slowfast_amd/csrc/sf_igemm.h
+++ b/slowfast_amd/csrc/sf_igemm.h
@@ -1,5 +1,13 @@
 #pragma once
 #include "sf_common.h"
+
+struct BnbSet {
+    const f16* y;
+    const uint8_t* bits;
+    const float* scale; const float* shift;
+    float* part;
+    int ld, ldb, c0, c1;
+};
 
 struct IgemmParams {
     GatherSide g;
@@ -29,6 +37,8 @@
     const uint8_t* bnb_bits;
     F32Rows f32;
     int linear;
+    BnbSet bnb2[2];
+    int bnb2_n, bnb2_dual;
 };
 
 __device__ __forceinline__ void bnb_accumulate(const f16x8& dz, const f16x8& yv, const float (&sc)[8], const float (&sh)[8],
@@ -86,7 +96,125 @@
     }
 }
 
-template <int BN, int WM, int WN, bool PW, bool GL = false, bool OCC4 = false, bool F32R = false>
+template <int NT, int NW, int BM, int BN, int CH>
+__device__ __forceinline__ void bnb2_store_tile(const BnbSet& A, const BnbSet& B, const bool dual, const f16* stg, f16* yout, int ldy,
+                                                const f16* resid, int ldr, const uint8_t* resid_bits, int M, int Nout, int m0, int n0,
+                                                int mt, float* red) {
+    constexpr int CG = BN / 8, STG_LD = BN + 8, ITER = BM * CG / NT;
+    static_assert(BM * CG % NT == 0 && ITER >= 1 && ITER % CH == 0, "whole store iterations / chunks");
+    static_assert(NT % CG == 0 && 64 % CG == 0, "a thread keeps one column group over the whole store loop");
+    const int tid = threadIdx.x, lane = tid & 63, wave = tid >> 6;
+    const int ecg = tid % CG, ecol = n0 + ecg * 8;
+    const bool inA = ecol >= A.c0 && ecol < A.c1, inB = ecol >= B.c0 && ecol < B.c1;
+    const bool act = inA || inB;
+    const int pc = ecol - (inA ? A.c0 : B.c0);
+    const f16* const py = (inA ? A.y : B.y) + pc;
+    const int pld = inA ? A.ld : B.ld;
+    const uint8_t* pb = inA ? A.bits : B.bits;
+    const int pldb = inA ? A.ldb : B.ldb;
+    const bool use_bits = act && pb != nullptr;
+    if (use_bits) pb += pc >> 3;
+    const bool two = dual && inA && inB;
+    const f16* const py2 = B.y + (ecol - B.c0);
+    float sg[8], sgy[8], sgy2[8], sc[8], sh[8];
+#pragma unroll
+    for (int e = 0; e < 8; ++e) { sg[e] = 0.f; sgy[e] = 0.f; sgy2[e] = 0.f; sc[e] = 1.f; sh[e] = 0.f; }
+    if (act && !use_bits) { load8f((inA ? A.scale : B.scale) + pc, sc); load8f((inA ? A.shift : B.shift) + pc, sh); }
+    for (int it0 = 0; it0 < ITER; it0 += CH) {
+        EpiLoads L[CH];
+        f16x8 y2[CH];
+        bool ok[CH], rok[CH];
+#pragma unroll
+        for (int u = 0; u < CH; ++u) {
+            const int idx = tid + (it0 + u) * NT;
+            const int m = m0 + idx / CG;
+            ok[u] = m < M && ecol < Nout;
+            rok[u] = ok[u] && resid;
+            L[u].rbits = 0xffu; L[u].bbits = 0u;
+            if (rok[u]) {
+                L[u].r = ld16(resid + (int64_t)m * ldr + ecol);
+                if (resid_bits) L[u].rbits = resid_bits[(int64_t)m * (Nout >> 3) + (ecol >> 3)];
+            }
+            if (ok[u] && act) {
+                L[u].y = ld16(py + (int64_t)m * pld);
+                if (use_bits) L[u].bbits = pb[(int64_t)m * pldb];
+                if (two) y2[u] = ld16(py2 + (int64_t)m * B.ld);
+            }
+        }
+#pragma unroll
+        for (int u = 0; u < CH; ++u) {
+            if (!ok[u]) continue;
+            const int idx = tid + (it0 + u) * NT;
+            const int row = idx / CG, m = m0 + row;
+            f16x8 v = ld16(stg + row * STG_LD + ecg * 8);
+            if (rok[u]) {
+#pragma unroll
+                for (int e = 0; e < 8; ++e) {
+                    const f16 r = ((L[u].rbits >> e) & 1u) ? L[u].r[e] : (f16)0.f;
+                    v[e] = (f16)((float)v[e] + (float)r);
+                }
+            }
+            st16(yout + (int64_t)m * ldy + ecol, v);
+            if (act) {
+#pragma unroll
+                for (int e = 0; e < 8; ++e) {
+                    const bool open = use_bits ? ((L[u].bbits >> e) & 1u) != 0u : ((float)L[u].y[e] * sc[e] + sh[e] > 0.f);
+                    const float g = open ? (float)v[e] : 0.f;
+                    sg[e] += g;
+                    sgy[e] += g * (float)L[u].y[e];
+                    if (two) sgy2[e] += g * (float)y2[u][e];
+                }
+            }
+        }
+    }
+    const bool tileA = n0 < A.c1 && n0 + BN > A.c0, tileB = n0 < B.c1 && n0 + BN > B.c0;
+    if (!tileA && !tileB) return;
+#pragma unroll
+    for (int e = 0; e < 8; ++e)
+        for (int mask = CG; mask < 64; mask <<= 1) {
+            sg[e] += __shfl_xor(sg[e], mask);
+            sgy[e] += __shfl_xor(sgy[e], mask);
+            if (dual) sgy2[e] += __shfl_xor(sgy2[e], mask);
+        }
+    __syncthreads();
+    if (lane < CG) {
+#pragma unroll
+        for (int e = 0; e < 8; ++e) {
+            red[(wave * CG + lane) * 24 + e] = sg[e];
+            red[(wave * CG + lane) * 24 + 8 + e] = sgy[e];
+            red[(wave * CG + lane) * 24 + 16 + e] = sgy2[e];
+        }
+    }
+    __syncthreads();
+    if (tid < CG * 8) {
+        const int cgi = tid >> 3, e = tid & 7;
+        const int col = n0 + cgi * 8 + e;
+        const bool cA = col >= A.c0 && col < A.c1, cB = col >= B.c0 && col < B.c1;
+        if (cA || cB) {
+            float s = 0.f, q = 0.f, q2 = 0.f;
+#pragma unroll
+            for (int w = 0; w < NW; ++w) {
+                s += red[(w * CG + cgi) * 24 + e];
+                q += red[(w * CG + cgi) * 24 + 8 + e];
+                q2 += red[(w * CG + cgi) * 24 + 16 + e];
+            }
+            if (cA) {
+                const int W = A.c1 - A.c0;
+                float* prow = A.part + (int64_t)mt * 2 * W;
+                prow[col - A.c0] = s;
+                prow[W + col - A.c0] = q;
+            }
+            if (cB) {
+                const int W = B.c1 - B.c0;
+                float* prow = B.part + (int64_t)mt * 2 * W;
+                prow[col - B.c0] = s;
+                prow[W + col - B.c0] = cA ? q2 : q;
+            }
+        }
+    }
+}
+
+template <int BN, int WM, int WN, bool PW, bool GL = false, bool OCC4 = false, bool F32R = false, bool BN2 = false>
 __global__ __launch_bounds__(SF_THREADS, OCC4 ? 4 : 1) void sf_igemm_kernel(IgemmParams p) {
     constexpr int BM = 128, BK = 32;
     constexpr int NST = 2;
@@ -323,6 +451,11 @@
             p.stat_part[((int64_t)mt * 2 + 0) * p.Nout + col] = s;
             p.stat_part[((int64_t)mt * 2 + 1) * p.Nout + col] = q;
         }
+    }
+    if constexpr (BN2) {
+        bnb2_store_tile<SF_THREADS, 4, BM, BN, (BN >= 128 && OCC4) ? 2 : 1>(p.bnb2[0], p.bnb2[1], p.bnb2_dual != 0, stg, yout, p.ldy, resid, p.ldr, p.resid_bits,
+                                                  p.M, p.Nout, m0, n0, mt, reinterpret_cast<float*>(smem));
+        return;
     }
     constexpr int CG = BN / 8;
     static_assert(SF_THREADS % CG == 0 && 64 % CG == 0, "a thread keeps one column group over the whole store loop");
diff --git a/slowfast_amd/csrc/sf_igemm2.h b/slowfast_amd/csrc/sf_igemm2.h
--- a/slowfast_amd/csrc/sf_igemm2.h
+++ b/slowfast_amd/csrc/sf_igemm2.h
@@ -44,6 +44,8 @@
     int ablate;
     F32Rows f32;
     int linear;
+    BnbSet bnb2[2];
+    int bnb2_n, bnb2_dual;
 };
 
 template <int BK>
@@ -52,7 +54,7 @@
     else return lds_tile_off(row, kslot);
 }
 
-template <int BM, int BN, int WAVES_M, int WAVES_N, bool F32R>
+template <int BM, int BN, int WAVES_M, int WAVES_N, bool F32R, bool BN2 = false>
 __device__ __forceinline__ void i2_epilogue(const Igemm2Params& p, f32x4 (&acc)[BM / WAVES_M / 16][BN / WAVES_N / 16], f16* smem,
                                             float (*s_red)[2][BN], int* s_orow, int mt, int nt) {
     constexpr int NW = WAVES_M * WAVES_N, NT = 64 * NW;
@@ -127,6 +129,11 @@
             p.stat_part[((int64_t)prow * 2 + 1) * p.Nout + col] = q;
         }
     }
+    if constexpr (BN2) {
+        bnb2_store_tile<NT, NW, BM, BN, 2>(p.bnb2[0], p.bnb2[1], p.bnb2_dual != 0, stg, p.y, p.ldy, p.resid, p.ldr, p.resid_bits, p.M,
+                                           p.Nout, m0, n0, mt, reinterpret_cast<float*>(smem));
+        return;
+    }
     constexpr int CG = BN / 8;
     static_assert(NT % CG == 0 && 64 % CG == 0, "a thread keeps one column group over the whole store loop");
     const bool bnb = p.bnb_part != nullptr;
@@ -204,7 +211,7 @@
     if (bnb) bnb_reduce_store<NW, CG>(bsg, bsgy, reinterpret_cast<float*>(smem), p.bnb_part + (int64_t)mt * 2 * p.Nout, n0, p.Nout);
 }
 
-template <int BM, int BN, int WAVES_M, int WAVES_N, int BK, int NST, bool F32R = false>
+template <int BM, int BN, int WAVES_M, int WAVES_N, int BK, int NST, bool F32R = false, bool BN2 = false>
 __global__ __launch_bounds__(64 * WAVES_M * WAVES_N, (BK == 32 ? 2 : 1) * (WAVES_M * WAVES_N) / 4) void sf_igemm2_kernel(Igemm2Params p) {
     constexpr int NW = WAVES_M * WAVES_N, NT = 64 * NW;
     constexpr int WM = BM / WAVES_M, WN = BN / WAVES_N;
@@ -352,5 +359,5 @@
         if (SF_ABLATE(p) & 8) return;
     }
 
-    i2_epilogue<BM, BN, WAVES_M, WAVES_N, F32R>(p, acc, smem, s_red, s_orow, mt, nt);
+    i2_epilogue<BM, BN, WAVES_M, WAVES_N, F32R, BN2>(p, acc, smem, s_red, s_orow, mt, nt);
 }
diff --git a/slowfast_amd/engine.py b/slowfast_amd/engine.py
--- a/slowfast_amd/engine.py
+++ b/slowfast_amd/engine.py
@@ -15,6 +15,8 @@
 PACK_PLAN = os.environ.get("SF_PACK_PLAN", "1") != "0"
 MATERIALIZE = os.environ.get("SF_MATERIALIZE", "1") != "0"
 BN_FUSE_REDUCE = os.environ.get("SF_BN_FUSE_REDUCE", "1") != "0"
+BN_FUSE_PROJ = os.environ.get("SF_BN_FUSE_PROJ", "1") != "0"
+BN_FUSE_LATERAL = os.environ.get("SF_BN_FUSE_LATERAL", "1") != "0"
 SEGMENTS = None
 
 
@@ -609,6 +611,12 @@
         else:
             cat = ops.cl_empty((N, Cs + Cf, T, H, W), x_s.device)
             ops.bn_act(x_s, out=cat[:, :Cs])
+        prev = getattr(x_s, "_sf_block_bn", None)
+        if BN_FUSE_REDUCE and BN_FUSE_LATERAL and prev is not None and mod.training:
+            tag = {"bits": prev["bits"], "y0": prev["y0"], "sync": prev["sync"], "win": (0, Cs)}
+            if _sync_of(unit.bn) is None:
+                tag["set_b"] = {"y": yf, "scale": st.scale, "shift": st.shift, "win": (Cs, Cs + Cf)}
+            cat._sf_block_bn = tag
         ops.bn_act(yf, st.scale, st.shift, relu=True, out=cat[:, Cs:])
         if CAPTURE is not None:
             CAPTURE.append({"kind": "fuse", "mod": mod, "raw": [yf], "bn": [(st.scale, st.shift)]})
@@ -622,12 +630,16 @@
         unit = ctx.mod._unit
         (x_f,) = ctx.saved_tensors
         dcat = as_cl(dcat)
-        dyf = unit.bn_backward(dcat[:, ctx.Cs:], ctx.yf, ctx.st, relu_self=True)
+        part_f = tagged_bn_part(dcat, ctx.yf, slot=1)
+        dyf = unit.bn_backward(dcat[:, ctx.Cs:], ctx.yf, ctx.st, relu_self=True, part=part_f)
         need_dx = ctx.needs_input_grad[1]
         dx_f = unit.backward(x_f, None, dyf, need_dx=need_dx, resid=as_cl(dxf) if dxf is not None else None)
         _notify(unit.params())
         ctx.yf = None
         dx_s = dcat[:, :ctx.Cs] if ctx.needs_input_grad[0] else None
+        tag = getattr(dcat, _BN_PART_SLOTS[0], None)
+        if dx_s is not None and tag is not None and tag[2] == dcat.data_ptr() and tag[3] == dcat._version:
+            setattr(dx_s, _BN_PART_SLOTS[0], (tag[0], tag[1], dx_s.data_ptr(), dx_s._version))
         return (dx_s, dx_f, None) + param_grads(ctx, 3)
 
 
@@ -677,6 +689,8 @@
         ctx.save_for_backward(x)
         if BN_FUSE_REDUCE and tr:
             out._sf_block_bn = {"bits": bits, "y0": yc, "sync": _sync_of(units[-1].bn) is not None}
+            if P is not None and BN_FUSE_PROJ and _sync_of(P.bn) is None:
+                out._sf_block_bn["y1"] = y1
         return out
 
     @staticmethod
@@ -689,11 +703,12 @@
         bn, s1 = ctx.bn
         last = len(units) - 1
         part_c = tagged_bn_part(dout, raw[last])
+        part_p = tagged_bn_part(dout, y1, slot=1) if P is not None else None
         dout = as_cl(dout)
         need_dx = ctx.needs_input_grad[0]
         dy = units[last].bn_backward(dout, raw[last], bn[last], zmask=bits, part=part_c)
         if P is not None:
-            dy1 = P.bn_backward(dout, y1, s1, zmask=bits)
+            dy1 = P.bn_backward(dout, y1, s1, zmask=bits, part=part_p)
         for i in range(last, 0, -1):
             part = None
             if act[i - 1] is not None and BN_FUSE_REDUCE and _sync_of(units[i - 1].bn) is None:
@@ -713,6 +728,10 @@
             dx = units[0].backward(x, None, dy, need_dx=need_dx, resid=dout, resid_bits=bits, bn_fuse=prev)
         if prev is not None:
             dx, pc = dx
+            if isinstance(pc, tuple):
+                pc, pb = pc
+                if pb is not None:
+                    tag_bn_part(dx, prev["y1"] if "y1" in prev else prev["set_b"]["y"], pb, slot=1)
             if pc is not None:
                 tag_bn_part(dx, prev["y0"], pc)
         _notify(mod._param_list)
@@ -724,20 +743,28 @@
 _cut_bn_tags = {}
 
 
+_BN_PART_SLOTS = ("_sf_bn_part", "_sf_bn_part2")
+
+
 def retag_cut_grad(g):
-    tag = _cut_bn_tags.pop(g.data_ptr(), None)
-    if tag is not None and getattr(g, "_sf_bn_part", None) is None and tag[2] == g.data_ptr() and tag[3] == g._version:
-        g._sf_bn_part = tag
-
-
-def tag_bn_part(dx, y0, part):
-    dx._sf_bn_part = (y0.data_ptr(), part, dx.data_ptr(), dx._version)
+    tags = _cut_bn_tags.pop(g.data_ptr(), None)
+    for slot, tag in (tags or {}).items():
+        if getattr(g, _BN_PART_SLOTS[slot], None) is None and tag[2] == g.data_ptr() and tag[3] == g._version:
+            setattr(g, _BN_PART_SLOTS[slot], tag)
+
+
+def tag_bn_part(dx, y0, part, slot=0):
+    tag = (y0.data_ptr(), part, dx.data_ptr(), dx._version)
+    setattr(dx, _BN_PART_SLOTS[slot], tag)
     if CUT_BACKWARD:
-        _cut_bn_tags[dx.data_ptr()] = dx._sf_bn_part
-
-
-def tagged_bn_part(dout, y0):
-    tag = getattr(dout, "_sf_bn_part", None)
+        rec = _cut_bn_tags.get(dx.data_ptr())
+        if rec is None or any(t[1] is not tag[1] and getattr(dx, _BN_PART_SLOTS[k], None) is not t for k, t in rec.items()):
+            rec = _cut_bn_tags[dx.data_ptr()] = {}
+        rec[slot] = tag
+
+
+def tagged_bn_part(dout, y0, slot=0):
+    tag = getattr(dout, _BN_PART_SLOTS[slot], None)
     if tag is None or tag[0] != y0.data_ptr() or tag[2] != dout.data_ptr() or tag[3] != dout._version:
         return None
     return tag[1]
diff --git a/slowfast_amd/lib.py b/slowfast_amd/lib.py
--- a/slowfast_amd/lib.py
+++ b/slowfast_amd/lib.py
@@ -3,7 +3,7 @@
 from ctypes import POINTER, Structure, c_char_p, c_float, c_int, c_int32, c_int64, c_void_p
 
 _HERE = os.path.dirname(os.path.abspath(__file__))
-ABI_VERSION = 26
+ABI_VERSION = 27
 ACT_MODE = os.environ.get("SF_ACT_DTYPE", "fp16").lower()
 if ACT_MODE not in ("fp16", "bf16"):
     raise ValueError(f"SF_ACT_DTYPE={ACT_MODE!r}: expected fp16 or bf16")
@@ -30,6 +30,12 @@
 
     _fields_ = [("w", c_void_p), ("wf", c_void_p), ("wd", c_void_p)] + [(n, c_int32) for n in (
         "Co", "Cow", "Cw", "Cp", "taps", "ldf", "ldd", "pad")]
+
+
+class BnSet(Structure):
+
+    _fields_ = [("y", c_void_p), ("ldy", c_int32), ("bits", c_void_p), ("ld_bits", c_int32), ("scale", c_void_p),
+                ("shift", c_void_p), ("c0", c_int32), ("c1", c_int32), ("part", c_void_p), ("rows", c_int32)]
 
 
 class DwDesc(Structure):
@@ -75,6 +81,7 @@
     "sf_conv_dgrad": (c_int, [POINTER(ConvDesc), _P, _P, _P, c_int32, _P, _P, _P]),
     "sf_conv_dgrad_bn": (c_int, [POINTER(ConvDesc), _P, _P, _P, c_int32, _P, _P, _P, _P, _P, _P, c_int32, _P, c_int32,
                                  POINTER(c_int32), _P]),
+    "sf_conv_dgrad_bn2": (c_int, [POINTER(ConvDesc), _P, _P, _P, c_int32, _P, _P, POINTER(BnSet), c_int32, c_int32, _P]),
     "sf_conv_wgrad_workspace": (c_int64, [POINTER(ConvDesc)]),
     "sf_conv_wgrad_rowtab_bytes": (c_int64, [POINTER(ConvDesc)]),
     "sf_conv_wgrad_rowtab": (c_int, [POINTER(ConvDesc), _P, _P]),
diff --git a/slowfast_amd/ops.py b/slowfast_amd/ops.py
--- a/slowfast_amd/ops.py
+++ b/slowfast_amd/ops.py
@@ -4,7 +4,7 @@
 
 from . import lib as _sflib
 
-from .lib import ConvDesc, SfError, get_lib
+from .lib import BnSet, ConvDesc, SfError, get_lib
 
 _f16 = _sflib.act_dtype()
 
@@ -205,6 +205,8 @@
         assert tuple(resid.shape) == geom.in_shape
     if out is not None:
         assert tuple(out.shape) == geom.in_shape
+    if isinstance(bn, dict) and ("win" in bn or "y1" in bn or "set_b" in bn):
+        return _conv_dgrad_bn2(dy, wd, geom, resid, out, resid_bits, bn)
     if bn is not None:
         if not isinstance(bn, dict):
             y0, sc, sh = bn
@@ -236,6 +238,44 @@
                    _ptr(resid_bits), dx.data_ptr(), _stream(dy),
                    work=geom.work(reads_x=int(resid is not None), reads_y=1, writes_x=1))
     return dx
+
+
+def _conv_dgrad_bn2(dy, wd, geom, resid, out, resid_bits, bn):
+    N, Ci, T, H, W = geom.in_shape
+    M = N * T * H * W
+    bits, y0 = bn["bits"], bn["y0"]
+    c0, c1 = bn.get("win", (0, Ci))
+    assert "y1" not in bn or "set_b" not in bn, "a second set is either the projection's (y1) or a windowed one (set_b)"
+    assert tuple(y0.shape) == (N, c1 - c0, T, H, W)
+    assert bits.dtype == torch.uint8 and bits.numel() == M * ((c1 - c0) // 8) and bits.is_contiguous()
+    if resid_bits is not None:
+        assert resid is not None and resid_bits.dtype == torch.uint8 and resid_bits.numel() == rows(resid) * (Ci // 8)
+    dx = cl_empty(geom.in_shape, dy.device) if out is None else out
+    cap = (M + 127) // 128
+    sets = (BnSet * 2)()
+    keep = [torch.empty((cap, 2, c1 - c0), dtype=torch.float32, device=dy.device)]
+    sets[0] = BnSet(y0.data_ptr(), cl_ld(y0), bits.data_ptr(), (c1 - c0) // 8, None, None, c0, c1, keep[0].data_ptr(), 0)
+    nsets = 1
+    if "y1" in bn:
+        y1 = bn["y1"]
+        assert tuple(y1.shape) == tuple(y0.shape)
+        keep.append(torch.empty((cap, 2, c1 - c0), dtype=torch.float32, device=dy.device))
+        sets[1] = BnSet(y1.data_ptr(), cl_ld(y1), bits.data_ptr(), (c1 - c0) // 8, None, None, c0, c1, keep[1].data_ptr(), 0)
+        nsets = 2
+    elif "set_b" in bn:
+        b = bn["set_b"]
+        b0, b1 = b["win"]
+        yb, sc, sh = b["y"], b["scale"], b["shift"]
+        assert tuple(yb.shape) == (N, b1 - b0, T, H, W) and sc.dtype == torch.float32 and sh.dtype == torch.float32
+        assert sc.numel() >= b1 - b0 and sh.numel() >= b1 - b0
+        keep.append(torch.empty((cap, 2, b1 - b0), dtype=torch.float32, device=dy.device))
+        sets[1] = BnSet(yb.data_ptr(), cl_ld(yb), None, 0, sc.data_ptr(), sh.data_ptr(), b0, b1, keep[1].data_ptr(), 0)
+        nsets = 2
+    get_lib().call("sf_conv_dgrad_bn2", byref(geom.desc(cl_ld(dx), cl_ld(dy))), dy.data_ptr(), wd.data_ptr(), _ptr(resid),
+                   cl_ld(resid) if resid is not None else 0, _ptr(resid_bits), dx.data_ptr(), sets, nsets, cap, _stream(dy),
+                   work=geom.work(reads_x=nsets + int(resid is not None), reads_y=1, writes_x=1))
+    parts = [keep[i][:sets[i].rows] if i < nsets and sets[i].rows > 0 else None for i in range(2)]
+    return dx, (parts[0], parts[1])
 
 
 _workspaces = {}
```
